# linjieli222/HERO

Hardware: AMD Instinct MI355X
Metric: videos/sec training step, HERO-base TVR-shaped batch (higher is better)
Workload: dtype bf16; 1 GPU; configs[1]: HERO-base TVR finetune micro-step (train-tvr-8gpu.json shapes: 32 videos x 60 frames, 15 subs x (4 frames + 20 tokens), 15-token query; vfeat 4352; fwd + VSM loss + bwd, all-reduce/clip/AdamW every 2nd micro-step); global_batch=32, parallelism=dp1, grad_accum=2, launch=hipGraph replay, input=one batch resident in HBM

## Files before the change

### hero_amd/_lib.py

```python
import ctypes as C
import os

import torch

_HERE = os.path.dirname(os.path.abspath(__file__))
LIB_PATH = os.environ.get("HERO_HIP_LIB") or os.path.join(_HERE, "libhero_hip.so")

ABI_VERSION = 3
F32, BF16 = 0, 1
LAYOUT_K, LAYOUT_O = 0, 1
ACT_NONE, ACT_GELU, ACT_RELU, ACT_GELU_BWD, ACT_RELU_BWD, ACT_GELU_DG, ACT_MUL_AUX = 0, 1, 2, 3, 4, 5, 6

EXPORTS = [
    "hero_last_error", "hero_abi_version", "hero_abi_struct_count", "hero_abi_struct_bytes", "hero_gemm", "hero_gemm_splits", "hero_fold_slabs", "hero_wgrad_group", "hero_wgrad_batch_plan", "hero_wgrad_batch", "hero_prof_enable", "hero_prof_read", "hero_probe_mfma", "hero_probe_hbm", "hero_gemm_force_config", "hero_layernorm_fwd",
    "hero_layernorm_bwd_workspace_bytes", "hero_layernorm_bwd", "hero_colsum_workspace_bytes",
    "hero_colsum", "hero_colsum_multi", "hero_colsum_multi_workspace_bytes", "hero_layernorm_bwd_blocks", "hero_attention_fwd", "hero_attention_bwd", "hero_attention_max_len", "hero_attention_max_packed_len", "hero_attention_stats_ok", "hero_attention_force_ppw",
    "hero_gather_rows", "hero_inverse_first", "hero_csr_gather_sum", "hero_scatter_add_rows", "hero_segment_sort_workspace_bytes", "hero_scatter_add_sorted_workspace_bytes", "hero_segment_sort", "hero_scatter_add_sorted", "hero_cast", "hero_transpose_cast", "hero_copy_multi",
    "hero_relu_bwd", "hero_gelu_bwd", "hero_add", "hero_sumsq", "hero_adamw", "hero_adamw_multi", "hero_adamw_multi_chunk",
    "hero_query_pool_fwd", "hero_query_pool_bwd", "hero_rownorm_fwd", "hero_rownorm_bwd", "hero_score_max_fwd",
    "hero_score_max_bwd", "hero_rank_loss", "hero_sums_scaled", "hero_st_ed_fwd", "hero_st_ed_bwd", "hero_st_ed_bwd_workspace_bytes",
    "hero_cross_entropy_fwd", "hero_cross_entropy_bwd", "hero_qa_pool_fwd", "hero_qa_pool_bwd",
    "hero_topk_rows", "hero_st_ed_probs", "hero_moment_topk", "hero_moment_nms", "hero_first_hit",
    "hero_collate_subs", "hero_collate_clip_mask", "hero_collate_frame_map", "hero_collate_gather_feats", "hero_derive_multi",
    "hero_comm_available", "hero_comm_unique_id", "hero_comm_init", "hero_comm_destroy", "hero_comm_rank", "hero_comm_world",
    "hero_comm_allreduce_buckets", "hero_comm_broadcast", "hero_comm_allgather", "hero_comm_allgather_var",
]


class Dropout(C.Structure):
    _fields_ = [("seed_ptr", C.c_void_p), ("site", C.c_uint64),
                ("threshold16", C.c_uint32), ("scale", C.c_float)]


class GemmEpilogue(C.Structure):
    _fields_ = [("bias", C.c_void_p), ("residual", C.c_void_p), ("aux", C.c_void_p),
                ("act", C.c_int), ("out_f32", C.c_int), ("beta", C.c_float),
                ("split_k", C.c_int), ("dropout", Dropout), ("colsum", C.c_void_p), ("colsum_partial", C.c_int), ("pad_", C.c_int), ("split_stride", C.c_longlong)]


class CrossEntropy(C.Structure):
    _fields_ = [("logits", C.c_void_p), ("labels", C.c_void_p), ("loss", C.c_void_p), ("lse", C.c_void_p),
                ("dloss", C.c_void_p), ("dlogits", C.c_void_p), ("rows", C.c_int), ("cols", C.c_int),
                ("ld", C.c_int), ("dtype", C.c_int), ("inv_temp", C.c_float), ("ignore_index", C.c_int64)]


class Derive(C.Structure):
    _fields_ = [("src", C.c_void_p), ("dst", C.c_void_p), ("n", C.c_int64), ("mode", C.c_int), ("p0", C.c_int),
                ("p1", C.c_int), ("p2", C.c_int)]


DERIVE_MASK_ADD, DERIVE_F32, DERIVE_I32, DERIVE_FLAT_GATHER = 0, 1, 2, 3


class WgradProblem(C.Structure):
    _fields_ = [("dy", C.c_void_p), ("x", C.c_void_p), ("dw", C.c_void_p), ("M", C.c_int), ("N", C.c_int),
                ("ld_dy", C.c_int), ("ld_x", C.c_int), ("ld_dw", C.c_int), ("split_hint", C.c_int), ("dbias", C.c_void_p)]


class LnFwd(C.Structure):
    _fields_ = [("x", C.c_void_p), ("tab", C.c_void_p * 3), ("idx", C.c_void_p * 3),
                ("gamma", C.c_void_p), ("beta", C.c_void_p), ("y", C.c_void_p),
                ("pre", C.c_void_p), ("mean", C.c_void_p), ("rstd", C.c_void_p),
                ("rows", C.c_int), ("cols", C.c_int), ("eps", C.c_float),
                ("x_dtype", C.c_int), ("y_dtype", C.c_int), ("dropout", Dropout)]


class LnBwd(C.Structure):
    _fields_ = [("x", C.c_void_p), ("dy", C.c_void_p), ("gamma", C.c_void_p),
                ("mean", C.c_void_p), ("rstd", C.c_void_p), ("dx", C.c_void_p),
                ("dx_dropped", C.c_void_p), ("dgamma", C.c_void_p), ("dbeta", C.c_void_p),
                ("grad_beta", C.c_float), ("workspace", C.c_void_p),
                ("rows", C.c_int), ("cols", C.c_int), ("x_dtype", C.c_int), ("dtype", C.c_int),
                ("dropout_out", Dropout), ("dropout_in", Dropout), ("dbias_in", C.c_void_p), ("defer_fold", C.c_int)]


class Colsum(C.Structure):
    _fields_ = [("src", C.c_void_p), ("dst", C.c_void_p), ("rows", C.c_int), ("cols", C.c_int), ("ld", C.c_int),
                ("dtype", C.c_int), ("beta", C.c_float), ("row_cols", C.c_int), ("dst_rows", C.c_void_p)]


class Attn(C.Structure):
    _fields_ = [("qkv", C.c_void_p), ("mask", C.c_void_p), ("ctx", C.c_void_p),
                ("probs", C.c_void_p), ("dctx", C.c_void_p), ("dqkv", C.c_void_p),
                ("S", C.c_int), ("L", C.c_int), ("H", C.c_int), ("scale", C.c_float),
                ("dtype", C.c_int), ("dropout", Dropout), ("seq_off", C.c_void_p), ("stats", C.c_void_p)]


class AdamW(C.Structure):
    _fields_ = [("p", C.c_void_p), ("g", C.c_void_p), ("m", C.c_void_p), ("v", C.c_void_p),
                ("n", C.c_size_t), ("lr", C.c_float), ("beta1", C.c_float), ("beta2", C.c_float),
                ("eps", C.c_float), ("weight_decay", C.c_float), ("step", C.c_int),
                ("grad_sumsq", C.c_void_p), ("max_grad_norm", C.c_float),
                ("grad_scale", C.c_float), ("shadow", C.c_void_p)]


class TensorDesc(C.Structure):
    _fields_ = [("p", C.c_void_p), ("g", C.c_void_p), ("m", C.c_void_p), ("v", C.c_void_p),
                ("n", C.c_uint64), ("group", C.c_int32), ("step_lag", C.c_int32)]


class AdamWGroup(C.Structure):
    _fields_ = [("lr", C.c_float), ("beta1", C.c_float), ("beta2", C.c_float), ("eps", C.c_float),
                ("weight_decay", C.c_float)]


class AdamWMulti(C.Structure):
    _fields_ = [("descs", C.c_void_p), ("chunk_tensor", C.c_void_p), ("chunk_index", C.c_void_p),
                ("n_chunks", C.c_int), ("groups", AdamWGroup * 8), ("step", C.c_int),
                ("grad_sumsq", C.c_void_p), ("max_grad_norm", C.c_float), ("grad_scale", C.c_float),
                ("step_ptr", C.c_void_p), ("lr_ptr", C.c_void_p), ("tensor_steps", C.c_void_p), ("n_tensors", C.c_int)]


class CopyDesc(C.Structure):
    _fields_ = [("src", C.c_void_p), ("dst", C.c_void_p), ("rows", C.c_int32), ("cols", C.c_int32),
                ("ldd", C.c_int32), ("transpose", C.c_int32), ("dst_dtype", C.c_int32), ("pad_", C.c_int32)]


class QueryPool(C.Structure):
    _fields_ = [("q", C.c_void_p), ("mask", C.c_void_p), ("w", C.c_void_p), ("pooled", C.c_void_p),
                ("att", C.c_void_p), ("dpooled", C.c_void_p), ("dq", C.c_void_p), ("dw", C.c_void_p),
                ("B", C.c_int), ("L", C.c_int), ("D", C.c_int), ("dtype", C.c_int)]


class RowNorm(C.Structure):
    _fields_ = [("x", C.c_void_p), ("y", C.c_void_p), ("rnorm", C.c_void_p), ("dy", C.c_void_p),
                ("dx", C.c_void_p), ("rows", C.c_int), ("cols", C.c_int), ("x_dtype", C.c_int),
                ("eps", C.c_float)]


class ScoreMax(C.Structure):
    _fields_ = [("s", C.c_void_p), ("mask", C.c_void_p), ("out", C.c_void_p), ("arg", C.c_void_p),
                ("ds_ctx", C.c_void_p), ("ds_q", C.c_void_p), ("gc", C.c_void_p), ("gq", C.c_void_p),
                ("qn", C.c_void_p), ("cn", C.c_void_p), ("dqn", C.c_void_p), ("dcn", C.c_void_p),
                ("M", C.c_int), ("N", C.c_int), ("L", C.c_int), ("D", C.c_int), ("n0", C.c_int),
                ("n_own", C.c_int), ("ld_s", C.c_int), ("gc_scale", C.c_float), ("gq_scale", C.c_float)]


class RankLoss(C.Structure):
    _fields_ = [("s", C.c_void_p), ("loss_ctx_rows", C.c_void_p), ("loss_q_rows", C.c_void_p),
                ("ds_ctx", C.c_void_p), ("ds_q", C.c_void_p), ("nq", C.c_int), ("nv", C.c_int),
                ("margin", C.c_float), ("lse", C.c_int), ("hard", C.c_int), ("pool", C.c_int),
                ("hard_w", C.c_float), ("easy_w", C.c_float)]


class StEd(C.Structure):
    _fields_ = [("q2", C.c_void_p), ("ctx", C.c_void_p), ("mask", C.c_void_p), ("w_st", C.c_void_p),
                ("w_ed", C.c_void_p), ("targets", C.c_void_p), ("loss_rows", C.c_void_p),
                ("p_st", C.c_void_p), ("p_ed", C.c_void_p), ("sim", C.c_void_p), ("g", C.c_void_p),
                ("dq2", C.c_void_p), ("dctx", C.c_void_p), ("dw_st", C.c_void_p), ("dw_ed", C.c_void_p),
                ("B", C.c_int), ("L", C.c_int), ("D", C.c_int), ("K", C.c_int), ("dtype", C.c_int), ("g_scale", C.c_float),
                ("ws", C.c_void_p)]


class CommBucket(C.Structure):
    _fields_ = [("buf", C.c_void_p), ("count", C.c_size_t), ("dtype", C.c_int), ("pad_", C.c_int)]


ABI_STRUCTS = [Dropout, GemmEpilogue, WgradProblem, LnFwd, LnBwd, Colsum, Attn, AdamW, TensorDesc, AdamWGroup, AdamWMulti,
               CopyDesc, QueryPool, RowNorm, ScoreMax, RankLoss, StEd, CrossEntropy, Derive, CommBucket]


def abi_struct_sizes():
    return {st.__name__: C.sizeof(st) for st in ABI_STRUCTS}


_lib = None


def lib():
    global _lib
    if _lib is None:
        if not os.path.exists(LIB_PATH):
            raise RuntimeError(
                "hero_amd: %s is missing. Build it with `python -m hero_amd.build` "
                "(needs hipcc; cross-compiles for gfx950 without a GPU). There is no fallback "
                "path." % LIB_PATH)
        L = C.CDLL(LIB_PATH)
        L.hero_last_error.restype = C.c_char_p
        have = L.hero_abi_version()
        if have != ABI_VERSION:
            raise RuntimeError("hero_amd: %s reports ABI version %d, this binding was written against %d (struct layouts "
                               "differ: rebuild with `python -m hero_amd.build --force`)" % (LIB_PATH, have, ABI_VERSION))
        L.hero_abi_struct_bytes.argtypes = [C.c_int]
        if L.hero_abi_struct_count() != len(ABI_STRUCTS):
            raise RuntimeError("hero_amd: %s declares %d ABI structs, this binding mirrors %d" % (LIB_PATH, L.hero_abi_struct_count(), len(ABI_STRUCTS)))
        bad = [(st.__name__, C.sizeof(st), L.hero_abi_struct_bytes(i)) for i, st in enumerate(ABI_STRUCTS)
               if C.sizeof(st) != L.hero_abi_struct_bytes(i)]
        if bad:
            raise RuntimeError("hero_amd: struct layouts differ from %s (name, binding bytes, library bytes): %s" % (LIB_PATH, bad))
        L.hero_layernorm_bwd_workspace_bytes.restype = C.c_size_t
        L.hero_colsum_workspace_bytes.restype = C.c_size_t
        L.hero_colsum_multi_workspace_bytes.restype = C.c_size_t
        L.hero_colsum_multi_workspace_bytes.argtypes = [C.POINTER(Colsum), C.c_int]
        L.hero_colsum_multi.argtypes = [C.POINTER(Colsum), C.c_int, C.c_void_p, C.c_void_p]
        L.hero_layernorm_bwd_blocks.argtypes = [C.c_int]
        L.hero_gemm.argtypes = [C.c_void_p, C.c_void_p, C.c_void_p] + [C.c_int] * 9 + [
            C.POINTER(GemmEpilogue), C.c_void_p]
        L.hero_gemm_splits.argtypes = [C.c_int, C.c_int, C.c_int]
        L.hero_fold_slabs.argtypes = [C.c_void_p, C.c_int, C.c_size_t, C.c_void_p, C.c_size_t, C.c_int, C.c_void_p]
        L.hero_wgrad_group.argtypes = [C.POINTER(WgradProblem), C.c_int, C.c_int, C.c_int, C.c_void_p]
        L.hero_wgrad_batch_plan.argtypes = [C.POINTER(WgradProblem), C.c_int, C.c_int, C.c_void_p, C.c_int]
        L.hero_wgrad_batch.argtypes = [C.POINTER(WgradProblem), C.c_int, C.c_int, C.c_int, C.c_void_p, C.c_int, C.c_void_p]
        L.hero_prof_enable.argtypes = [C.c_int]
        L.hero_prof_read.argtypes = [C.c_int, C.POINTER(C.c_double), C.POINTER(C.c_double),
                                     C.POINTER(C.c_longlong)]
        L.hero_probe_mfma.argtypes = [C.c_void_p, C.c_size_t, C.POINTER(C.c_double), C.POINTER(C.c_double), C.c_void_p]
        L.hero_probe_hbm.argtypes = [C.c_void_p, C.c_void_p, C.c_size_t, C.POINTER(C.c_double), C.POINTER(C.c_double), C.c_void_p]
        L.hero_layernorm_fwd.argtypes = [C.POINTER(LnFwd), C.c_void_p]
        L.hero_layernorm_bwd.argtypes = [C.POINTER(LnBwd), C.c_void_p]
        L.hero_layernorm_bwd_workspace_bytes.argtypes = [C.c_int, C.c_int]
        L.hero_colsum_workspace_bytes.argtypes = [C.c_int, C.c_int]
        L.hero_colsum.argtypes = [C.c_void_p, C.c_void_p, C.c_int, C.c_int, C.c_int, C.c_int,
                                  C.c_float, C.c_void_p, C.c_void_p]
        L.hero_attention_fwd.argtypes = [C.POINTER(Attn), C.c_void_p]
        L.hero_attention_bwd.argtypes = [C.POINTER(Attn), C.c_void_p]
        L.hero_attention_stats_ok.argtypes = [C.c_int, C.c_int]
        L.hero_attention_force_ppw.argtypes = [C.c_int]
        L.hero_attention_max_len.argtypes = [C.c_int, C.c_int]
        L.hero_attention_max_packed_len.argtypes = [C.c_int]
        L.hero_gather_rows.argtypes = [C.c_void_p, C.c_void_p, C.c_void_p, C.c_void_p,
                                       C.c_int, C.c_int, C.c_int, C.c_void_p]
        L.hero_inverse_first.argtypes = [C.c_void_p, C.c_int, C.c_void_p, C.c_int, C.c_int, C.c_void_p]
        L.hero_csr_gather_sum.argtypes = [C.c_void_p, C.c_void_p, C.c_void_p, C.c_void_p,
                                          C.c_int, C.c_int, C.c_int, C.c_void_p]
        L.hero_scatter_add_rows.argtypes = [C.c_void_p, C.c_void_p, C.c_void_p, C.c_void_p,
                                            C.c_int, C.c_int, C.c_int, C.c_int, C.c_int, C.c_void_p]
        L.hero_segment_sort_workspace_bytes.argtypes = [C.c_int]
        L.hero_segment_sort_workspace_bytes.restype = C.c_size_t
        L.hero_segment_sort.argtypes = [C.c_void_p, C.c_int, C.c_int, C.c_int, C.c_void_p, C.c_void_p, C.c_void_p]
        L.hero_scatter_add_sorted_workspace_bytes.argtypes = [C.c_int, C.c_int]
        L.hero_scatter_add_sorted_workspace_bytes.restype = C.c_size_t
        L.hero_scatter_add_sorted.argtypes = [C.c_void_p, C.c_void_p, C.c_void_p, C.c_void_p, C.c_int, C.c_int, C.c_int, C.c_int,
                                              C.c_void_p, C.c_void_p]
        L.hero_st_ed_bwd_workspace_bytes.argtypes = [C.c_int]
        L.hero_st_ed_bwd_workspace_bytes.restype = C.c_size_t
        L.hero_cast.argtypes = [C.c_void_p, C.c_void_p, C.c_size_t, C.c_int, C.c_int, C.c_void_p]
        L.hero_transpose_cast.argtypes = [C.c_void_p, C.c_void_p, C.c_int, C.c_int, C.c_int, C.c_int,
                                          C.c_void_p]
        L.hero_relu_bwd.argtypes = [C.c_void_p, C.c_void_p, C.c_void_p, C.c_size_t, C.c_int,
                                    C.c_void_p]
        L.hero_gelu_bwd.argtypes = L.hero_relu_bwd.argtypes
        L.hero_add.argtypes = [C.c_void_p, C.c_void_p, C.c_void_p, C.c_size_t, C.c_int, C.c_void_p]
        L.hero_sumsq.argtypes = [C.c_void_p, C.c_size_t, C.c_void_p, C.c_void_p, C.c_void_p]
        L.hero_adamw.argtypes = [C.POINTER(AdamW), C.c_void_p]
        L.hero_adamw_multi.argtypes = [C.POINTER(AdamWMulti), C.c_void_p]
        L.hero_copy_multi.argtypes = [C.c_void_p, C.c_void_p, C.c_void_p, C.c_int, C.c_void_p]
        for fn, st in (("hero_query_pool_fwd", QueryPool), ("hero_query_pool_bwd", QueryPool),
                       ("hero_rownorm_fwd", RowNorm), ("hero_rownorm_bwd", RowNorm),
                       ("hero_score_max_fwd", ScoreMax), ("hero_score_max_bwd", ScoreMax),
                       ("hero_rank_loss", RankLoss), ("hero_st_ed_fwd", StEd), ("hero_st_ed_bwd", StEd)):
            getattr(L, fn).argtypes = [C.POINTER(st), C.c_void_p]
        L.hero_sums_scaled.argtypes = [C.c_void_p, C.c_int, C.c_int, C.POINTER(C.c_float), C.c_void_p, C.c_void_p]
        L.hero_topk_rows.argtypes = [C.c_void_p, C.c_int, C.c_int, C.c_int, C.c_int, C.c_float, C.c_void_p, C.c_void_p, C.c_void_p]
        L.hero_st_ed_probs.argtypes = [C.c_void_p, C.c_longlong] + [C.c_void_p] * 4 + [C.c_int] * 5 + [C.c_void_p] * 3
        L.hero_moment_topk.argtypes = [C.c_void_p] * 3 + [C.c_int] * 6 + [C.c_void_p] * 3
        L.hero_moment_nms.argtypes = [C.c_void_p] * 3 + [C.c_int, C.c_int, C.c_double, C.c_int, C.c_int] + [C.c_void_p] * 3
        L.hero_first_hit.argtypes = [C.c_void_p] * 3 + [C.c_int] * 3 + [C.c_void_p, C.c_void_p, C.c_float, C.c_void_p, C.c_int, C.c_void_p, C.c_void_p]
        L.hero_collate_subs.argtypes = [C.c_void_p] * 4 + [C.c_int] * 3 + [C.c_void_p]
        L.hero_collate_gather_feats.argtypes = [C.c_void_p] * 7 + [C.c_int] * 5 + [C.c_void_p]
        L.hero_derive_multi.argtypes = [C.POINTER(Derive), C.c_int, C.c_void_p]
        L.hero_collate_clip_mask.argtypes = [C.c_void_p, C.c_void_p, C.c_int, C.c_int, C.c_void_p]
        L.hero_collate_frame_map.argtypes = [C.c_void_p] * 7 + [C.c_int] * 4 + [C.c_void_p]
        L.hero_cross_entropy_fwd.argtypes = [C.POINTER(CrossEntropy), C.c_void_p]
        L.hero_cross_entropy_bwd.argtypes = [C.POINTER(CrossEntropy), C.c_void_p]
        L.hero_qa_pool_fwd.argtypes = [C.c_void_p] * 8 + [C.c_int] * 6 + [C.c_void_p]
        L.hero_qa_pool_bwd.argtypes = [C.c_void_p] * 11 + [C.c_int] * 6 + [C.c_void_p]
        L.hero_comm_unique_id.argtypes = [C.c_void_p]
        L.hero_comm_init.argtypes = [C.c_void_p, C.c_int, C.c_int, C.POINTER(C.c_void_p)]
        L.hero_comm_destroy.argtypes = [C.c_void_p]
        L.hero_comm_rank.argtypes = [C.c_void_p]
        L.hero_comm_world.argtypes = [C.c_void_p]
        L.hero_comm_allreduce_buckets.argtypes = [C.c_void_p, C.POINTER(CommBucket), C.c_int, C.c_void_p]
        L.hero_comm_broadcast.argtypes = [C.c_void_p, C.c_void_p, C.c_size_t, C.c_int, C.c_void_p]
        L.hero_comm_allgather.argtypes = [C.c_void_p, C.c_void_p, C.c_void_p, C.c_size_t, C.c_void_p]
        L.hero_comm_allgather_var.argtypes = [C.c_void_p, C.c_void_p, C.c_void_p, C.POINTER(C.c_size_t), C.c_void_p]
        _lib = L
    return _lib


def check(rc):
    if rc != 0:
        raise RuntimeError("libhero_hip: %s (code %d)" % (lib().hero_last_error().decode(), rc))


def dt(t):
    if t.dtype == torch.float32:
        return F32
    if t.dtype == torch.bfloat16:
        return BF16
    raise TypeError("hero_amd: unsupported dtype %s (float32 / bfloat16 only)" % t.dtype)


def ptr(t):
    if t is None:
        return None
    if not t.is_cuda:
        raise RuntimeError("hero_amd: tensor is on %s; the HIP path needs CUDA/ROCm tensors and has "
                           "no CPU fallback" % t.device)
    if not t.is_contiguous():
        raise RuntimeError("hero_amd: non-contiguous tensor passed to a HIP kernel")
    return t.data_ptr()


_raw_stream = getattr(torch._C, "_cuda_getCurrentRawStream", None)
_cur_device = getattr(torch._C, "_cuda_getDevice", None)


def stream():
    if _raw_stream is not None and _cur_device is not None:
        return _raw_stream(_cur_device())
    return torch.cuda.current_stream().cuda_stream


def no_dropout():
    return Dropout(None, 0, 0, 1.0)
```

### hero_amd/csrc/rows.hip

```cpp
#include "common.h"

namespace hero {

template <typename T>
__global__ void gather_rows_kernel(const T* __restrict__ a, const T* __restrict__ b, const int32_t* __restrict__ idx,
                                   T* __restrict__ out, int rows, int cols) {
  const int c4n = cols >> 2;
  for (size_t q = blockIdx.x * (size_t)blockDim.x + threadIdx.x; q < (size_t)rows * c4n; q += (size_t)gridDim.x * blockDim.x) {
    const int r = (int)(q / c4n), c = (int)(q - (size_t)r * c4n) * 4;
    const int i = idx[r];
    float4 v = make_float4(0.f, 0.f, 0.f, 0.f);
    if (i >= 0) v = V4<T>::ld(a + (size_t)i * cols + c);
    else if (i <= -2) v = V4<T>::ld(b + (size_t)(-i - 2) * cols + c);
    V4<T>::st(out + (size_t)r * cols + c, v);
  }
}

__global__ __launch_bounds__(1024) void inverse_first_kernel(const int32_t* __restrict__ idx, int n, int32_t* __restrict__ inv, int na, int nb) {
  extern __shared__ int lds_inv[];
  const int tot = na + nb;
  for (int i = threadIdx.x; i < tot; i += 1024) lds_inv[i] = 0x7fffffff;
  __syncthreads();
  for (int j = threadIdx.x; j < n; j += 1024) {
    const int v = idx[j];
    if (v >= 0 && v < na) atomicMin(&lds_inv[v], j);
    else if (v <= -2 && -v - 2 < nb) atomicMin(&lds_inv[na - v - 2], j);
  }
  __syncthreads();
  for (int i = threadIdx.x; i < tot; i += 1024) { const int v = lds_inv[i]; inv[i] = v == 0x7fffffff ? -1 : v; }
}

template <typename T>
__global__ void csr_gather_sum_kernel(const T* __restrict__ src, const int32_t* __restrict__ offs,
                                      const int32_t* __restrict__ ent, T* __restrict__ out, int rows, int cols) {
  const int c4n = cols >> 2;
  for (size_t q = blockIdx.x * (size_t)blockDim.x + threadIdx.x; q < (size_t)rows * c4n; q += (size_t)gridDim.x * blockDim.x) {
    const int r = (int)(q / c4n), c = (int)(q - (size_t)r * c4n) * 4;
    float4 v = make_float4(0.f, 0.f, 0.f, 0.f);
    for (int e = offs[r]; e < offs[r + 1]; ++e) {
      const float4 w = V4<T>::ld(src + (size_t)ent[e] * cols + c);
      v.x += w.x; v.y += w.y; v.z += w.z; v.w += w.w;
    }
    V4<T>::st(out + (size_t)r * cols + c, v);
  }
}

__device__ __forceinline__ void atomic_add2(float* p, float x, float y) {
  atomicAdd(p, x);
  atomicAdd(p + 1, y);
}
__device__ __forceinline__ void atomic_add2(bf16_t* p, float x, float y) {
  uint32_t* w = reinterpret_cast<uint32_t*>(p);
  uint32_t old = *w, assumed;
  do {
    assumed = old;
    const float lo = __uint_as_float(assumed << 16) + x;
    const float hi = __uint_as_float(assumed & 0xffff0000u) + y;
    const uint32_t nw = (uint32_t)f2bf(lo) | ((uint32_t)f2bf(hi) << 16);
    old = atomicCAS(w, assumed, nw);
  } while (old != assumed);
}

template <typename TS, typename TD>
__global__ void scatter_add_rows_kernel(const TS* __restrict__ src, const int32_t* __restrict__ idx, TD* dst_a, TD* dst_b,
                                        int rows, int cols, int skip) {
  const int c2n = cols >> 1;
  for (size_t q = blockIdx.x * (size_t)blockDim.x + threadIdx.x; q < (size_t)rows * c2n; q += (size_t)gridDim.x * blockDim.x) {
    const int r = (int)(q / c2n), c = (int)(q - (size_t)r * c2n) * 2;
    const int i = idx[r];
    if (i == -1 || i == skip) continue;
    const float x = ld1<TS>(src + (size_t)r * cols + c), y = ld1<TS>(src + (size_t)r * cols + c + 1);
    if (x == 0.f && y == 0.f) continue;
    TD* d = i >= 0 ? dst_a + (size_t)i * cols + c : (dst_b ? dst_b + (size_t)(-i - 2) * cols + c : nullptr);
    if (d) atomic_add2(d, x, y);
  }
}

constexpr int SORT_NT = 1024;
__global__ __launch_bounds__(SORT_NT) void segment_sort_kernel(const int32_t* __restrict__ idx, int rows, int skip, int nbits,
                                                               uint2* __restrict__ buf0, uint2* __restrict__ buf1,
                                                               int32_t* __restrict__ order) {
  extern __shared__ uint32_t hist[];
  uint32_t* wsum = hist + 16 * SORT_NT;
  const int t = threadIdx.x, lane = t & 63, wv = t >> 6;
  const int cpt = (rows + SORT_NT - 1) / SORT_NT;
  const int beg = min(t * cpt, rows), end = min(beg + cpt, rows);
  const uint32_t last_key = (1u << nbits) - 1u;
  for (int i = beg; i < end; ++i) {
    const int v = idx[i];
    buf0[i] = make_uint2((v < 0 || v == skip) ? last_key : (uint32_t)v, (uint32_t)i);
  }
  __syncthreads();
  uint2* src = buf0;
  uint2* dst = buf1;
  for (int shift = 0; shift < nbits; shift += 4) {
    uint32_t cnt[16];
#pragma unroll
    for (int b = 0; b < 16; ++b) cnt[b] = 0;
    for (int i = beg; i < end; ++i) {
      const uint32_t d = (src[i].x >> shift) & 15u;
#pragma unroll
      for (int b = 0; b < 16; ++b) cnt[b] += (d == (uint32_t)b);
    }
#pragma unroll
    for (int b = 0; b < 16; ++b) hist[b * SORT_NT + t] = cnt[b];
    __syncthreads();
    uint32_t loc[16], run = 0;
#pragma unroll
    for (int k = 0; k < 16; ++k) { loc[k] = run; run += hist[16 * t + k]; }
    uint32_t inc = run;
#pragma unroll
    for (int o = 1; o < 64; o <<= 1) {
      const uint32_t u = __shfl_up(inc, o, 64);
      if (lane >= o) inc += u;
    }
    if (lane == 63) wsum[wv] = inc;
    __syncthreads();
    uint32_t base = inc - run;
    for (int w = 0; w < wv; ++w) base += wsum[w];
#pragma unroll
    for (int k = 0; k < 16; ++k) hist[16 * t + k] = base + loc[k];
    __syncthreads();
    uint32_t pos[16];
#pragma unroll
    for (int b = 0; b < 16; ++b) pos[b] = hist[b * SORT_NT + t];
    for (int i = beg; i < end; ++i) {
      const uint2 e = src[i];
      const uint32_t d = (e.x >> shift) & 15u;
      uint32_t at = 0;
#pragma unroll
      for (int b = 0; b < 16; ++b)
        if (d == (uint32_t)b) { at = pos[b]; pos[b] += 1; }
      dst[at] = e;
    }
    __syncthreads();
    uint2* tmp = src; src = dst; dst = tmp;
  }
  for (int i = t; i < rows; i += SORT_NT) order[i] = (int32_t)src[i].y;
}

#ifndef HERO_SEG_B
#define HERO_SEG_B 16
#endif
constexpr int SEG_B = HERO_SEG_B;
constexpr int UNR = 8;
__device__ __forceinline__ int seg_key(const int32_t* idx, const int32_t* order, int i, int rows, int skip) {
  if (i < 0 || i >= rows) return -2;
  const int v = idx[order[i]];
  return (v < 0 || v == skip) ? -1 : v;
}

template <typename TS, int NCH>
__global__ __launch_bounds__(256) void scatter_sorted_kernel(const TS* __restrict__ src, const int32_t* __restrict__ idx,
                                                             const int32_t* __restrict__ order, float* __restrict__ dst,
                                                             float* __restrict__ partial, int rows, int cols, int skip) {
  const int blk = blockIdx.x * 4 + (threadIdx.x >> 6), lane = threadIdx.x & 63;
  const int base = blk * SEG_B;
  if (base >= rows) return;
  const int n = min(SEG_B, rows - base);
  const int my_row = lane < n ? order[base + lane] : 0;
  int my_key = -2;
  if (lane < n) { const int v = idx[my_row]; my_key = (v < 0 || v == skip) ? -1 : v; }
  const int prev_key = seg_key(idx, order, base - 1, rows, skip), next_key = seg_key(idx, order, base + n, rows, skip);
  for (int c0 = 0; c0 < cols; c0 += NCH * 256) {
    float4 acc[NCH];
#pragma unroll
    for (int k = 0; k < NCH; ++k) acc[k] = make_float4(0.f, 0.f, 0.f, 0.f);
    int seg_start = 0;
    for (int p0 = 0; p0 < n; p0 += UNR) {
      float4 v[UNR][NCH], old[UNR][NCH];
      int keys[UNR];
#pragma unroll
      for (int u = 0; u < UNR; ++u) {
        const int p = min(p0 + u, n - 1);
        keys[u] = __shfl(my_key, p, 64);
        const int r = __shfl(my_row, p, 64);
        const int kd = max(keys[u], 0);
#pragma unroll
        for (int k = 0; k < NCH; ++k) {
          const int c = min(c0 + k * 256 + lane * 4, cols - 4);
          v[u][k] = V4<TS>::ld(src + (size_t)r * cols + c);
          old[u][k] = *reinterpret_cast<const float4*>(dst + (size_t)kd * cols + c);
        }
      }
#pragma unroll
      for (int u = 0; u < UNR; ++u) {
        const int p = p0 + u;
        if (p < n) {
          const int key = keys[u];
          const int key_next = p + 1 < n ? __shfl(my_key, p + 1, 64) : -3;
          if (key >= 0) {
#pragma unroll
            for (int k = 0; k < NCH; ++k) { acc[k].x += v[u][k].x; acc[k].y += v[u][k].y; acc[k].z += v[u][k].z; acc[k].w += v[u][k].w; }
          }
          if (key_next != key) {
            if (key >= 0) {
              const bool left_open = seg_start == 0 && prev_key == key;
              const bool right_open = p == n - 1 && next_key == key;
              const bool closed = !left_open && !right_open;
              float* out = closed ? dst + (size_t)key * cols : partial + ((size_t)blk * 2 + (left_open ? 0 : 1)) * cols;
#pragma unroll
              for (int k = 0; k < NCH; ++k) {
                const int c = c0 + k * 256 + lane * 4;
                if (c < cols) {
                  float4 o = acc[k];
                  if (closed) { o.x += old[u][k].x; o.y += old[u][k].y; o.z += old[u][k].z; o.w += old[u][k].w; }
                  *reinterpret_cast<float4*>(out + c) = o;
                }
              }
            }
#pragma unroll
            for (int k = 0; k < NCH; ++k) acc[k] = make_float4(0.f, 0.f, 0.f, 0.f);
            seg_start = p + 1;
          }
        }
      }
    }
  }
}

__global__ __launch_bounds__(256) void scatter_sorted_fold_kernel(const int32_t* __restrict__ idx, const int32_t* __restrict__ order,
                                                                  float* __restrict__ dst, const float* __restrict__ partial,
                                                                  int rows, int cols, int skip) {
  const int blk = blockIdx.x * 4 + (threadIdx.x >> 6), lane = threadIdx.x & 63;
  const int base = blk * SEG_B;
  if (base >= rows) return;
  const int n = min(SEG_B, rows - base);
  const int last = seg_key(idx, order, base + n - 1, rows, skip);
  if (last < 0 || seg_key(idx, order, base + n, rows, skip) != last) return;
  const bool whole = seg_key(idx, order, base, rows, skip) == last;
  if (whole && seg_key(idx, order, base - 1, rows, skip) == last) return;
  const int nblk = (rows + SEG_B - 1) / SEG_B;
  int nb = 0;
  for (int b0 = blk + 1; b0 < nblk; b0 += 64) {
    const int b = b0 + lane;
    const bool cont = b < nblk && seg_key(idx, order, b * SEG_B, rows, skip) == last;
    const unsigned long long m = __ballot(cont);
    const int run = m == ~0ull ? 64 : __builtin_ctzll(~m);
    nb += run;
    if (run < 64) break;
  }
  constexpr int NCH = 3, FB = 8;
  for (int c0 = 0; c0 < cols; c0 += NCH * 256) {
    float4 acc[NCH];
    int cc[NCH];
#pragma unroll
    for (int k = 0; k < NCH; ++k) {
      cc[k] = min(c0 + k * 256 + lane * 4, cols - 4);
      acc[k] = *reinterpret_cast<const float4*>(partial + ((size_t)blk * 2 + 1) * cols + cc[k]);
    }
    for (int b0 = 1; b0 <= nb; b0 += FB) {
      float4 t[FB][NCH];
#pragma unroll
      for (int u = 0; u < FB; ++u) {
        const int b = blk + min(b0 + u, nb);
#pragma unroll
        for (int k = 0; k < NCH; ++k) t[u][k] = *reinterpret_cast<const float4*>(partial + ((size_t)b * 2 + 0) * cols + cc[k]);
      }
#pragma unroll
      for (int u = 0; u < FB; ++u) {
        if (b0 + u <= nb) {
#pragma unroll
          for (int k = 0; k < NCH; ++k) { acc[k].x += t[u][k].x; acc[k].y += t[u][k].y; acc[k].z += t[u][k].z; acc[k].w += t[u][k].w; }
        }
      }
    }
#pragma unroll
    for (int k = 0; k < NCH; ++k) {
      const int c = c0 + k * 256 + lane * 4;
      if (c < cols) {
        float4* d = reinterpret_cast<float4*>(dst + (size_t)last * cols + c);
        float4 o = *d;
        o.x += acc[k].x; o.y += acc[k].y; o.z += acc[k].z; o.w += acc[k].w;
        *d = o;
      }
    }
  }
}

template <typename TS, typename TD>
__global__ void cast_kernel(const TS* __restrict__ s, TD* __restrict__ d, size_t n) {
  const size_t n4 = n >> 2;
  for (size_t q = blockIdx.x * (size_t)blockDim.x + threadIdx.x; q < n4; q += (size_t)gridDim.x * blockDim.x)
    V4<TD>::st(d + q * 4, V4<TS>::ld(s + q * 4));
  if (blockIdx.x == 0 && threadIdx.x < (n & 3)) st1<TD>(d + n4 * 4 + threadIdx.x, ld1<TS>(s + n4 * 4 + threadIdx.x));
}
template <typename TD>
__global__ __launch_bounds__(256) void transpose_cast_kernel(const float* __restrict__ src, TD* __restrict__ dst, int R, int C, int ldd) {
  __shared__ float tile[32][33];
  const int tx = threadIdx.x & 31, ty = threadIdx.x >> 5;
  const int r0 = blockIdx.y * 32, c0 = blockIdx.x * 32;
#pragma unroll
  for (int k = 0; k < 4; ++k) {
    const int r = r0 + ty + 8 * k, c = c0 + tx;
    tile[ty + 8 * k][tx] = (r < R && c < C) ? src[(size_t)r * C + c] : 0.f;
  }
  __syncthreads();
#pragma unroll
  for (int k = 0; k < 4; ++k) {
    const int c = c0 + ty + 8 * k, r = r0 + tx;
    if (c < C && r < R) st1<TD>(dst + (size_t)c * ldd + r, tile[tx][ty + 8 * k]);
  }
}

__global__ __launch_bounds__(256) void copy_multi_kernel(const HeroCopyDesc* __restrict__ descs, const int32_t* __restrict__ tile_desc,
                                                         const int32_t* __restrict__ tile_index) {
  __shared__ float tile[64][65];
  const HeroCopyDesc d = descs[tile_desc[blockIdx.x]];
  const int tcols = (d.cols + 63) >> 6;
  const int ti = tile_index[blockIdx.x];
  const int r0 = (ti / tcols) * 64, c0 = (ti % tcols) * 64;
  const int q = threadIdx.x & 15, ty = threadIdx.x >> 4;
  const bool vec = (d.cols & 3) == 0 && (d.ldd & 3) == 0 && ((uintptr_t)d.src & 15) == 0 && ((uintptr_t)d.dst & 15) == 0;
  if (!d.transpose) {
#pragma unroll
    for (int k = 0; k < 4; ++k) {
      const int r = r0 + ty + 16 * k, c = c0 + 4 * q;
      if (r >= d.rows || c >= d.cols) continue;
      if (vec) {
        const float4 v = *reinterpret_cast<const float4*>(d.src + (size_t)r * d.cols + c);
        if (d.dst_dtype == HERO_BF16) V4<bf16_t>::st(static_cast<bf16_t*>(d.dst) + (size_t)r * d.ldd + c, v);
        else *reinterpret_cast<float4*>(static_cast<float*>(d.dst) + (size_t)r * d.ldd + c) = v;
      } else {
        for (int e = 0; e < 4 && c + e < d.cols; ++e) {
          const float v = d.src[(size_t)r * d.cols + c + e];
          if (d.dst_dtype == HERO_BF16) static_cast<bf16_t*>(d.dst)[(size_t)r * d.ldd + c + e] = f2bf(v);
          else static_cast<float*>(d.dst)[(size_t)r * d.ldd + c + e] = v;
        }
      }
    }
    return;
  }
  const bool vin = (d.cols & 3) == 0 && ((uintptr_t)d.src & 15) == 0;
#pragma unroll
  for (int k = 0; k < 4; ++k) {
    const int rl = ty + 16 * k, r = r0 + rl, c = c0 + 4 * q;
    float4 v = make_float4(0.f, 0.f, 0.f, 0.f);
    if (r < d.rows && c < d.cols) {
      if (vin) v = *reinterpret_cast<const float4*>(d.src + (size_t)r * d.cols + c);
      else {
        v.x = d.src[(size_t)r * d.cols + c];
        if (c + 1 < d.cols) v.y = d.src[(size_t)r * d.cols + c + 1];
        if (c + 2 < d.cols) v.z = d.src[(size_t)r * d.cols + c + 2];
        if (c + 3 < d.cols) v.w = d.src[(size_t)r * d.cols + c + 3];
      }
    }
    tile[rl][4 * q] = v.x; tile[rl][4 * q + 1] = v.y; tile[rl][4 * q + 2] = v.z; tile[rl][4 * q + 3] = v.w;
  }
  __syncthreads();
  const bool vout = (d.ldd & 3) == 0 && (((uintptr_t)d.dst) & 15) == 0 && (d.rows & 3) == 0;
#pragma unroll
  for (int k = 0; k < 4; ++k) {
    const int cl = ty + 16 * k, c = c0 + cl, r = r0 + 4 * q;
    if (c >= d.cols || r >= d.rows) continue;
    const float4 v = make_float4(tile[4 * q][cl], tile[4 * q + 1][cl], tile[4 * q + 2][cl], tile[4 * q + 3][cl]);
    if (vout) {
      if (d.dst_dtype == HERO_BF16) V4<bf16_t>::st(static_cast<bf16_t*>(d.dst) + (size_t)c * d.ldd + r, v);
      else *reinterpret_cast<float4*>(static_cast<float*>(d.dst) + (size_t)c * d.ldd + r) = v;
    } else {
      const float e4[4] = {v.x, v.y, v.z, v.w};
      for (int e = 0; e < 4 && r + e < d.rows; ++e) {
        if (d.dst_dtype == HERO_BF16) static_cast<bf16_t*>(d.dst)[(size_t)c * d.ldd + r + e] = f2bf(e4[e]);
        else static_cast<float*>(d.dst)[(size_t)c * d.ldd + r + e] = e4[e];
      }
    }
  }
}

template <typename T>
__global__ void relu_bwd_kernel(const T* __restrict__ dy, const T* __restrict__ y, T* __restrict__ dx, size_t n) {
  const size_t n4 = n >> 2;
  for (size_t q = blockIdx.x * (size_t)blockDim.x + threadIdx.x; q < n4; q += (size_t)gridDim.x * blockDim.x) {
    float4 g = V4<T>::ld(dy + q * 4);
    const float4 v = V4<T>::ld(y + q * 4);
    g.x = v.x > 0.f ? g.x : 0.f; g.y = v.y > 0.f ? g.y : 0.f; g.z = v.z > 0.f ? g.z : 0.f; g.w = v.w > 0.f ? g.w : 0.f;
    V4<T>::st(dx + q * 4, g);
  }
}
template <typename T>
__global__ void gelu_bwd_kernel(const T* __restrict__ dy, const T* __restrict__ u, T* __restrict__ dx, size_t n) {
  const size_t n4 = n >> 2;
  for (size_t q = blockIdx.x * (size_t)blockDim.x + threadIdx.x; q < n4; q += (size_t)gridDim.x * blockDim.x) {
    float4 g = V4<T>::ld(dy + q * 4);
    const float4 v = V4<T>::ld(u + q * 4);
    g.x *= gelu_erf_grad(v.x); g.y *= gelu_erf_grad(v.y); g.z *= gelu_erf_grad(v.z); g.w *= gelu_erf_grad(v.w);
    V4<T>::st(dx + q * 4, g);
  }
}
template <typename T>
__global__ void add_kernel(const T* __restrict__ a, const T* __restrict__ b, T* __restrict__ y, size_t n) {
  const size_t n4 = n >> 2;
  for (size_t q = blockIdx.x * (size_t)blockDim.x + threadIdx.x; q < n4; q += (size_t)gridDim.x * blockDim.x) {
    float4 u = V4<T>::ld(a + q * 4);
    const float4 v = V4<T>::ld(b + q * 4);
    u.x += v.x; u.y += v.y; u.z += v.z; u.w += v.w;
    V4<T>::st(y + q * 4, u);
  }
}

__global__ void sumsq_kernel(const float* __restrict__ g, size_t n, float* out) {
  __shared__ float red[4];
  float s = 0.f;
  const size_t n4 = n >> 2;
  for (size_t q = blockIdx.x * (size_t)blockDim.x + threadIdx.x; q < n4; q += (size_t)gridDim.x * blockDim.x) {
    const float4 v = *reinterpret_cast<const float4*>(g + q * 4);
    s += (v.x * v.x + v.y * v.y) + (v.z * v.z + v.w * v.w);
  }
  if (blockIdx.x == 0 && threadIdx.x < (n & 3)) { const float v = g[n4 * 4 + threadIdx.x]; s += v * v; }
  s = wave_sum(s);
  if ((threadIdx.x & 63) == 0) red[threadIdx.x >> 6] = s;
  __syncthreads();
  if (threadIdx.x == 0) out[blockIdx.x] = (red[0] + red[1]) + (red[2] + red[3]);
}
__global__ void sumsq_final_kernel(const float* __restrict__ partial, int nblocks, float* out) {
  __shared__ float red[4];
  float s = 0.f;
  for (int i = threadIdx.x; i < nblocks; i += 256) s += partial[i];
  s = wave_sum(s);
  if ((threadIdx.x & 63) == 0) red[threadIdx.x >> 6] = s;
  __syncthreads();
  if (threadIdx.x == 0) out[0] += (red[0] + red[1]) + (red[2] + red[3]);
}

__global__ void adamw_kernel(HeroAdamW a, float bc1, float bc2) {
  float gs = a.grad_scale;
  if (a.grad_sumsq) {
    const float norm = sqrtf(*a.grad_sumsq) * fabsf(a.grad_scale);
    const float clip = a.max_grad_norm / (norm + 1e-6f);
    if (clip < 1.f) gs *= clip;
  }
  const float step_size = a.lr * sqrtf(bc2) / bc1;
  const float decay = a.lr * a.weight_decay;
  bf16_t* sh = static_cast<bf16_t*>(a.shadow);
  const size_t n4 = a.n >> 2;
  for (size_t q = blockIdx.x * (size_t)blockDim.x + threadIdx.x; q < n4; q += (size_t)gridDim.x * blockDim.x) {
    float4 p = *reinterpret_cast<float4*>(a.p + q * 4);
    const float4 g4 = *reinterpret_cast<const float4*>(a.g + q * 4);
    float4 m = *reinterpret_cast<float4*>(a.m + q * 4);
    float4 v = *reinterpret_cast<float4*>(a.v + q * 4);
    float* pp = &p.x; const float* gp = &g4.x; float* mp = &m.x; float* vp = &v.x;
#pragma unroll
    for (int k = 0; k < 4; ++k) {
      const float g = gp[k] * gs;
      mp[k] = a.beta1 * mp[k] + (1.f - a.beta1) * g;
      vp[k] = a.beta2 * vp[k] + (1.f - a.beta2) * g * g;
      pp[k] -= step_size * mp[k] / (sqrtf(vp[k]) + a.eps);
      pp[k] -= decay * pp[k];
    }
    *reinterpret_cast<float4*>(a.p + q * 4) = p;
    *reinterpret_cast<float4*>(a.m + q * 4) = m;
    *reinterpret_cast<float4*>(a.v + q * 4) = v;
    if (sh) V4<bf16_t>::st(sh + q * 4, p);
  }
  if (blockIdx.x == 0 && threadIdx.x < (a.n & 3)) {
    const size_t i = n4 * 4 + threadIdx.x;
    const float g = a.g[i] * gs;
    const float m = a.beta1 * a.m[i] + (1.f - a.beta1) * g;
    const float v = a.beta2 * a.v[i] + (1.f - a.beta2) * g * g;
    float p = a.p[i] - step_size * m / (sqrtf(v) + a.eps);
    p -= decay * p;
    a.p[i] = p; a.m[i] = m; a.v[i] = v;
    if (sh) sh[i] = f2bf(p);
  }
}

constexpr int MT_CHUNK = 16384;
__global__ void adamw_steps_inc_kernel(const HeroTensorDesc* descs, int n, int32_t* steps) {
  const int i = blockIdx.x * blockDim.x + threadIdx.x;
  if (i < n) steps[descs[i].step_lag] += 1;
}
__global__ __launch_bounds__(256) void adamw_multi_kernel(HeroAdamWMulti a) {
  const int ti = a.chunk_tensor[blockIdx.x];
  const HeroTensorDesc d = a.descs[ti];
  const HeroAdamWGroup gr = a.groups[d.group];
  const size_t beg = (size_t)a.chunk_index[blockIdx.x] * MT_CHUNK;
  const size_t end = beg + MT_CHUNK < d.n ? beg + MT_CHUNK : d.n;
  float gs = a.grad_scale;
  if (a.grad_sumsq) {
    const float norm = sqrtf(*a.grad_sumsq) * fabsf(a.grad_scale);
    const float clip = a.max_grad_norm / (norm + 1e-6f);
    if (clip < 1.f) gs *= clip;
  }
  const float st = a.tensor_steps ? (float)a.tensor_steps[d.step_lag] : (float)((a.step_ptr ? *a.step_ptr : a.step) - d.step_lag);
  const float lr = a.lr_ptr ? a.lr_ptr[d.group] : gr.lr;
  const float bc1 = 1.f - powf(gr.beta1, st), bc2 = 1.f - powf(gr.beta2, st);
  const float step_size = lr * sqrtf(bc2) / bc1;
  const float decay = lr * gr.weight_decay;
  const bool vec = (((uintptr_t)d.p | (uintptr_t)d.g | (uintptr_t)d.m | (uintptr_t)d.v) & 15) == 0;
  if (vec) {
    const size_t e4 = beg + ((end - beg) & ~(size_t)3);
    for (size_t i = beg + threadIdx.x * 4; i < e4; i += 256 * 4) {
      float4 p = *reinterpret_cast<float4*>(d.p + i);
      const float4 g4 = *reinterpret_cast<const float4*>(d.g + i);
      float4 m = *reinterpret_cast<float4*>(d.m + i);
      float4 v = *reinterpret_cast<float4*>(d.v + i);
      float* pp = &p.x; const float* gp = &g4.x; float* mp = &m.x; float* vp = &v.x;
#pragma unroll
      for (int k = 0; k < 4; ++k) {
        const float g = gp[k] * gs;
        mp[k] = gr.beta1 * mp[k] + (1.f - gr.beta1) * g;
        vp[k] = gr.beta2 * vp[k] + (1.f - gr.beta2) * g * g;
        pp[k] -= step_size * mp[k] / (sqrtf(vp[k]) + gr.eps);
        pp[k] -= decay * pp[k];
      }
      *reinterpret_cast<float4*>(d.p + i) = p;
      *reinterpret_cast<float4*>(d.m + i) = m;
      *reinterpret_cast<float4*>(d.v + i) = v;
    }
    for (size_t i = e4 + threadIdx.x; i < end; i += 256) {
      const float g = d.g[i] * gs;
      const float m = gr.beta1 * d.m[i] + (1.f - gr.beta1) * g;
      const float v = gr.beta2 * d.v[i] + (1.f - gr.beta2) * g * g;
      float p = d.p[i] - step_size * m / (sqrtf(v) + gr.eps);
      p -= decay * p;
      d.p[i] = p; d.m[i] = m; d.v[i] = v;
    }
  } else {
    for (size_t i = beg + threadIdx.x; i < end; i += 256) {
      const float g = d.g[i] * gs;
      const float m = gr.beta1 * d.m[i] + (1.f - gr.beta1) * g;
      const float v = gr.beta2 * d.v[i] + (1.f - gr.beta2) * g * g;
      float p = d.p[i] - step_size * m / (sqrtf(v) + gr.eps);
      p -= decay * p;
      d.p[i] = p; d.m[i] = m; d.v[i] = v;
    }
  }
}

static inline int grid_for(size_t work_items) {
  size_t b = (work_items + 255) / 256;
  if (b < 1) b = 1;
  if (b > 2048) b = 2048;
  return (int)b;
}

}

using namespace hero;

extern "C" int hero_gather_rows(const void* a, const void* b, const int32_t* idx, void* out, int rows, int cols, int dtype,
                                hero_stream_t stream) {
  HERO_REQUIRE(idx && out, "hero_gather_rows: null pointer");
  HERO_REQUIRE(cols > 0 && cols % 4 == 0, "hero_gather_rows: cols (%d) must be a multiple of 4", cols);
  if (rows <= 0) return HERO_OK;
  hipStream_t s = static_cast<hipStream_t>(stream);
  const int grid = grid_for((size_t)rows * (cols >> 2));
  if (dtype == HERO_F32)
    hipLaunchKernelGGL(gather_rows_kernel<float>, dim3(grid), dim3(256), 0, s, (const float*)a, (const float*)b, idx, (float*)out, rows, cols);
  else if (dtype == HERO_BF16)
    hipLaunchKernelGGL(gather_rows_kernel<bf16_t>, dim3(grid), dim3(256), 0, s, (const bf16_t*)a, (const bf16_t*)b, idx, (bf16_t*)out, rows, cols);
  else { set_error("hero_gather_rows: bad dtype %d", dtype); return HERO_ERR_ARG; }
  return check_launch("hero_gather_rows");
}

extern "C" int hero_inverse_first(const int32_t* idx, int n, int32_t* inv, int na, int nb, hero_stream_t stream) {
  HERO_REQUIRE(idx && inv && n >= 0 && na >= 0 && nb >= 0, "hero_inverse_first: bad arguments");
  if (na + nb == 0) return HERO_OK;
  const size_t lds = (size_t)(na + nb) * sizeof(int);
  if (lds > 150 * 1024) { set_error("hero_inverse_first: %d source rows exceed the LDS-resident table (38400)", na + nb); return HERO_ERR_UNSUPPORTED; }
  if (lds > 65536) HERO_ENSURE_LDS(&inverse_first_kernel, 150 * 1024, "inverse_first_kernel");
  hipLaunchKernelGGL(inverse_first_kernel, dim3(1), dim3(1024), lds, static_cast<hipStream_t>(stream), idx, n, inv, na, nb);
  return check_launch("hero_inverse_first");
}

extern "C" int hero_csr_gather_sum(const void* src, const int32_t* offsets, const int32_t* entries, void* out, int rows,
                                   int cols, int dtype, hero_stream_t stream) {
  HERO_REQUIRE(src && offsets && out, "hero_csr_gather_sum: null pointer");
  HERO_REQUIRE(cols > 0 && cols % 4 == 0, "hero_csr_gather_sum: cols (%d) must be a multiple of 4", cols);
  if (rows <= 0) return HERO_OK;
  hipStream_t s = static_cast<hipStream_t>(stream);
  const int grid = grid_for((size_t)rows * (cols >> 2));
  if (dtype == HERO_F32)
    hipLaunchKernelGGL(csr_gather_sum_kernel<float>, dim3(grid), dim3(256), 0, s, (const float*)src, offsets, entries, (float*)out, rows, cols);
  else if (dtype == HERO_BF16)
    hipLaunchKernelGGL(csr_gather_sum_kernel<bf16_t>, dim3(grid), dim3(256), 0, s, (const bf16_t*)src, offsets, entries, (bf16_t*)out, rows, cols);
  else { set_error("hero_csr_gather_sum: bad dtype %d", dtype); return HERO_ERR_ARG; }
  return check_launch("hero_csr_gather_sum");
}

extern "C" int hero_scatter_add_rows(const void* src, const int32_t* idx, void* dst_a, void* dst_b, int rows, int cols,
                                     int src_dtype, int dst_dtype, int skip_idx, hero_stream_t stream) {
  HERO_REQUIRE(src && idx && dst_a, "hero_scatter_add_rows: null pointer");
  HERO_REQUIRE(cols > 0 && cols % 2 == 0, "hero_scatter_add_rows: cols (%d) must be even", cols);
  if (rows <= 0) return HERO_OK;
  hipStream_t s = static_cast<hipStream_t>(stream);
  const int grid = grid_for((size_t)rows * (cols >> 1));
  const int skip = skip_idx >= 0 ? skip_idx : -1;
  if (src_dtype == HERO_F32 && dst_dtype == HERO_F32)
    hipLaunchKernelGGL((scatter_add_rows_kernel<float, float>), dim3(grid), dim3(256), 0, s, (const float*)src, idx, (float*)dst_a, (float*)dst_b, rows, cols, skip);
  else if (src_dtype == HERO_BF16 && dst_dtype == HERO_F32)
    hipLaunchKernelGGL((scatter_add_rows_kernel<bf16_t, float>), dim3(grid), dim3(256), 0, s, (const bf16_t*)src, idx, (float*)dst_a, (float*)dst_b, rows, cols, skip);
  else if (src_dtype == HERO_BF16 && dst_dtype == HERO_BF16)
    hipLaunchKernelGGL((scatter_add_rows_kernel<bf16_t, bf16_t>), dim3(grid), dim3(256), 0, s, (const bf16_t*)src, idx, (bf16_t*)dst_a, (bf16_t*)dst_b, rows, cols, skip);
  else { set_error("hero_scatter_add_rows: unsupported dtypes %d -> %d", src_dtype, dst_dtype); return HERO_ERR_UNSUPPORTED; }
  return check_launch("hero_scatter_add_rows");
}

extern "C" size_t hero_segment_sort_workspace_bytes(int rows) { return (size_t)(rows > 0 ? rows : 0) * 2 * sizeof(uint2); }

extern "C" int hero_segment_sort(const int32_t* idx, int rows, int n_dst, int skip_idx, int32_t* order, void* workspace,
                                 hero_stream_t stream) {
  HERO_REQUIRE(idx && order && workspace, "hero_segment_sort: null pointer");
  HERO_REQUIRE(n_dst > 0 && n_dst < (1 << 30), "hero_segment_sort: n_dst = %d", n_dst);
  if (rows <= 0) return HERO_OK;
  int nbits = 1;
  while ((1 << nbits) <= n_dst) ++nbits;
  nbits = (nbits + 3) & ~3;
  const int lds = (16 * SORT_NT + 32) * (int)sizeof(uint32_t);
  HERO_ENSURE_LDS(&segment_sort_kernel, lds, "segment_sort_kernel");
  uint2* b0 = static_cast<uint2*>(workspace);
  hipLaunchKernelGGL(segment_sort_kernel, dim3(1), dim3(SORT_NT), lds, static_cast<hipStream_t>(stream), idx, rows,
                     skip_idx >= 0 ? skip_idx : -1, nbits, b0, b0 + rows, order);
  return check_launch("hero_segment_sort");
}

extern "C" size_t hero_scatter_add_sorted_workspace_bytes(int rows, int cols) {
  if (rows <= 0 || cols <= 0) return 0;
  return (size_t)((rows + SEG_B - 1) / SEG_B) * 2 * (size_t)cols * sizeof(float);
}

extern "C" int hero_scatter_add_sorted(const void* src, const int32_t* idx, const int32_t* order, float* dst, int rows, int cols,
                                       int src_dtype, int skip_idx, void* workspace, hero_stream_t stream) {
  HERO_REQUIRE(src && idx && order && dst && workspace, "hero_scatter_add_sorted: null pointer");
  HERO_REQUIRE(cols > 0 && cols % 4 == 0, "hero_scatter_add_sorted: cols (%d) must be a multiple of 4", cols);
  if (rows <= 0) return HERO_OK;
  hipStream_t s = static_cast<hipStream_t>(stream);
  const int nblk = (rows + SEG_B - 1) / SEG_B, grid = (nblk + 3) / 4, skip = skip_idx >= 0 ? skip_idx : -1;
  float* part = static_cast<float*>(workspace);
  if (src_dtype == HERO_BF16) hipLaunchKernelGGL((scatter_sorted_kernel<bf16_t, 3>), dim3(grid), dim3(256), 0, s, (const bf16_t*)src, idx, order, dst, part, rows, cols, skip);
  else if (src_dtype == HERO_F32) hipLaunchKernelGGL((scatter_sorted_kernel<float, 3>), dim3(grid), dim3(256), 0, s, (const float*)src, idx, order, dst, part, rows, cols, skip);
  else { set_error("hero_scatter_add_sorted: bad dtype %d", src_dtype); return HERO_ERR_ARG; }
  int rc = check_launch("hero_scatter_add_sorted");
  if (rc) return rc;
  hipLaunchKernelGGL(scatter_sorted_fold_kernel, dim3(grid), dim3(256), 0, s, idx, order, dst, part, rows, cols, skip);
  return check_launch("hero_scatter_add_sorted(fold)");
}

extern "C" int hero_cast(const void* src, void* dst, size_t n, int sd, int dd, hero_stream_t stream) {
  HERO_REQUIRE(src && dst, "hero_cast: null pointer");
  if (n == 0) return HERO_OK;
  hipStream_t s = static_cast<hipStream_t>(stream);
  const int grid = grid_for(n >> 2);
  if (sd == HERO_F32 && dd == HERO_BF16) hipLaunchKernelGGL((cast_kernel<float, bf16_t>), dim3(grid), dim3(256), 0, s, (const float*)src, (bf16_t*)dst, n);
  else if (sd == HERO_BF16 && dd == HERO_F32) hipLaunchKernelGGL((cast_kernel<bf16_t, float>), dim3(grid), dim3(256), 0, s, (const bf16_t*)src, (float*)dst, n);
  else if (sd == HERO_F32 && dd == HERO_F32) hipLaunchKernelGGL((cast_kernel<float, float>), dim3(grid), dim3(256), 0, s, (const float*)src, (float*)dst, n);
  else if (sd == HERO_BF16 && dd == HERO_BF16) hipLaunchKernelGGL((cast_kernel<bf16_t, bf16_t>), dim3(grid), dim3(256), 0, s, (const bf16_t*)src, (bf16_t*)dst, n);
  else { set_error("hero_cast: bad dtypes %d -> %d", sd, dd); return HERO_ERR_ARG; }
  return check_launch("hero_cast");
}

extern "C" int hero_transpose_cast(const float* src, void* dst, int rows, int cols, int ldd, int dst_dtype, hero_stream_t stream) {
  HERO_REQUIRE(src && dst, "hero_transpose_cast: null pointer");
  if (rows <= 0 || cols <= 0) return HERO_OK;
  hipStream_t s = static_cast<hipStream_t>(stream);
  const dim3 grid((cols + 31) / 32, (rows + 31) / 32);
  if (dst_dtype == HERO_BF16) hipLaunchKernelGGL(transpose_cast_kernel<bf16_t>, grid, dim3(256), 0, s, src, (bf16_t*)dst, rows, cols, ldd);
  else if (dst_dtype == HERO_F32) hipLaunchKernelGGL(transpose_cast_kernel<float>, grid, dim3(256), 0, s, src, (float*)dst, rows, cols, ldd);
  else { set_error("hero_transpose_cast: bad dtype %d", dst_dtype); return HERO_ERR_ARG; }
  return check_launch("hero_transpose_cast");
}

extern "C" int hero_copy_multi(const HeroCopyDesc* descs, const int32_t* tile_desc, const int32_t* tile_index, int n_tiles,
                               hero_stream_t stream) {
  HERO_REQUIRE(descs && tile_desc && tile_index, "hero_copy_multi: null pointer");
  if (n_tiles <= 0) return HERO_OK;
  hipLaunchKernelGGL(copy_multi_kernel, dim3(n_tiles), dim3(256), 0, static_cast<hipStream_t>(stream), descs, tile_desc, tile_index);
  return check_launch("hero_copy_multi");
}

extern "C" int hero_relu_bwd(const void* dy, const void* y, void* dx, size_t n, int dtype, hero_stream_t stream) {
  HERO_REQUIRE(dy && y && dx, "hero_relu_bwd: null pointer");
  HERO_REQUIRE(n % 4 == 0, "hero_relu_bwd: n must be a multiple of 4");
  if (n == 0) return HERO_OK;
  hipStream_t s = static_cast<hipStream_t>(stream);
  const int grid = grid_for(n >> 2);
  if (dtype == HERO_F32) hipLaunchKernelGGL(relu_bwd_kernel<float>, dim3(grid), dim3(256), 0, s, (const float*)dy, (const float*)y, (float*)dx, n);
  else if (dtype == HERO_BF16) hipLaunchKernelGGL(relu_bwd_kernel<bf16_t>, dim3(grid), dim3(256), 0, s, (const bf16_t*)dy, (const bf16_t*)y, (bf16_t*)dx, n);
  else { set_error("hero_relu_bwd: bad dtype %d", dtype); return HERO_ERR_ARG; }
  return check_launch("hero_relu_bwd");
}

extern "C" int hero_gelu_bwd(const void* dy, const void* u, void* dx, size_t n, int dtype, hero_stream_t stream) {
  HERO_REQUIRE(dy && u && dx, "hero_gelu_bwd: null pointer");
  HERO_REQUIRE(n % 4 == 0, "hero_gelu_bwd: n must be a multiple of 4");
  if (n == 0) return HERO_OK;
  hipStream_t s = static_cast<hipStream_t>(stream);
  const int grid = grid_for(n >> 2);
  if (dtype == HERO_F32) hipLaunchKernelGGL(gelu_bwd_kernel<float>, dim3(grid), dim3(256), 0, s, (const float*)dy, (const float*)u, (float*)dx, n);
  else if (dtype == HERO_BF16) hipLaunchKernelGGL(gelu_bwd_kernel<bf16_t>, dim3(grid), dim3(256), 0, s, (const bf16_t*)dy, (const bf16_t*)u, (bf16_t*)dx, n);
  else { set_error("hero_gelu_bwd: bad dtype %d", dtype); return HERO_ERR_ARG; }
  return check_launch("hero_gelu_bwd");
}

extern "C" int hero_add(const void* a, const void* b, void* y, size_t n, int dtype, hero_stream_t stream) {
  HERO_REQUIRE(a && b && y, "hero_add: null pointer");
  HERO_REQUIRE(n % 4 == 0, "hero_add: n must be a multiple of 4");
  if (n == 0) return HERO_OK;
  hipStream_t s = static_cast<hipStream_t>(stream);
  const int grid = grid_for(n >> 2);
  if (dtype == HERO_F32) hipLaunchKernelGGL(add_kernel<float>, dim3(grid), dim3(256), 0, s, (const float*)a, (const float*)b, (float*)y, n);
  else if (dtype == HERO_BF16) hipLaunchKernelGGL(add_kernel<bf16_t>, dim3(grid), dim3(256), 0, s, (const bf16_t*)a, (const bf16_t*)b, (bf16_t*)y, n);
  else { set_error("hero_add: bad dtype %d", dtype); return HERO_ERR_ARG; }
  return check_launch("hero_add");
}

template <typename TO>
__global__ void __launch_bounds__(256) fold_slabs_kernel(const float* __restrict__ slabs, int n_slabs, size_t stride, TO* __restrict__ out, size_t n4) {
  for (size_t i = (size_t)blockIdx.x * 256 + threadIdx.x; i < n4; i += (size_t)gridDim.x * 256) {
    float4 a = *reinterpret_cast<const float4*>(slabs + 4 * i);
    for (int s = 1; s < n_slabs; ++s) {
      const float4 b = *reinterpret_cast<const float4*>(slabs + (size_t)s * stride + 4 * i);
      a.x += b.x; a.y += b.y; a.z += b.z; a.w += b.w;
    }
    V4<TO>::st(out + 4 * i, a);
  }
}

extern "C" int hero_fold_slabs(const float* slabs, int n_slabs, size_t stride, void* out, size_t n, int out_dtype, hero_stream_t stream) {
  HERO_REQUIRE(slabs && out && n_slabs >= 1, "hero_fold_slabs: null pointer / no slab");
  HERO_REQUIRE(n % 4 == 0 && stride % 4 == 0 && (((uintptr_t)slabs | (uintptr_t)out) & 7) == 0, "hero_fold_slabs: n and stride must be multiples of 4, pointers aligned");
  if (n == 0) return HERO_OK;
  hipStream_t s = static_cast<hipStream_t>(stream);
  const int grid = grid_for(n >> 2);
  if (out_dtype == HERO_F32) hipLaunchKernelGGL(fold_slabs_kernel<float>, dim3(grid), dim3(256), 0, s, slabs, n_slabs, stride, (float*)out, n >> 2);
  else if (out_dtype == HERO_BF16) hipLaunchKernelGGL(fold_slabs_kernel<bf16_t>, dim3(grid), dim3(256), 0, s, slabs, n_slabs, stride, (bf16_t*)out, n >> 2);
  else { set_error("hero_fold_slabs: bad dtype %d", out_dtype); return HERO_ERR_ARG; }
  return check_launch("hero_fold_slabs");
}

extern "C" int hero_sumsq(const float* g, size_t n, float* sumsq, float* workspace, hero_stream_t stream) {
  HERO_REQUIRE(g && sumsq && workspace, "hero_sumsq: null pointer");
  if (n == 0) return HERO_OK;
  hipStream_t s = static_cast<hipStream_t>(stream);
  const int nb = grid_for(n >> 2);
  hipLaunchKernelGGL(sumsq_kernel, dim3(nb), dim3(256), 0, s, g, n, workspace);
  hipLaunchKernelGGL(sumsq_final_kernel, dim3(1), dim3(256), 0, s, workspace, nb, sumsq);
  return check_launch("hero_sumsq");
}

extern "C" int hero_adamw(const HeroAdamW* a, hero_stream_t stream) {
  HERO_REQUIRE(a && a->p && a->g && a->m && a->v, "hero_adamw: null pointer");
  HERO_REQUIRE(a->step >= 1, "hero_adamw: step must be >= 1");
  if (a->n == 0) return HERO_OK;
  hipStream_t s = static_cast<hipStream_t>(stream);
  const float bc1 = 1.f - powf(a->beta1, (float)a->step);
  const float bc2 = 1.f - powf(a->beta2, (float)a->step);
  hipLaunchKernelGGL(adamw_kernel, dim3(grid_for(a->n >> 2)), dim3(256), 0, s, *a, bc1, bc2);
  return check_launch("hero_adamw");
}

extern "C" int hero_adamw_multi(const HeroAdamWMulti* a, hero_stream_t stream) {
  HERO_REQUIRE(a && a->descs && a->chunk_tensor && a->chunk_index, "hero_adamw_multi: null pointer");
  HERO_REQUIRE(a->step >= 1 || a->step_ptr || a->tensor_steps, "hero_adamw_multi: step must be >= 1");
  if (a->n_chunks <= 0) return HERO_OK;
  if (a->tensor_steps) {
    HERO_REQUIRE(a->n_tensors > 0, "hero_adamw_multi: tensor_steps needs n_tensors");
    hipLaunchKernelGGL(adamw_steps_inc_kernel, dim3((a->n_tensors + 255) / 256), dim3(256), 0, static_cast<hipStream_t>(stream), a->descs,
                       a->n_tensors, a->tensor_steps);
    const int rc = check_launch("hero_adamw_multi(steps)");
    if (rc) return rc;
  }
  hipLaunchKernelGGL(adamw_multi_kernel, dim3(a->n_chunks), dim3(256), 0, static_cast<hipStream_t>(stream), *a);
  return check_launch("hero_adamw_multi");
}
extern "C" int hero_adamw_multi_chunk(void) { return MT_CHUNK; }
```

### hero_amd/functional.py

```python
import ctypes as C
import math
import os
import weakref

import numpy as np
import torch

from . import _lib as L

_COMPUTE_DTYPE = torch.bfloat16


def set_compute_dtype(dtype):
    global _COMPUTE_DTYPE
    if dtype not in (torch.float32, torch.bfloat16):
        raise ValueError("compute dtype must be torch.float32 or torch.bfloat16")
    _COMPUTE_DTYPE = dtype


def compute_dtype():
    return _COMPUTE_DTYPE


class _Rng:

    def __init__(self):
        self.seeds = {}
        self.site = 0

    def seed_tensor(self, device):
        idx = device.index if device.index is not None else (torch.cuda.current_device() if device.type == "cuda" else None)
        key = (device.type, idx)
        t = self.seeds.get(key)
        if t is None:
            t = torch.tensor([torch.initial_seed() & 0x7FFFFFFFFFFFFFFF], dtype=torch.int64,
                             device=device)
            self.seeds[key] = t
        return t

    def make(self, p, training, device):
        if not training or p <= 0.0:
            return None
        if p >= 1.0:
            raise ValueError("dropout p must be < 1")
        self.site += 1
        return L.Dropout(self.seed_tensor(device).data_ptr(), self.site,
                         max(1, int(round(p * 65536.0))), 1.0 / (1.0 - p))


RNG = _Rng()


def manual_seed(seed, device=None):
    RNG.site = 0
    for t in RNG.seeds.values():
        t.fill_(seed & 0x7FFFFFFFFFFFFFFF)
    if device is not None:
        RNG.seed_tensor(torch.device(device)).fill_(seed & 0x7FFFFFFFFFFFFFFF)


def advance_seed():
    for t in RNG.seeds.values():
        t.add_(1)


def _d(drop):
    return drop if drop is not None else L.no_dropout()


_WCACHE = {}
_WEPOCH = [0]
_WGEN = [0]


def weight_cache_generation():
    return _WGEN[0]


def notify_weights_updated():
    _WEPOCH[0] += 1


def clear_weight_cache():
    _WGEN[0] += 1
    _WCACHE.clear()
    for k in [k for k in _REFRESH if k not in _REFRESH_PINNED]:
        del _REFRESH[k]


_TRUST = [False]


class weights_frozen:

    def __enter__(self):
        self.prev = _TRUST[0]
        _TRUST[0] = True

    def __exit__(self, *exc):
        _TRUST[0] = self.prev


_REFRESH = {}
_REFRESH_PINNED = set()


def refresh_weight_cache():
    if not _WCACHE:
        return
    entries = list(_WCACHE.items())
    tsig = tuple((key, val[1].data_ptr(), tuple(p.data_ptr() for p in val[2])) for key, val in entries)
    if tsig not in _REFRESH:
        if len(_REFRESH) > 16:
            for k in [k for k in _REFRESH if k not in _REFRESH_PINNED][:8]:
                del _REFRESH[k]
        descs, tdesc, tidx = [], [], []
        for key, (_, out, params) in entries:
            transposed = len(key) == 3
            esz, code = out.element_size(), L.dt(out)
            off = 0
            for p in params:
                if not p.is_contiguous() or p.dtype != torch.float32:
                    raise RuntimeError("hero_amd: master weights must be contiguous fp32")
                rows = p.shape[0] if p.dim() > 1 else 1
                cols = p.numel() // rows
                if transposed:
                    d = L.CopyDesc(p.data_ptr(), out.data_ptr() + off * esz, rows, cols, out.shape[1], 1, code, 0)
                    off += rows
                else:
                    d = L.CopyDesc(p.data_ptr(), out.data_ptr() + off * esz, rows, cols, cols, 0, code, 0)
                    off += rows * cols
                nt = (-(-rows // 64)) * (-(-cols // 64))
                tdesc += [len(descs)] * nt
                tidx += list(range(nt))
                descs.append(d)
        dev = entries[0][1][1].device
        arr = (L.CopyDesc * len(descs))(*descs)
        raw = torch.frombuffer(bytearray(bytes(arr)), dtype=torch.uint8).to(dev)
        _REFRESH[tsig] = (raw, torch.tensor(tdesc, dtype=torch.int32, device=dev),
                          torch.tensor(tidx, dtype=torch.int32, device=dev), len(tdesc))
    if torch.cuda.is_current_stream_capturing():
        _REFRESH_PINNED.add(tsig)
    raw, tdesc, tidx, n = _REFRESH[tsig]
    L.check(L.lib().hero_copy_multi(raw.data_ptr(), tdesc.data_ptr(), tidx.data_ptr(), n, L.stream()))
    ep = _WEPOCH[0]
    for key, (_, out, params) in entries:
        _WCACHE[key] = ((tuple(p._version for p in params), tuple(p.data_ptr() for p in params), ep), out, params)


def packed(params, dtype):
    params = tuple(params)
    if len(params) == 1 and dtype == torch.float32 and params[0].is_contiguous():
        return params[0].detach()
    key = (tuple(id(p) for p in params), dtype)
    hit = _WCACHE.get(key)
    if _TRUST[0] and hit is not None and hit[0] is not None and hit[0][2] == _WEPOCH[0]:
        return hit[1]
    sig = (tuple(p._version for p in params), tuple(p.data_ptr() for p in params), _WEPOCH[0])
    if hit is not None and hit[0] == sig:
        return hit[1]
    rows = sum(p.shape[0] for p in params)
    shape = (rows,) + tuple(params[0].shape[1:])
    reuse = hit is not None and tuple(hit[1].shape) == shape and hit[1].device == params[0].device
    out = hit[1] if reuse else torch.empty(shape, dtype=dtype, device=params[0].device)
    off = 0
    for p in params:
        n = p.numel()
        dst = out[off:off + p.shape[0]]
        L.check(L.lib().hero_cast(L.ptr(p.detach().contiguous()), dst.data_ptr(), n, L.F32,
                                  L.dt(out), L.stream()))
        off += p.shape[0]
    if hit is None or not reuse:
        _WGEN[0] += 1
    _WCACHE[key] = (sig, out, params)
    return out


def packed_t(params, dtype):
    params = tuple(params)
    key = (tuple(id(p) for p in params), dtype, "T")
    hit = _WCACHE.get(key)
    if _TRUST[0] and hit is not None and hit[0] is not None and hit[0][2] == _WEPOCH[0]:
        return hit[1]
    sig = (tuple(p._version for p in params), tuple(p.data_ptr() for p in params), _WEPOCH[0])
    if hit is not None and hit[0] == sig:
        return hit[1]
    kin = params[0].shape[1]
    cols = sum(p.shape[0] for p in params)
    reuse = hit is not None and tuple(hit[1].shape) == (kin, cols) and hit[1].device == params[0].device
    out = hit[1] if reuse else torch.empty((kin, cols), dtype=dtype, device=params[0].device)
    off = 0
    for p in params:
        L.check(L.lib().hero_transpose_cast(L.ptr(p.detach().contiguous()),
                                            out.data_ptr() + off * out.element_size(), p.shape[0], kin,
                                            cols, L.dt(out), L.stream()))
        off += p.shape[0]
    if hit is None or not reuse:
        _WGEN[0] += 1
    _WCACHE[key] = (sig, out, params)
    return out


class GradSink:

    def dst(self, p):
        if p.grad is None:
            p.grad = torch.zeros_like(p, memory_format=torch.contiguous_format)
        return p.grad

    def dst_group(self, params):
        return None

    def use(self, p):
        pass

    def done(self, p):
        pass

    def wants_overlap(self):
        return False


SINK = GradSink()


def set_grad_sink(sink):
    global SINK
    SINK = sink if sink is not None else GradSink()


def _use(*params):
    for p in params:
        if p is not None and p.requires_grad:
            SINK.use(p)


def _is_param(t):
    return t is not None and t.is_leaf and t.requires_grad


def _p(t):
    return t if isinstance(t, int) else L.ptr(t)


def k_gemm(A, B, Cm, M, N, K, lda, ldb, ldc, al, bl, dtype_code, bias=None, residual=None,
           aux=None, act=L.ACT_NONE, out_f32=False, beta=0.0, split_k=1, drop=None, colsum=None, split_stride=0,
           colsum_partial=False):
    epi = L.GemmEpilogue(_p(bias), _p(residual), _p(aux), act, 1 if out_f32 else 0,
                         beta, split_k, _d(drop), _p(colsum), 1 if colsum_partial else 0, 0, split_stride)
    L.check(L.lib().hero_gemm(_p(A), _p(B), _p(Cm), M, N, K, lda, ldb, ldc, al, bl,
                              dtype_code, C.byref(epi), L.stream()))


def k_linear(x2, Wc, bias=None, act=L.ACT_NONE, aux=None, residual=None, drop=None):
    M, K = x2.shape
    N = Wc.shape[0]
    y = torch.empty((M, N), dtype=x2.dtype, device=x2.device)
    k_gemm(x2, Wc, y, M, N, K, K, K, N, L.LAYOUT_K, L.LAYOUT_K, L.dt(x2), bias=bias,
           residual=residual, aux=aux, act=act, drop=drop)
    return y


def k_dgrad(dy2, Wc, act=L.ACT_NONE, aux=None, residual=None):
    M, N = dy2.shape
    K = Wc.shape[1]
    dx = torch.empty((M, K), dtype=dy2.dtype, device=dy2.device)
    k_gemm(dy2, Wc, dx, M, K, N, N, K, K, L.LAYOUT_K, L.LAYOUT_O, L.dt(dy2), act=act, aux=aux,
           residual=residual)
    return dx


def k_dgrad_t(dy2, Wt, act=L.ACT_NONE, aux=None, residual=None, colsum=None, colsum_partial=False):
    M, N = dy2.shape
    K = Wt.shape[0]
    if (dy2.dtype == torch.bfloat16 and act == L.ACT_NONE and aux is None and residual is None and colsum is None
            and N >= 8192 and M * K <= (1 << 21) and (M * K) % 4 == 0 and (N - N // 64 * 64) % 8 == 0
            and dy2.is_contiguous() and Wt.is_contiguous() and Wt.shape[1] == N):
        return _dgrad_long_reduction(dy2, Wt)
    dx = torch.empty((M, K), dtype=dy2.dtype, device=dy2.device)
    k_gemm(dy2, Wt, dx, M, K, N, N, N, K, L.LAYOUT_K, L.LAYOUT_K, L.dt(dy2), act=act, aux=aux,
           residual=residual, colsum=colsum, colsum_partial=colsum_partial)
    return dx


def _dgrad_long_reduction(dy2, Wt):
    M, N = dy2.shape
    K = Wt.shape[0]
    n1 = N // 64 * 64
    tiles = -(-M // 128) * -(-K // 128)
    split = max(1, min(n1 // 64 // 8, 16, -(-512 // tiles)))
    n_main = L.lib().hero_gemm_splits(n1, split, L.BF16)
    stride = M * K
    slabs = torch.empty((n_main + (1 if n1 < N else 0), M, K), dtype=torch.float32, device=dy2.device)
    if n_main > 1:
        k_gemm(dy2, Wt, slabs, M, K, n1, N, N, K, L.LAYOUT_K, L.LAYOUT_K, L.BF16, out_f32=True, split_k=split, split_stride=stride)
    else:
        k_gemm(dy2, Wt, slabs, M, K, n1, N, N, K, L.LAYOUT_K, L.LAYOUT_K, L.BF16, out_f32=True)
    if n1 < N:
        k_gemm(L.ptr(dy2) + 2 * n1, L.ptr(Wt) + 2 * n1, L.ptr(slabs) + 4 * n_main * stride, M, K, N - n1, N, N, K,
               L.LAYOUT_K, L.LAYOUT_K, L.BF16, out_f32=True)
    out = torch.empty((M, K), dtype=torch.bfloat16, device=dy2.device)
    L.check(L.lib().hero_fold_slabs(L.ptr(slabs), slabs.shape[0], stride, L.ptr(out), stride, L.BF16, L.stream()))
    return out


def _split_for(n_out, n_in, rows, bk):
    tiles = ((n_out + 127) // 128) * ((n_in + 127) // 128)
    ktiles = max(1, -(-rows // bk))
    flops = 2.0 * n_out * n_in * rows
    out_bytes = 4.0 * n_out * n_in
    best, best_t = 1, None
    for s in range(1, 17):
        if s > 1 and ktiles // s < 4:
            break
        blocks = tiles * s
        rounds = -(-blocks // 512)
        last = blocks - (rounds - 1) * 512
        t = flops / blocks * ((rounds - 1) / 1.83e12 + (1 / 2.7e12 if last <= 256 else 1 / 1.83e12))
        if s > 1:
            t += out_bytes * s / 2.0e12
        if best_t is None or t < best_t:
            best, best_t = s, t
    return best


_WQ = []
_WQ_TASK = [-1]
GROUP_WGRADS = [True]
WGRAD_BATCH = [32]
WGRAD_DBIAS_RIDE = [True]
WGRAD_RIDE_MAX_ROWS = [1 << 30]
B1_EPILOGUE = [False]
B1_PARTIALS = [True]
WGRAD_QUEUE_BYTES = [int(os.environ.get("HERO_WGRAD_QUEUE_MB", "4096")) << 20]
_WQ_BYTES = [0]
_WPLANS = {}
_WPLANS_PINNED = set()


def _wgrad_queue_full(device):
    if _WQ_BYTES[0] <= WGRAD_QUEUE_BYTES[0]:
        return False
    hard = _WQ_HARD.get(device.index)
    if hard is None:
        env = os.environ.get("HERO_WGRAD_QUEUE_HARD_MB")
        hard = (int(env) << 20) if env else max(2 * WGRAD_QUEUE_BYTES[0], int(0.15 * torch.cuda.get_device_properties(device).total_memory))
        _WQ_HARD[device.index] = hard
    if _WQ_BYTES[0] > hard:
        return True
    tiles = sum(-(-e[4] // 192) * -(-e[1].shape[1] // 192) for e in _WQ)
    full, rem = divmod(tiles, 256)
    if rem == 0:
        return True
    p = -(-rem // 8)
    slices = max(1, min(32 // p, 8))
    return tiles / 256.0 >= 0.9 * (full + (1.4 if slices > 1 else 1.0) / slices)


_WQ_HARD = {}


def _wgrad_limit():
    return 4 if (WGRAD_BATCH[0] <= 4 or SINK.wants_overlap()) else min(WGRAD_BATCH[0], 32)


def _wgrad_plan(probs, n, rows, device):
    key = (rows, device.index, tuple((probs[i].M, probs[i].N) for i in range(n)))
    hit = _WPLANS.get(key, False)
    if hit is False:
        buf = np.zeros(8 + 8 * 512 * 16, dtype=np.int32)
        words = L.lib().hero_wgrad_batch_plan(probs, n, rows, buf.ctypes.data, buf.size)
        if words < 0:
            L.check(words)
        hit = (torch.from_numpy(buf[:words].copy()).to(device), words) if words > 0 else None
        if len(_WPLANS) > 256:
            for k in [k for k in _WPLANS if k not in _WPLANS_PINNED][:128]:
                del _WPLANS[k]
        _WPLANS[key] = hit
    if hit is not None and torch.cuda.is_current_stream_capturing():
        _WPLANS_PINNED.add(key)
    return hit


_CB_TASK = [-1]


def _ensure_flush_callback(task):
    if _CB_TASK[0] != task:
        _CB_TASK[0] = task
        torch.autograd.Variable._execution_engine.queue_callback(deferred_flush)


def deferred_flush():
    _CB_TASK[0] = -1
    wgrad_flush()
    colsum_flush()


_CQ = []
_CQ_TASK = [-1]


def _colsum_defer_ok():
    return GROUP_WGRADS[0] and not SINK.wants_overlap() and torch._C._current_graph_task_id() != -1


def _colsum_queue(keep, src_ptr, dst, rows, cols, ld, dtype, on_done=None, dst_rows=None, row_cols=0):
    task = torch._C._current_graph_task_id()
    if _CQ and _CQ_TASK[0] != task:
        del _CQ[:]
    _CQ_TASK[0] = task
    _ensure_flush_callback(task)
    _CQ.append(((keep, dst_rows), L.Colsum(src_ptr, L.ptr(dst), rows, cols, ld, dtype, 1.0, row_cols, L.ptr(dst_rows)), dst, on_done))
    if len(_CQ) >= 64:
        colsum_flush()


def colsum_flush():
    while _CQ:
        part, seen = [], []
        while _CQ and len(part) < 64:
            lo = _CQ[0][1].dst
            hi = lo + 4 * _CQ[0][2].numel()
            if any(lo < b and a < hi for a, b in seen):
                break
            seen.append((lo, hi))
            part.append(_CQ.pop(0))
        n = len(part)
        probs = (L.Colsum * n)(*[e[1] for e in part])
        need = L.lib().hero_colsum_multi_workspace_bytes(probs, n) // 4
        ws = _workspace(max(need, 1), part[0][2].device, slot="colsum_multi")
        L.check(L.lib().hero_colsum_multi(probs, n, L.ptr(ws), L.stream()))
        for e in part:
            if e[3] is not None:
                e[3]()


def wgrad_flush():
    _WQ_BYTES[0] = 0
    while _WQ:
        rows, dtype = _WQ[0][0].shape[0], _WQ[0][0].dtype
        dst_key = lambda e: (e[2].data_ptr(), e[6].data_ptr() if e[6] is not None else None)
        seen_w, seen_b = {_WQ[0][2].data_ptr()}, {dst_key(_WQ[0])[1]} - {None}
        n = 1
        while n < len(_WQ) and n < 32 and _WQ[n][0].shape[0] == rows and _WQ[n][0].dtype == dtype:
            kw, kb = dst_key(_WQ[n])
            if kw in seen_w or (kb is not None and kb in seen_b):
                break
            seen_w.add(kw)
            if kb is not None:
                seen_b.add(kb)
            n += 1
        group, rest = _WQ[:n], _WQ[n:]
        del _WQ[:]
        _WQ.extend(rest)
        probs = (L.WgradProblem * n)()
        for i, (dy2, x2, out, col0, N, _, _, _) in enumerate(group):
            K = x2.shape[1]
            probs[i] = L.WgradProblem(L.ptr(dy2) + col0 * dy2.element_size(), L.ptr(x2), L.ptr(out), N, K,
                                      dy2.shape[1], K, K, _split_for(N, K, rows, 64 if dtype == torch.bfloat16 else 32), None)
        plan = _wgrad_plan(probs, n, rows, group[0][0].device) if dtype == torch.bfloat16 else None
        if plan is not None:
            ride = WGRAD_DBIAS_RIDE[0] and rows <= WGRAD_RIDE_MAX_ROWS[0]
            for i, e in enumerate(group):
                probs[i].dbias = L.ptr(e[6]) if ride else None
                if not ride and e[6] is not None:
                    k_colsum(e[0], out=e[6], beta=1.0, col0=e[3], ncols=e[4], on_done=lambda: None)
            L.check(L.lib().hero_wgrad_batch(probs, n, rows, L.BF16, L.ptr(plan[0]), plan[1], L.stream()))
            for e in group:
                if e[6] is not None and e[7] is not None:
                    e[7]()
        else:
            for g0 in range(0, n, 4):
                sub = (L.WgradProblem * min(4, n - g0))(*[probs[i] for i in range(g0, min(g0 + 4, n))])
                L.check(L.lib().hero_wgrad_group(sub, len(sub), rows, L.dt(group[0][0]), L.stream()))
            for dy2, _, _, col0, N, _, dbias, dbias_done in group:
                if dbias is not None:
                    k_colsum(dy2, out=dbias, beta=1.0, col0=col0, ncols=N, on_done=dbias_done or (lambda: None))
        for e in group:
            if e[5] is not None:
                e[5]()


def k_wgrad(dy2, x2, out=None, beta=0.0, col0=0, ncols=None, on_done=None, dbias=None, dbias_done=None):
    M, ld = dy2.shape
    N = ld - col0 if ncols is None else ncols
    K = x2.shape[1]
    if (out is not None and beta == 1.0 and GROUP_WGRADS[0] and out.is_contiguous() and dy2.is_contiguous()
            and x2.is_contiguous() and torch._C._current_graph_task_id() != -1):
        task = torch._C._current_graph_task_id()
        if _WQ and _WQ_TASK[0] != task:
            del _WQ[:]
            _WQ_BYTES[0] = 0
        if _WQ and (_WQ[0][0].shape[0] != M or _WQ[0][0].dtype != dy2.dtype):
            wgrad_flush()
        if not _WQ:
            _WQ_TASK[0] = task
        _ensure_flush_callback(task)
        _WQ.append((dy2, x2, out, col0, N, on_done, dbias, dbias_done))
        _WQ_BYTES[0] += dy2.numel() * dy2.element_size()
        if len(_WQ) >= _wgrad_limit() or _wgrad_queue_full(dy2.device):
            wgrad_flush()
        return out
    if dbias is not None:
        k_colsum(dy2, out=dbias, beta=1.0, col0=col0, ncols=N, on_done=dbias_done or (lambda: None))
    if out is None:
        out = torch.empty((N, K), dtype=torch.float32, device=dy2.device)
    split = _split_for(N, K, M, 64 if dy2.dtype == torch.bfloat16 else 32)
    a = L.ptr(dy2) + col0 * dy2.element_size()
    k_gemm(a, x2, out, N, K, M, ld, K, K, L.LAYOUT_O, L.LAYOUT_O, L.dt(dy2), out_f32=True,
           beta=beta, split_k=split)
    if on_done is not None:
        on_done()
    return out


_WS = {}


def _workspace(n_floats, device, slot=""):
    key = (device.type, device.index, slot)
    t = _WS.get(key)
    if t is None or t.numel() < n_floats:
        t = torch.empty((max(n_floats, 1 << 20),), dtype=torch.float32, device=device)
        _WS[key] = t
    return t


def k_colsum(dy2, out=None, beta=0.0, col0=0, ncols=None, on_done=None):
    M, ld = dy2.shape
    N = ld - col0 if ncols is None else ncols
    if (on_done is not None and out is not None and beta == 1.0 and dy2.is_contiguous() and N % 4 == 0 and ld % 4 == 0
            and (col0 * dy2.element_size()) % 8 == 0 and _colsum_defer_ok()):
        _colsum_queue(dy2, L.ptr(dy2) + col0 * dy2.element_size(), out, M, N, ld, L.dt(dy2), on_done)
        return out
    if out is None:
        out = torch.empty((N,), dtype=torch.float32, device=dy2.device)
    ws = _workspace(256 * N, dy2.device)
    L.check(L.lib().hero_colsum(L.ptr(dy2) + col0 * dy2.element_size(), L.ptr(out), M, N, ld,
                                L.dt(dy2), beta, L.ptr(ws), L.stream()))
    if on_done is not None:
        on_done()
    return out


def acc_linear_grads(dy2, x2, weight, bias, col0=0, ncols=None):
    N = ncols if ncols is not None else weight.shape[0]
    want_b = bias is not None and bias.requires_grad
    if weight is not None and weight.requires_grad:
        k_wgrad(dy2, x2, out=SINK.dst(weight), beta=1.0, col0=col0, ncols=N, on_done=lambda: SINK.done(weight),
                dbias=SINK.dst(bias) if want_b else None, dbias_done=(lambda: SINK.done(bias)) if want_b else None)
    elif want_b:
        k_colsum(dy2, out=SINK.dst(bias), beta=1.0, col0=col0, ncols=N, on_done=lambda: SINK.done(bias))


def k_ln_fwd(x2, gamma, beta, eps, out_dtype, rows, cols, tabs=(), idxs=(), want_pre=False,
             drop=None, device=None):
    device = device or (x2.device if x2 is not None else gamma.device)
    y = torch.empty((rows, cols), dtype=out_dtype, device=device)
    mean = torch.empty((rows,), dtype=torch.float32, device=device)
    rstd = torch.empty((rows,), dtype=torch.float32, device=device)
    pre = torch.empty((rows, cols), dtype=out_dtype, device=device) if want_pre else None
    a = L.LnFwd()
    a.x = L.ptr(x2)
    for k in range(3):
        a.tab[k] = L.ptr(tabs[k]) if k < len(tabs) else None
        a.idx[k] = L.ptr(idxs[k]) if k < len(idxs) and idxs[k] is not None else None
    a.gamma, a.beta, a.y, a.pre = L.ptr(gamma), L.ptr(beta), L.ptr(y), L.ptr(pre)
    a.mean, a.rstd = L.ptr(mean), L.ptr(rstd)
    a.rows, a.cols, a.eps = rows, cols, eps
    a.x_dtype = L.dt(x2) if x2 is not None else L.dt(y)
    a.y_dtype = L.dt(y)
    a.dropout = _d(drop)
    L.check(L.lib().hero_layernorm_fwd(C.byref(a), L.stream()))
    return y, mean, rstd, pre


def ln_param_dsts(gamma_p, beta_p):
    dg = SINK.dst(gamma_p) if gamma_p.requires_grad else None
    db = SINK.dst(beta_p) if beta_p.requires_grad else None
    return dg, db


def ln_params_done(gamma_p, beta_p):
    if gamma_p.requires_grad:
        SINK.done(gamma_p)
    if beta_p.requires_grad:
        SINK.done(beta_p)


def k_ln_bwd(x2, dy2, gamma, mean, rstd, want_dx=True, want_params=True, drop_out=None,
             drop_in=None, dgamma=None, dbeta=None, grad_beta=0.0, dbias_in=None):
    rows, cols = dy2.shape
    dev = dy2.device
    dx = torch.empty_like(dy2) if want_dx else None
    dxd = torch.empty_like(dy2) if (want_dx and drop_in is not None) else None
    dg, db = dgamma, dbeta
    if want_params and dg is None and db is None:
        dg = torch.empty((cols,), dtype=torch.float32, device=dev)
        db = torch.empty((cols,), dtype=torch.float32, device=dev)
    ws = _workspace(3072 * cols, dev) if (dg is not None or db is not None or dbias_in is not None) else None
    defer = (grad_beta == 1.0 and ws is not None and cols <= 1024 and (want_dx or dbias_in is not None) and _colsum_defer_ok())
    if defer:
        nblk = L.lib().hero_layernorm_bwd_blocks(rows)
        ws = torch.empty((nblk, 3 * cols), dtype=torch.float32, device=dev)
    a = L.LnBwd()
    a.x, a.dy, a.gamma, a.mean, a.rstd = L.ptr(x2), L.ptr(dy2), L.ptr(gamma), L.ptr(mean), L.ptr(rstd)
    a.dx, a.dx_dropped, a.dgamma, a.dbeta = L.ptr(dx), L.ptr(dxd), L.ptr(dg), L.ptr(db)
    a.grad_beta, a.workspace = grad_beta, L.ptr(ws)
    a.rows, a.cols, a.x_dtype, a.dtype = rows, cols, L.dt(x2), L.dt(dy2)
    a.dropout_out, a.dropout_in = _d(drop_out), _d(drop_in)
    a.dbias_in = L.ptr(dbias_in)
    a.defer_fold = 1 if defer else 0
    L.check(L.lib().hero_layernorm_bwd(C.byref(a), L.stream()))
    if defer:
        for k, dst in enumerate((dg, db, dbias_in)):
            if dst is not None:
                _colsum_queue(ws, L.ptr(ws) + 4 * k * cols, dst, ws.shape[0], cols, 3 * cols, L.F32)
    return dx, (dxd if dxd is not None else dx), dg, db


ATTN_SAVE_PROBS = False


def k_attn_fwd(qkv, mask_add, S, Lq, H, drop=None, want_probs=True, out=None, seq_off=None):
    D = H * 64
    ctx = out if out is not None else torch.empty((qkv.shape[0], D), dtype=qkv.dtype, device=qkv.device)
    probs = stats = None
    if want_probs:
        if not ATTN_SAVE_PROBS and L.lib().hero_attention_stats_ok(L.dt(qkv), Lq):
            stats = torch.empty((S * H * Lq * 2,), dtype=torch.float32, device=qkv.device)
        else:
            probs = torch.empty((S, H, Lq, Lq), dtype=torch.float32, device=qkv.device)
    a = L.Attn(L.ptr(qkv), L.ptr(mask_add), L.ptr(ctx), L.ptr(probs), None, None, S, Lq, H,
               1.0 / math.sqrt(64.0), L.dt(qkv), _d(drop), L.ptr(seq_off), L.ptr(stats))
    L.check(L.lib().hero_attention_fwd(C.byref(a), L.stream()))
    return ctx, (stats if stats is not None else probs)


def k_attn_bwd(qkv, saved, dctx, S, Lq, H, drop=None, out=None, seq_off=None, ctx=None, mask_add=None):
    dqkv = out if out is not None else torch.empty_like(qkv)
    is_stats = saved.dim() == 1
    a = L.Attn(L.ptr(qkv), L.ptr(mask_add) if is_stats else None, L.ptr(ctx), None if is_stats else L.ptr(saved), L.ptr(dctx),
               L.ptr(dqkv), S, Lq, H, 1.0 / math.sqrt(64.0), L.dt(qkv), _d(drop), L.ptr(seq_off), L.ptr(saved) if is_stats else None)
    L.check(L.lib().hero_attention_bwd(C.byref(a), L.stream()))
    return dqkv


_SLACK = {}


def k_gather_rows(a, b, idx, rows, cols, tail_rows=0):
    ref = a if a is not None else b
    if tail_rows > 0:
        base = torch.empty((rows + tail_rows, cols), dtype=ref.dtype, device=ref.device)
        _SLACK[base.untyped_storage().data_ptr()] = weakref.ref(base)
        if len(_SLACK) > 64:
            for k in [k for k, r in _SLACK.items() if r() is None]:
                del _SLACK[k]
        out = base[:rows]
    else:
        out = torch.empty((rows, cols), dtype=ref.dtype, device=ref.device)
    L.check(L.lib().hero_gather_rows(L.ptr(a), L.ptr(b), L.ptr(idx), L.ptr(out), rows, cols,
                                     L.dt(ref), L.stream()))
    return out


def k_scatter_add(src2, idx, dst_a, dst_b=None, skip=-1):
    rows, cols = src2.shape
    L.check(L.lib().hero_scatter_add_rows(L.ptr(src2), L.ptr(idx), L.ptr(dst_a), L.ptr(dst_b), rows,
                                          cols, L.dt(src2), L.dt(dst_a), skip, L.stream()))


def segment_order(idx, n_dst, skip=-1):
    def build():
        order = torch.empty(idx.numel(), dtype=torch.int32, device=idx.device)
        ws = torch.empty(max(L.lib().hero_segment_sort_workspace_bytes(idx.numel()) // 4, 1), dtype=torch.int32, device=idx.device)
        L.check(L.lib().hero_segment_sort(L.ptr(idx), idx.numel(), n_dst, skip, L.ptr(order), L.ptr(ws), L.stream()))
        return order
    return memo("seg_order", (idx,), build, (n_dst, skip))


def k_scatter_add_sorted(src2, idx, dst, skip=-1):
    rows, cols = src2.shape
    order = segment_order(idx, dst.shape[0], skip)
    ws = _workspace(L.lib().hero_scatter_add_sorted_workspace_bytes(rows, cols) // 4, src2.device, slot="scatter_sorted")
    L.check(L.lib().hero_scatter_add_sorted(L.ptr(src2), L.ptr(idx), L.ptr(order), L.ptr(dst), rows, cols, L.dt(src2), skip,
                                            L.ptr(ws), L.stream()))


def k_cast(x, dtype):
    if x.dtype == dtype:
        return x
    x = x.contiguous()
    y = torch.empty(x.shape, dtype=dtype, device=x.device)
    L.check(L.lib().hero_cast(L.ptr(x), L.ptr(y), x.numel(), L.dt(x), L.dt(y), L.stream()))
    return y


def k_act_bwd(dy, aux, act):
    dx = torch.empty_like(dy)
    fn = L.lib().hero_relu_bwd if act == L.ACT_RELU else L.lib().hero_gelu_bwd
    L.check(fn(L.ptr(dy), L.ptr(aux), L.ptr(dx), dy.numel(), L.dt(dy), L.stream()))
    return dx


def _as2d(x):
    if not x.is_contiguous():
        x = x.contiguous()
    return x.view(-1, x.shape[-1])


class _MemoEntry:
    __slots__ = ("tag", "extra", "sources", "out", "fn", "spec", "key", "seq")

    def __init__(self, tag, extra, sources, out, fn, spec, key, seq):
        self.tag, self.extra, self.sources, self.out, self.fn, self.spec, self.key, self.seq = \
            tag, extra, sources, out, fn, spec, key, seq


_MEMO = {}
_MEMO_SEQ = 0


def _memo_key(tag, extra, tensors):
    return (tag, extra) + tuple((t.data_ptr(), t._version, tuple(t.shape), t.dtype) for t in tensors)


def memo(tag, tensors, fn, extra=(), spec=None):
    global _MEMO_SEQ
    key = _memo_key(tag, extra, tensors)
    hit = _MEMO.get(key)
    if hit is not None:
        return hit.out
    if torch.cuda.is_available() and torch.cuda.is_current_stream_capturing():
        return fn()
    if len(_MEMO) > 512:
        _MEMO.clear()
    out = fn()
    if spec is not None and not (len(tensors) == 1 and tensors[0].dtype == torch.int64 and tensors[0].is_contiguous()
                                 and tensors[0].is_cuda and out.is_contiguous() and out.numel() == tensors[0].numel()):
        spec = None
    _MEMO[key] = _MemoEntry(tag, extra, tensors, out, fn, spec, key, _MEMO_SEQ)
    _MEMO_SEQ += 1
    return out


def reset_caches():
    global _MEMO_SEQ
    clear_weight_cache()
    _REFRESH.clear()
    _REFRESH_PINNED.clear()
    _MEMO.clear()
    _MEMO_SEQ = 0
    _WS.clear()
    _WPLANS.clear()
    _WPLANS_PINNED.clear()
    _SEQ_OFF.clear()
    _SLACK.clear()
    del _WQ[:]
    del _CQ[:]
    set_grad_sink(None)
    from .model.layers import BertEncoder
    BertEncoder._PLANS.clear()
    BertEncoder._STATIC_PLANS.clear()


def host_sortable_orders(batch):
    ids_of = {e.out.data_ptr(): e.sources[0].data_ptr() for e in _MEMO.values()
              if e.tag == "row_index" and e.spec is not None and e.spec[0] == L.DERIVE_I32}
    keys = {t.data_ptr(): k for k, t in batch.items() if torch.is_tensor(t) and t.dtype == torch.int64}
    found = []
    for e in sorted(_MEMO.values(), key=lambda e: e.seq):
        if e.tag != "seg_order" or len(e.sources) != 1:
            continue
        k = keys.get(ids_of.get(e.sources[0].data_ptr()))
        if k is not None and batch[k].numel() == e.out.numel():
            found.append((k, e.out, int(e.extra[1])))
    return found


def host_segment_order(ids, skip):
    v = np.asarray(ids, dtype=np.int64).reshape(-1)
    key = np.where((v < 0) | (v == skip), np.int64(1) << 40, v)
    return np.argsort(key, kind="stable").astype(np.int32)


def refresh_memo(sources=None, skip_outputs=()):
    skip_ids = {id(t) for t in skip_outputs}
    src = {t.data_ptr() for t in sources or ()}
    level_of = {}
    levels = []
    for e in sorted(_MEMO.values(), key=lambda e: e.seq):
        ptrs = [t.data_ptr() for t in e.sources]
        if id(e.out) in skip_ids or (sources is not None and not any(p in src or p in level_of for p in ptrs)):
            continue
        n = 1 + max([level_of.get(p, 0) for p in ptrs] + [0])
        if isinstance(e.out, torch.Tensor):
            level_of[e.out.data_ptr()] = n
        if n > len(levels):
            levels.append([])
        levels[n - 1].append(e)
    done = []
    for todo in levels:
        spec = [e for e in todo if e.spec is not None]
        built = [e for e in todo if e.spec is None]
        for i in range(0, len(spec), 16):
            part = [L.Derive(L.ptr(e.sources[0]), L.ptr(e.out), e.out.numel(), *e.spec) for e in spec[i:i + 16]]
            L.check(L.lib().hero_derive_multi((L.Derive * len(part))(*part), len(part), L.stream()))
        for e in built:
            new = e.fn()
            if isinstance(e.out, torch.Tensor):
                if new.shape != e.out.shape:
                    raise RuntimeError("refresh_memo: a derived tensor changed shape %s -> %s; the batch structure is "
                                       "different, not just its contents" % (tuple(e.out.shape), tuple(new.shape)))
                e.out.copy_(new)
        done += spec + built
    return done


def restamp_memo(entries):
    for e in entries:
        if _MEMO.get(e.key) is e:
            del _MEMO[e.key]
            e.key = _memo_key(e.tag, e.extra, e.sources)
            _MEMO[e.key] = e


def as_mask_add(mask, S, Lq):
    if mask is None:
        return None
    if mask.dim() == 4:
        if mask.shape[1] != 1 or mask.shape[2] != 1:
            raise NotImplementedError("hero_amd attention supports key masks of shape (S,1,1,L) only")
        return mask.reshape(S, Lq).to(torch.float32).contiguous()
    if mask.requires_grad:
        return ((1.0 - mask.reshape(S, Lq).to(torch.float32)) * -10000.0).contiguous()
    return memo("mask_add", (mask,), lambda: ((1.0 - mask.reshape(S, Lq).to(torch.float32)) * -10000.0).contiguous(),
                (S, Lq), spec=(L.DERIVE_MASK_ADD, 0, 0, 0))


class CastFn(torch.autograd.Function):
    @staticmethod
    def forward(ctx, x, dtype):
        ctx.src = x.dtype
        return k_cast(x, dtype)

    @staticmethod
    def backward(ctx, dy):
        return k_cast(dy.contiguous(), ctx.src), None


def cast(x, dtype):
    return x if x.dtype == dtype else CastFn.apply(x, dtype)


class LinearFn(torch.autograd.Function):

    @staticmethod
    def forward(ctx, x, weight, bias, act, residual):
        x2 = _as2d(x)
        Wc = packed((weight,), x2.dtype)
        aux = torch.empty((x2.shape[0], Wc.shape[0]), dtype=x2.dtype, device=x2.device) \
            if act != L.ACT_NONE else None
        r2 = _as2d(residual) if residual is not None else None
        y = k_linear(x2, Wc, bias.detach() if bias is not None else None, act=act, aux=aux,
                     residual=r2)
        ctx.act = act
        ctx.has_res = residual is not None
        ctx.xshape = x.shape
        ctx.params = (weight, bias)
        ctx.sink = _is_param(weight) and (bias is None or _is_param(bias))
        if ctx.sink:
            _use(weight, bias)
        Wt = packed_t((weight,), x2.dtype) if ctx.needs_input_grad[0] else None
        ctx.save_for_backward(x2, Wt, aux)
        return y.view(*x.shape[:-1], Wc.shape[0])

    @staticmethod
    def backward(ctx, dy):
        x2, Wt, aux = ctx.saved_tensors
        weight, bias = ctx.params
        dy2 = _as2d(dy)
        dz = dy2 if ctx.act == L.ACT_NONE else k_act_bwd(dy2, aux, ctx.act)
        dx = k_dgrad_t(dz, Wt).view(ctx.xshape) if ctx.needs_input_grad[0] else None
        dW = db = None
        if ctx.sink:
            acc_linear_grads(dz, x2, weight, bias)
        else:
            dW = k_wgrad(dz, x2) if ctx.needs_input_grad[1] else None
            db = k_colsum(dz) if (bias is not None and ctx.needs_input_grad[2]) else None
        return dx, dW, db, None, (dy if ctx.has_res else None)


def linear(x, weight, bias=None, act=L.ACT_NONE, residual=None):
    if x.dtype == torch.bfloat16 and weight.shape[0] % 8 != 0:
        x = cast(x, torch.float32)
        residual = cast(residual, torch.float32) if residual is not None else None
    return LinearFn.apply(x, weight, bias, act, residual)


class MatmulNTFn(torch.autograd.Function):

    @staticmethod
    def forward(ctx, a, b):
        a2, b2 = a.contiguous(), b.contiguous()
        ctx.save_for_backward(a2, b2)
        return k_linear(a2, b2)

    @staticmethod
    def backward(ctx, dy):
        a2, b2 = ctx.saved_tensors
        dy2 = dy.contiguous()
        da = k_dgrad(dy2, b2) if ctx.needs_input_grad[0] else None
        db = k_wgrad(dy2, a2).to(b2.dtype) if ctx.needs_input_grad[1] else None
        return da, db


def matmul_nt(a, b):
    return MatmulNTFn.apply(a, b)


class CrossEntropyFn(torch.autograd.Function):

    @staticmethod
    def forward(ctx, logits, labels, ncols, ignore_index, inv_temp):
        x2 = logits.contiguous()
        rows, ld = x2.shape
        lab = labels.contiguous().to(torch.int64)
        loss = torch.empty((rows,), dtype=torch.float32, device=x2.device)
        lse = torch.empty((rows,), dtype=torch.float32, device=x2.device)
        a = L.CrossEntropy(L.ptr(x2), L.ptr(lab), L.ptr(loss), L.ptr(lse), None, None, rows, ncols, ld, L.dt(x2),
                           inv_temp, ignore_index)
        L.check(L.lib().hero_cross_entropy_fwd(C.byref(a), L.stream()))
        ctx.save_for_backward(x2, lab, lse)
        ctx.meta = (ncols, ignore_index, inv_temp)
        return loss

    @staticmethod
    def backward(ctx, dloss):
        x2, lab, lse = ctx.saved_tensors
        ncols, ignore_index, inv_temp = ctx.meta
        rows, ld = x2.shape
        g = dloss.contiguous().float()
        dx = torch.empty_like(x2)
        a = L.CrossEntropy(L.ptr(x2), L.ptr(lab), None, L.ptr(lse), L.ptr(g), L.ptr(dx), rows, ncols, ld, L.dt(x2),
                           inv_temp, ignore_index)
        L.check(L.lib().hero_cross_entropy_bwd(C.byref(a), L.stream()))
        return dx, None, None, None, None


def cross_entropy(logits, labels, ncols=None, ignore_index=-100, inv_temp=1.0):
    return CrossEntropyFn.apply(logits, labels, logits.shape[1] if ncols is None else ncols, ignore_index,
                                float(inv_temp))


class EmbedLnFn(torch.autograd.Function):

    @staticmethod
    def forward(ctx, x, gamma, beta, eps, drop, out_dtype, skip_idx, idxs, *tables):
        x2 = _as2d(x) if x is not None else None
        cols = gamma.shape[0]
        rows = x2.shape[0] if x2 is not None else idxs[0].numel()
        tabs = [t.detach()[i:i + 1] if isinstance(i, int) else t.detach()
                for t, i in zip(tables, tuple(idxs) + (None,) * len(tables))]
        y, mean, rstd, pre = k_ln_fwd(x2, gamma.detach(), beta.detach(), eps, out_dtype, rows, cols,
                                      tabs=tabs, idxs=[None if isinstance(i, int) else i for i in idxs],
                                      want_pre=len(tables) > 0, drop=drop, device=gamma.device)
        ctx.drop, ctx.idxs, ctx.skip = drop, idxs, skip_idx
        ctx.tables = tables
        ctx.ln = (gamma, beta)
        ctx.ln_sink = _is_param(gamma) and _is_param(beta)
        _use(*[t for t in tables if _is_param(t)])
        if ctx.ln_sink:
            _use(gamma, beta)
        ctx.has_x = x is not None
        ctx.xshape = x.shape if x is not None else None
        ctx.save_for_backward(pre if pre is not None else x2, gamma.detach(), mean, rstd)
        return y

    @staticmethod
    def backward(ctx, dy):
        pre, gamma, mean, rstd = ctx.saved_tensors
        dy2 = _as2d(dy)
        gp, bp = ctx.ln
        want_dx = (ctx.has_x and ctx.needs_input_grad[0]) or len(ctx.tables) > 0
        if ctx.ln_sink:
            dgd, dbd = ln_param_dsts(gp, bp)
            dx, _, _, _ = k_ln_bwd(pre, dy2, gamma, mean, rstd, want_dx=want_dx, drop_out=ctx.drop,
                                   dgamma=dgd, dbeta=dbd, grad_beta=1.0, want_params=False)
            ln_params_done(gp, bp)
            dg = db = None
        else:
            dx, _, dg, db = k_ln_bwd(pre, dy2, gamma, mean, rstd, want_dx=want_dx, drop_out=ctx.drop)
        grads_t = []
        for k, tab in enumerate(ctx.tables):
            idx = ctx.idxs[k] if k < len(ctx.idxs) else None
            skip = ctx.skip[k] if ctx.skip else -1
            row, idx = (idx, None) if isinstance(idx, int) else (0, idx)
            if _is_param(tab):
                per = getattr(idx, "_hero_period", 0) if idx is not None else 0
                if idx is None:
                    k_colsum(dx, out=SINK.dst(tab).view(-1, tab.shape[-1])[row], beta=1.0, on_done=lambda tab=tab: SINK.done(tab))
                    grads_t.append(None)
                    continue
                elif per and dx.shape[0] % per == 0 and dx.shape[0] // per >= 8:
                    D_ = dx.shape[1]
                    if (skip is None or skip < 0) and dx.is_contiguous() and (per * D_) % 4 == 0 and _colsum_defer_ok():
                        _colsum_queue(dx, L.ptr(dx), SINK.dst(tab), dx.shape[0] // per, per * D_, per * D_, L.dt(dx),
                                      on_done=lambda tab=tab: SINK.done(tab), dst_rows=idx[:per].contiguous(), row_cols=D_)
                        grads_t.append(None)
                        continue
                    folded = k_colsum(dx.view(dx.shape[0] // per, per * dx.shape[1]))
                    k_scatter_add(folded.view(per, dx.shape[1]), idx[:per], SINK.dst(tab), None, skip)
                elif (idx.dtype == torch.int32 and idx.is_contiguous() and dx.shape[1] % 4 == 0
                        and dx.shape[0] <= (1 << 17)):
                    k_scatter_add_sorted(dx, idx.view(-1), SINK.dst(tab).view(-1, tab.shape[-1]), skip)
                else:
                    k_scatter_add(dx, idx, SINK.dst(tab), None, skip)
                SINK.done(tab)
                grads_t.append(None)
            elif not ctx.needs_input_grad[8 + k]:
                grads_t.append(None)
            else:
                g = torch.zeros(tab.shape, dtype=torch.float32, device=dy.device)
                if idx is None:
                    k_colsum(dx, out=g.view(-1, tab.shape[-1])[row])
                else:
                    k_scatter_add(dx, idx, g, None, skip)
                grads_t.append(g)
        gx = dx.view(ctx.xshape) if (ctx.has_x and ctx.needs_input_grad[0]) else None
        return (gx, dg, db, None, None, None, None, None) + tuple(grads_t)


def embed_ln(x, gamma, beta, eps, drop, out_dtype, tables=(), idxs=(), skip_idx=None):
    return EmbedLnFn.apply(x, gamma, beta, eps, drop, out_dtype, skip_idx, tuple(idxs), *tables)


def _stack_in_place(blocks, rows, cols):
    first = blocks[0]
    total = sum(rows)
    ref = _SLACK.get(first.untyped_storage().data_ptr()) if first.is_cuda else None
    base = ref() if ref is not None else None
    if not (base is not None and first.is_contiguous() and first.dim() == 2 and first.storage_offset() == 0
            and base.dtype == first.dtype and base.shape[1] == cols and first.shape[0] == rows[0] and base.shape[0] >= total):
        return None
    full = base[:total]
    r0 = rows[0]
    for blk, n in zip(blocks[1:], rows[1:]):
        full[r0:r0 + n].copy_(blk.reshape(n, cols))
        r0 += n
    return full


class StackRowsFn(torch.autograd.Function):

    @staticmethod
    def forward(ctx, *xs):
        ctx.rows = [x.shape[0] for x in xs]
        full = _stack_in_place(xs, ctx.rows, xs[0].shape[1]) if all(x.dtype == xs[0].dtype for x in xs) else None
        return full if full is not None else torch.cat(xs, 0)

    @staticmethod
    def backward(ctx, dy):
        out, r0 = [], 0
        for i, n in enumerate(ctx.rows):
            out.append(dy[r0:r0 + n] if ctx.needs_input_grad[i] else None)
            r0 += n
        return tuple(out)


class SplitRowsFn(torch.autograd.Function):

    @staticmethod
    def forward(ctx, x, *sizes):
        ctx.sizes, ctx.meta = sizes, (x.shape[1], x.dtype, x.device)
        outs, r0 = [], 0
        for n in sizes:
            outs.append(x[r0:r0 + n])
            r0 += n
        return tuple(outs)

    @staticmethod
    def backward(ctx, *grads):
        cols, dtype, dev = ctx.meta
        parts = [g.reshape(n, cols) if g is not None else torch.zeros((n, cols), dtype=dtype, device=dev)
                 for g, n in zip(grads, ctx.sizes)]
        full = _stack_in_place(parts, list(ctx.sizes), cols) if all(p_.dtype == dtype for p_ in parts) else None
        return (full if full is not None else torch.cat(parts, 0),) + (None,) * len(ctx.sizes)


class _FirstRefCheck:
    __slots__ = ("flag", "event", "value")

    def __init__(self, flag, event):
        self.flag, self.event, self.value = flag, event, None

    def ok(self):
        if self.value is None:
            self.event.synchronize()
            self.value = int(self.flag[0]) == 0
        return self.value


def first_reference_map(idx, valid, na, nb):
    n = idx.numel()
    if (valid is None or valid.numel() != n or na + nb > 38400 or idx.dtype != torch.int32 or not idx.is_contiguous()
            or not idx.is_cuda):
        return None

    def build():
        inv = torch.empty(na + nb, dtype=torch.int32, device=idx.device)
        L.check(L.lib().hero_inverse_first(L.ptr(idx), n, L.ptr(inv), na, nb, L.stream()))
        return inv
    inv = memo("gather_inverse", (idx, valid), build, (na, nb))
    chk = getattr(inv, "_hero_first_check", None)
    if chk is None:
        if torch.cuda.is_current_stream_capturing():
            return None
        i64 = idx.to(torch.int64)
        src = torch.where(i64 >= 0, i64, na - i64 - 2).clamp_(0, na + nb - 1)
        pos = torch.arange(n, device=idx.device, dtype=torch.int32)
        later = (inv[src] != pos) & (idx != -1) & (valid.reshape(-1) != 0)
        flag = torch.empty(1, dtype=torch.int32).pin_memory()
        flag.copy_(later.any().to(torch.int32).reshape(1), non_blocking=True)
        ev = torch.cuda.Event()
        ev.record()
        chk = inv._hero_first_check = _FirstRefCheck(flag, ev)
    return inv, chk


class GatherRowsFn(torch.autograd.Function):

    @staticmethod
    def forward(ctx, a, b, idx, tail_rows=0, valid=None):
        a2, b2 = _as2d(a), (_as2d(b) if b is not None else None)
        ctx.save_for_backward(idx)
        ctx.ashape, ctx.bshape = a.shape, (b.shape if b is not None else None)
        na, nb = a2.shape[0], (b2.shape[0] if b2 is not None else 0)
        ctx.first = first_reference_map(idx, valid, na, nb) if valid is not None else None
        return k_gather_rows(a2, b2, idx, idx.numel(), a2.shape[1], tail_rows=tail_rows)

    @staticmethod
    def backward(ctx, dy):
        (idx,) = ctx.saved_tensors
        dy2 = _as2d(dy)
        if ctx.first is not None and ctx.first[1].ok():
            inv = ctx.first[0]
            na = inv.numel() if ctx.bshape is None else ctx.ashape.numel() // ctx.ashape[-1]
            both = k_gather_rows(dy2.contiguous(), None, inv, inv.numel(), dy2.shape[1])
            return both[:na].view(ctx.ashape), (both[na:].view(ctx.bshape) if ctx.bshape is not None else None), None, None, None
        da = torch.zeros(ctx.ashape, dtype=dy.dtype, device=dy.device)
        db = torch.zeros(ctx.bshape, dtype=dy.dtype, device=dy.device) if ctx.bshape is not None else None
        k_scatter_add(dy2, idx, da, db)
        return da, db, None, None, None


class PermuteRowsFn(torch.autograd.Function):

    @staticmethod
    def forward(ctx, a, idx, inv):
        a2 = _as2d(a)
        ctx.save_for_backward(inv)
        ctx.ashape = a.shape
        return k_gather_rows(a2, None, idx, idx.numel(), a2.shape[1])

    @staticmethod
    def backward(ctx, dy):
        (inv,) = ctx.saved_tensors
        dy2 = _as2d(dy)
        return k_gather_rows(dy2, None, inv, inv.numel(), dy2.shape[1]).view(ctx.ashape), None, None


class CsrGatherSumFn(torch.autograd.Function):

    @staticmethod
    def forward(ctx, src, offsets, entries, inverse, n_out):
        s2 = _as2d(src)
        out = torch.empty((n_out, s2.shape[1]), dtype=s2.dtype, device=s2.device)
        L.check(L.lib().hero_csr_gather_sum(L.ptr(s2), L.ptr(offsets), L.ptr(entries), L.ptr(out),
                                            n_out, s2.shape[1], L.dt(s2), L.stream()))
        ctx.save_for_backward(inverse)
        ctx.sshape = src.shape
        ctx.tail = int(getattr(src, "_hero_tail_rows", 0))
        return out

    @staticmethod
    def backward(ctx, dy):
        (inverse,) = ctx.saved_tensors
        dy2 = _as2d(dy)
        ds = k_gather_rows(dy2, None, inverse, inverse.numel(), dy2.shape[1], tail_rows=ctx.tail)
        return ds.view(ctx.sshape), None, None, None, None


class ExpandRowsFn(torch.autograd.Function):

    @staticmethod
    def forward(ctx, x, idx):
        x2 = x.reshape(x.shape[0], -1).contiguous()
        n = x2.shape[0]

        def i32():
            return idx.reshape(-1).to(torch.int32).contiguous()

        def csr():
            srt, order = torch.sort(idx.reshape(-1), stable=True)
            off = torch.searchsorted(srt, torch.arange(n + 1, device=idx.device, dtype=srt.dtype))
            return torch.cat([off.to(torch.int32), order.to(torch.int32)])
        i = memo("expand_idx", (idx,), i32, spec=(L.DERIVE_I32, 0, 0, 0))
        ctx.csr = memo("expand_csr", (idx,), csr, (n,))
        ctx.meta = (x.shape, n)
        out = k_gather_rows(x2, None, i, i.numel(), x2.shape[1])
        return out.view((i.numel(),) + tuple(x.shape[1:]))

    @staticmethod
    def backward(ctx, dy):
        shape, n = ctx.meta
        d2 = dy.reshape(dy.shape[0], -1).contiguous()
        out = torch.empty((n, d2.shape[1]), dtype=d2.dtype, device=d2.device)
        L.check(L.lib().hero_csr_gather_sum(L.ptr(d2), L.ptr(ctx.csr[:n + 1]), L.ptr(ctx.csr[n + 1:]), L.ptr(out), n, d2.shape[1],
                                            L.dt(d2), L.stream()))
        return out.view(shape), None


def _qkv_bwd(dqkv, x2, qkv_params, D):
    wq, bq, wk, bk, wv, bv = qkv_params
    ws, bs = (wq, wk, wv), (bq, bk, bv)
    gw = SINK.dst_group(ws) if all(p.requires_grad for p in ws) else None
    gb = SINK.dst_group(bs) if all(p.requires_grad for p in bs) else None
    if gw is not None:
        k_wgrad(dqkv, x2, out=gw, beta=1.0, on_done=lambda: [SINK.done(p) for p in ws],
                dbias=gb.view(-1) if gb is not None else None, dbias_done=lambda: [SINK.done(p) for p in bs])
    elif gb is not None:
        k_colsum(dqkv, out=gb.view(-1), beta=1.0, on_done=lambda: [SINK.done(p) for p in bs])
    for i, (w, b) in enumerate(zip(ws, bs)):
        acc_linear_grads(dqkv, x2, None if gw is not None else w, None if gb is not None else b, col0=i * D,
                         ncols=D)


class SelfAttentionFn(torch.autograd.Function):

    @staticmethod
    def forward(ctx, x, mask_add, H, drop_p, wq, bq, wk, bk, wv, bv):
        S, Lq, D = x.shape
        x2 = _as2d(x)
        Wqkv = packed((wq, wk, wv), x2.dtype)
        bqkv = packed((bq, bk, bv), torch.float32)
        qkv = k_linear(x2, Wqkv, bqkv)
        ctxt, probs = k_attn_fwd(qkv, mask_add, S, Lq, H, drop=drop_p)
        ctx.dims, ctx.drop, ctx.mask_add = (S, Lq, H, D), drop_p, mask_add
        ctx.params = (wq, bq, wk, bk, wv, bv)
        _use(*ctx.params)
        ctx.save_for_backward(x2, packed_t((wq, wk, wv), x2.dtype), qkv, probs, ctxt)
        return ctxt.view(S, Lq, D)

    @staticmethod
    def backward(ctx, dctx):
        x2, Wqkv_t, qkv, probs, ctxt = ctx.saved_tensors
        S, Lq, H, D = ctx.dims
        dqkv = k_attn_bwd(qkv, probs, _as2d(dctx), S, Lq, H, drop=ctx.drop, ctx=ctxt, mask_add=ctx.mask_add)
        dx = k_dgrad_t(dqkv, Wqkv_t).view(S, Lq, D) if ctx.needs_input_grad[0] else None
        _qkv_bwd(dqkv, x2, ctx.params, D)
        return (dx,) + (None,) * 9


class ProjResLnFn(torch.autograd.Function):

    @staticmethod
    def forward(ctx, h, res, eps, drop, w, b, gamma, beta):
        h2, r2 = _as2d(h), _as2d(res)
        Wc = packed((w,), h2.dtype)
        y = k_linear(h2, Wc, b.detach(), residual=r2, drop=drop)
        out, mean, rstd, _ = k_ln_fwd(y, gamma.detach(), beta.detach(), eps, y.dtype, y.shape[0], y.shape[1])
        ctx.drop = drop
        ctx.hshape, ctx.rshape = h.shape, res.shape
        ctx.params = (w, b, gamma, beta)
        _use(*ctx.params)
        ctx.save_for_backward(h2, packed_t((w,), h2.dtype), y, mean, rstd, gamma.detach())
        return out.view(res.shape)

    @staticmethod
    def backward(ctx, dout):
        h2, Wt, y, mean, rstd, gamma = ctx.saved_tensors
        w, b, gp, bp = ctx.params
        dgd, dbd = ln_param_dsts(gp, bp)
        fuse_b = b.requires_grad and y.shape[1] <= 1024
        dy, dyd, _, _ = k_ln_bwd(y, _as2d(dout), gamma, mean, rstd, drop_in=ctx.drop, dgamma=dgd,
                                 dbeta=dbd, grad_beta=1.0, want_params=False,
                                 dbias_in=SINK.dst(b) if fuse_b else None)
        ln_params_done(gp, bp)
        if fuse_b:
            SINK.done(b)
        acc_linear_grads(dyd, h2, w, None if fuse_b else b)
        dh = k_dgrad_t(dyd, Wt).view(ctx.hshape)
        return (dh, dy.view(ctx.rshape)) + (None,) * 6


ONE_ATTN_LAUNCH = [True]
_SEQ_OFF = {}


def _one_attention_launch(segs, masks, drops, x2):
    if not (ONE_ATTN_LAUNCH[0] and len(segs) > 1 and all(len(sg) == 2 for sg in segs) and x2.dtype == torch.bfloat16 and x2.is_cuda):
        return segs, masks, drops
    lmax = max(sg[1] for sg in segs)
    if ATTN_SAVE_PROBS or not L.lib().hero_attention_stats_ok(L.BF16, lmax) or any(m is not None and m.requires_grad for m in masks):
        return segs, masks, drops
    key = (tuple(segs), x2.device.index)
    off = _SEQ_OFF.get(key)
    if off is None:
        o, r = [0], 0
        for S_, L_ in segs:
            for _ in range(S_):
                r += L_
                o.append(r)
        off = _SEQ_OFF[key] = torch.tensor(o, dtype=torch.int32, device=x2.device)
    if all(m is None for m in masks):
        mcat = None
    else:
        def build():
            parts = []
            for (S_, L_), m in zip(segs, masks):
                mm = m.reshape(S_, L_).float() if m is not None else torch.zeros((S_, L_), dtype=torch.float32, device=x2.device)
                parts.append(torch.nn.functional.pad(mm, (0, lmax - L_)) if L_ < lmax else mm)
            return torch.cat(parts, 0).contiguous()
        mcat = memo("attn_mask_cat", tuple(m for m in masks if m is not None), build, (tuple(segs),))
    return (("packed", sum(sg[0] for sg in segs), lmax, off),), (mcat,), (drops[0],)


class AttnBlockFn(torch.autograd.Function):

    @staticmethod
    def forward(ctx, x, segs, masks, H, eps, drops_attn, drop_hid, wq, bq, wk, bk, wv, bv, wo, bo, g1, b1):
        x2 = _as2d(x)
        D = x2.shape[1]
        Wqkv = packed((wq, wk, wv), x2.dtype)
        bqkv = packed((bq, bk, bv), torch.float32)
        Wo = packed((wo,), x2.dtype)
        qkv = k_linear(x2, Wqkv, bqkv)
        ctxt = torch.empty((x2.shape[0], D), dtype=x2.dtype, device=x2.device)
        segs, masks, drops_attn = _one_attention_launch(segs, masks, drops_attn, x2)
        probs = []
        r0 = 0
        for seg, m, dr in zip(segs, masks, drops_attn):
            if len(seg) == 4:
                _, S, Lq, off = seg
                _, p = k_attn_fwd(qkv, m, S, Lq, H, drop=dr, out=ctxt, seq_off=off)
                probs.append(p)
                continue
            S, Lq = seg
            _, p = k_attn_fwd(qkv[r0:r0 + S * Lq], m, S, Lq, H, drop=dr, out=ctxt[r0:r0 + S * Lq])
            probs.append(p)
            r0 += S * Lq
        y1 = k_linear(ctxt, Wo, bo.detach(), residual=x2, drop=drop_hid)
        a, mean, rstd, _ = k_ln_fwd(y1, g1.detach(), b1.detach(), eps, y1.dtype, x2.shape[0], D)
        ctx.meta = (segs, H, D, drops_attn, drop_hid, x.shape)
        ctx.masks = masks
        ctx.params = (wq, bq, wk, bk, wv, bv, wo, bo, g1, b1)
        _use(*ctx.params)
        ctx.save_for_backward(x2, packed_t((wq, wk, wv), x2.dtype), packed_t((wo,), x2.dtype), qkv, ctxt, y1,
                              mean, rstd, g1.detach(), *probs)
        return a.view(x.shape)

    @staticmethod
    def backward(ctx, da):
        x2, Wqkv_t, Wo_t, qkv, ctxt, y1, mean, rstd, g1 = ctx.saved_tensors[:9]
        probs = ctx.saved_tensors[9:]
        segs, H, D, drops_attn, drop_hid, xshape = ctx.meta
        wq, bq, wk, bk, wv, bv, wo, bo, g1p, b1p = ctx.params
        dgd, dbd = ln_param_dsts(g1p, b1p)
        fuse_b = bo.requires_grad and D <= 1024
        dy1, dy1d, _, _ = k_ln_bwd(y1, _as2d(da), g1, mean, rstd, drop_in=drop_hid, dgamma=dgd,
                                   dbeta=dbd, grad_beta=1.0, want_params=False,
                                   dbias_in=SINK.dst(bo) if fuse_b else None)
        ln_params_done(g1p, b1p)
        if fuse_b:
            SINK.done(bo)
        acc_linear_grads(dy1d, ctxt, wo, None if fuse_b else bo)
        dctx = k_dgrad_t(dy1d, Wo_t)
        dqkv = torch.empty_like(qkv)
        r0 = 0
        for seg, p, dr, m in zip(segs, probs, drops_attn, ctx.masks):
            if len(seg) == 4:
                _, S, Lq, off = seg
                k_attn_bwd(qkv, p, dctx, S, Lq, H, drop=dr, out=dqkv, seq_off=off, ctx=ctxt, mask_add=m)
                continue
            S, Lq = seg
            k_attn_bwd(qkv[r0:r0 + S * Lq], p, dctx[r0:r0 + S * Lq], S, Lq, H, drop=dr,
                       out=dqkv[r0:r0 + S * Lq], ctx=ctxt[r0:r0 + S * Lq], mask_add=m)
            r0 += S * Lq
        _qkv_bwd(dqkv, x2, (wq, bq, wk, bk, wv, bv), D)
        dx = k_dgrad_t(dqkv, Wqkv_t, residual=dy1).view(xshape)
        return (dx,) + (None,) * 16


class FfnBlockFn(torch.autograd.Function):

    @staticmethod
    def forward(ctx, a, eps, drop_hid, w1, b1, w2, b2, g2, bt2):
        shp = a.shape
        a2 = _as2d(a)
        W1, W2 = packed((w1,), a2.dtype), packed((w2,), a2.dtype)
        u = torch.empty((a2.shape[0], W1.shape[0]), dtype=a2.dtype, device=a2.device)
        hg = k_linear(a2, W1, b1.detach(), act=L.ACT_GELU_DG, aux=u)
        y2 = k_linear(hg, W2, b2.detach(), residual=a2, drop=drop_hid)
        out, mean, rstd, _ = k_ln_fwd(y2, g2.detach(), bt2.detach(), eps, y2.dtype, y2.shape[0], y2.shape[1])
        ctx.drop, ctx.shp = drop_hid, shp
        ctx.params = (w1, b1, w2, b2, g2, bt2)
        _use(*ctx.params)
        ctx.save_for_backward(a2, packed_t((w1,), a2.dtype), packed_t((w2,), a2.dtype), u, hg, y2, mean,
                              rstd, g2.detach())
        return out.view(shp)

    @staticmethod
    def backward(ctx, dout):
        a2, W1_t, W2_t, u, hg, y2, mean, rstd, g2 = ctx.saved_tensors
        w1, b1, w2, b2, g2p, bt2p = ctx.params
        dgd, dbd = ln_param_dsts(g2p, bt2p)
        fuse_b = b2.requires_grad and y2.shape[1] <= 1024
        dy2, dy2d, _, _ = k_ln_bwd(y2, _as2d(dout), g2, mean, rstd, drop_in=ctx.drop, dgamma=dgd,
                                   dbeta=dbd, grad_beta=1.0, want_params=False,
                                   dbias_in=SINK.dst(b2) if fuse_b else None)
        ln_params_done(g2p, bt2p)
        if fuse_b:
            SINK.done(b2)
        acc_linear_grads(dy2d, hg, w2, None if fuse_b else b2)
        part = None
        if b1.requires_grad and B1_PARTIALS[0] and dy2d.dtype == torch.bfloat16:
            part = torch.empty((-(-dy2d.shape[0] // 64), W2_t.shape[0]), dtype=torch.float32, device=dy2d.device)
        fuse_b1 = part is None and b1.requires_grad and (SINK.wants_overlap() or not GROUP_WGRADS[0] or B1_EPILOGUE[0])
        du = k_dgrad_t(dy2d, W2_t, act=L.ACT_MUL_AUX, aux=u,
                       colsum=part if part is not None else (SINK.dst(b1) if fuse_b1 else None), colsum_partial=part is not None)
        if part is not None:
            k_colsum(part, out=SINK.dst(b1), beta=1.0, on_done=lambda: SINK.done(b1))
        acc_linear_grads(du, a2, w1, None if (fuse_b1 or part is not None) else b1)
        if fuse_b1:
            SINK.done(b1)
        da = k_dgrad_t(du, W1_t, residual=dy2).view(ctx.shp)
        return (da,) + (None,) * 8
```

### hero_amd/optim/adamw.py

```python
import ctypes as C

import numpy as np
import torch
from torch.optim import Optimizer

from .. import _lib as L
from .. import functional as HF


class AdamW(Optimizer):
    def __init__(self, params, lr=1e-3, betas=(0.9, 0.999), eps=1e-6, weight_decay=0.0,
                 correct_bias=True):
        if lr < 0.0 or eps < 0.0 or not (0.0 <= betas[0] < 1.0) or not (0.0 <= betas[1] < 1.0):
            raise ValueError("invalid AdamW hyper-parameters")
        if not correct_bias:
            raise NotImplementedError("correct_bias=False is not used by HERO")
        super().__init__(params, dict(lr=lr, betas=betas, eps=eps, weight_decay=weight_decay,
                                      correct_bias=correct_bias))
        if len(self.param_groups) > 8:
            raise ValueError("hero_amd AdamW supports up to 8 parameter groups")
        self._global_step = 0
        self._tables = {}
        self._pinned = []
        self._tsteps = None
        self._slots = None
        self.last_active = []

    def load_state_dict(self, state_dict):
        super().load_state_dict(state_dict)
        self._tables = {}
        self._tsteps = None

    def __setstate__(self, state):
        super().__setstate__(state)
        self._tables, self._pinned = {}, []
        self._tsteps = self._slots = None

    def grad_sumsq(self, flat=None):
        dev = next(p for g in self.param_groups for p in g["params"]).device
        out = torch.zeros(1, dtype=torch.float32, device=dev)
        if getattr(self, "_sumsq_ws", None) is None or self._sumsq_ws.device != dev:
            self._sumsq_ws = torch.empty(2048, dtype=torch.float32, device=dev)
        ws = self._sumsq_ws
        if flat is not None:
            L.check(L.lib().hero_sumsq(L.ptr(flat), flat.numel(), L.ptr(out), L.ptr(ws), L.stream()))
            return out
        for g in self.param_groups:
            for p in g["params"]:
                if p.grad is not None:
                    gr = p.grad if p.grad.is_contiguous() else p.grad.contiguous()
                    L.check(L.lib().hero_sumsq(L.ptr(gr), gr.numel(), L.ptr(out), L.ptr(ws), L.stream()))
        return out

    def _device_steps(self, dev):
        if self._tsteps is None:
            params = [p for g in self.param_groups for p in g["params"]]
            self._slots = {p: i for i, p in enumerate(params)}
            host = [int(self.state[p].get("step", 0)) if p in self.state else 0 for p in params]
            self._tsteps = torch.tensor(host, dtype=torch.int32, device=dev)
        return self._tsteps

    def sync_steps_from_device(self):
        if self._tsteps is None:
            return
        host = self._tsteps.cpu().tolist()
        for p, i in self._slots.items():
            if p in self.state and "step" in self.state[p]:
                self.state[p]["step"] = host[i]
        self._global_step = max([self._global_step] + host)

    def _build_table(self, active, slots=False):
        chunk = L.lib().hero_adamw_multi_chunk()
        descs = (L.TensorDesc * len(active))()
        ct, ci = [], []
        for i, (gi, p) in enumerate(active):
            st = self.state[p]
            g = p.grad
            if not (p.is_contiguous() and g.is_contiguous()):
                raise RuntimeError("hero_amd AdamW needs contiguous parameters and gradients")
            descs[i] = L.TensorDesc(L.ptr(p), L.ptr(g), L.ptr(st["exp_avg"]), L.ptr(st["exp_avg_sq"]),
                                    p.numel(), gi, self._slots[p] if slots else self._global_step - st["step"])
            n = -(-p.numel() // chunk)
            ct.extend([i] * n)
            ci.extend(range(n))
        dev = active[0][1].device
        raw = torch.frombuffer(bytearray(bytes(descs)), dtype=torch.uint8).to(dev)
        t_ct = torch.from_numpy(np.asarray(ct, dtype=np.int32)).to(dev)
        t_ci = torch.from_numpy(np.asarray(ci, dtype=np.int32)).to(dev)
        return raw, t_ct, t_ci, len(ct)

    @torch.no_grad()
    def step(self, closure=None, grad_sumsq=None, max_grad_norm=0.0, grad_scale=1.0, skip=None,
             step_tensor=None, lr_tensor=None):
        loss = closure() if closure is not None else None
        device_state = step_tensor is not None
        if not device_state:
            if self._tsteps is not None:
                self.sync_steps_from_device()
                self._tsteps = None
            self._global_step += 1
        active = []
        for gi, group in enumerate(self.param_groups):
            for p in group["params"]:
                if p.grad is None or (skip is not None and p in skip):
                    continue
                st = self.state[p]
                if not st:
                    st["step"] = 0
                    st["exp_avg"] = torch.zeros_like(p, memory_format=torch.contiguous_format)
                    st["exp_avg_sq"] = torch.zeros_like(p, memory_format=torch.contiguous_format)
                if not device_state:
                    st["step"] += 1
                active.append((gi, p))
        if not active:
            return loss
        tsteps = self._device_steps(active[0][1].device) if device_state else None
        self.last_active = active
        sig = self._table_for(active, device_state)
        raw, t_ct, t_ci, n_chunks = self._tables[sig]
        return self._launch(raw, t_ct, t_ci, n_chunks, len(active), tsteps, grad_sumsq, max_grad_norm, grad_scale, step_tensor, lr_tensor, loss)

    def prebuild(self, active, device_state=True):
        if active:
            self._device_steps(active[0][1].device)
            self._table_for(list(active), device_state)

    def _table_for(self, active, device_state):
        if device_state:
            sig = ("dev",) + tuple((id(p), p.data_ptr(), p.grad.data_ptr(), self.state[p]["exp_avg"].data_ptr(),
                                    self.state[p]["exp_avg_sq"].data_ptr(), self._slots[p]) for _, p in active)
        else:
            sig = tuple((id(p), p.data_ptr(), p.grad.data_ptr(), self.state[p]["exp_avg"].data_ptr(),
                         self.state[p]["exp_avg_sq"].data_ptr(), self._global_step - self.state[p]["step"]) for _, p in active)
        capturing = torch.cuda.is_current_stream_capturing()
        if sig not in self._tables:
            if len(self._tables) >= 16 and not capturing:
                self._tables = {}
            self._tables[sig] = self._build_table(active, slots=device_state)
        if capturing and not any(t is self._tables[sig] for t in self._pinned):
            self._pinned.append(self._tables[sig])
        return sig

    def _launch(self, raw, t_ct, t_ci, n_chunks, n_active, tsteps, grad_sumsq, max_grad_norm, grad_scale, step_tensor, lr_tensor, loss):
        a = L.AdamWMulti()
        a.descs, a.chunk_tensor, a.chunk_index, a.n_chunks = raw.data_ptr(), t_ct.data_ptr(), t_ci.data_ptr(), n_chunks
        for gi, group in enumerate(self.param_groups):
            b1, b2 = group["betas"]
            a.groups[gi] = L.AdamWGroup(group["lr"], b1, b2, group["eps"], group["weight_decay"])
        a.step = max(self._global_step, 1)
        a.step_ptr, a.lr_ptr = L.ptr(step_tensor), L.ptr(lr_tensor)
        a.tensor_steps, a.n_tensors = L.ptr(tsteps), n_active
        a.grad_sumsq = L.ptr(grad_sumsq)
        a.max_grad_norm, a.grad_scale = max_grad_norm, grad_scale
        L.check(L.lib().hero_adamw_multi(C.byref(a), L.stream()))
        HF.notify_weights_updated()
        return loss
```

### hero_amd/step.py

```python
import os
from types import SimpleNamespace

import torch

from . import functional as HF
from .optim import build_optimizer, get_lr_sched
from .utils import distributed as D

TVR_OPTS = dict(
    learning_rate=1e-4, lr_mul=1.0, weight_decay=0.01, optim="adamw", betas=[0.9, 0.98],
    grad_norm=1.0, warmup_steps=500, num_train_steps=5000, gradient_accumulation_steps=2,
    train_batch_size=32, dropout=0.1, lw_neg_q=8.0, lw_neg_ctx=8.0, lw_st_ed=0.01, margin=0.1)
TVQA_OPTS = dict(
    learning_rate=5e-5, lr_mul=10.0, weight_decay=0.01, optim="adamw", betas=[0.9, 0.98],
    grad_norm=1.0, warmup_steps=1000, num_train_steps=10000, gradient_accumulation_steps=2,
    train_batch_size=4, dropout=0.1, lw_st_ed=0.4)
QA_TASKS = ("tvqa", "how2qa")


def qkv_groups(model):
    from .model.layers import BertSelfAttention
    groups = []
    for m in model.modules():
        if isinstance(m, BertSelfAttention):
            groups.append((m.query.weight, m.key.weight, m.value.weight))
            groups.append((m.query.bias, m.key.bias, m.value.bias))
    return groups


class _packing:

    def __init__(self, mode):
        self.mode = mode

    def __enter__(self):
        from .model.layers import BertEncoder
        self.prev, BertEncoder.packing_mode = BertEncoder.packing_mode, self.mode

    def __exit__(self, *exc):
        from .model.layers import BertEncoder
        BertEncoder.packing_mode = self.prev


def _packing_mode_of(batch):
    if not hasattr(batch, "get") or not batch.get("_static_buffers"):
        return "all"
    return "static" if batch.get("_static_plan") else "none"


class TrainStep:
    def __init__(self, model, opts=None, task="tvr", bucket_bytes=64 << 20, use_graph=False, static_usage=False,
                 grad_compress="bf16", uniform_shapes=False, graph_collectives=None):
        self.model = model
        self.opts = SimpleNamespace(**{**TVR_OPTS, **(opts or {})})
        self.task = task
        self.optimizer = build_optimizer(model, self.opts)
        if task in QA_TASKS:
            head = {id(p) for n, p in model.named_parameters() if p.requires_grad and "v_encoder" not in n}
            if {id(p) for g in self.optimizer.param_groups[:2] for p in g["params"]} != head:
                raise RuntimeError("TrainStep: build_optimizer no longer puts the task head's parameters in groups 0 and 1")
        self.arena = D.GradArena(list(model.parameters()), bucket_bytes=bucket_bytes,
                                 groups=qkv_groups(model), static_usage=static_usage,
                                 compress=grad_compress if D.collectives_active() else None)
        self.micro = 0
        self.global_step = 0
        D.broadcast_tensors([p.data for p in model.parameters()], 0)
        self.uniform_shapes = bool(uniform_shapes)
        if graph_collectives is None:
            graph_collectives = os.environ.get("HERO_DP_GRAPH", "0") not in ("", "0")
        self.use_graph = use_graph and (not D.collectives_active() or (graph_collectives and uniform_shapes))
        self.counts = {"replayed": 0, "eager_in_graph_mode": 0, "captures": 0}
        self._graphs = {}
        self._window = []
        model.register_load_state_dict_post_hook(lambda *_: HF.notify_weights_updated())
        dev = next(model.parameters()).device
        self._step_t = torch.zeros(1, dtype=torch.int32, device=dev)
        self._lr_t = torch.zeros(8, dtype=torch.float32, device=dev)

    def enable_graph(self, collectives=False):
        if D.collectives_active() and not (collectives and self.uniform_shapes):
            raise RuntimeError("graph replay of a data-parallel step needs collectives=True and uniform_shapes=True")
        if self.micro % self.opts.gradient_accumulation_steps != 0:
            raise RuntimeError("switch to graph replay on an accumulation boundary")
        self.use_graph = True

    def _fwd_bwd(self, batch, task=None):
        HF.advance_seed()
        HF.RNG.site = 0
        with _packing(_packing_mode_of(batch)), HF.weights_frozen(), D.uniform_shapes(self.uniform_shapes):
            out = self.model(batch, task=task or self.task, compute_loss=True)
            if (task or self.task) in QA_TASKS:
                loss = out[0] + self.opts.lw_st_ed * out[1]
            else:
                loss = (out[0] + out[1] + out[2]) if isinstance(out, (tuple, list)) else out
            if loss.dim() > 0:
                loss = loss.mean()
            loss.backward()
        return loss.detach()

    def _optimise(self, device_state):
        self.arena.finish()
        untouched = [p for p in self.arena.params if p not in self.arena.touched]
        sumsq = self.optimizer.grad_sumsq(self.arena.flat) if self.opts.grad_norm != -1 else None
        if device_state:
            self._step_t.add_(1)
        self.optimizer.step(grad_sumsq=sumsq, max_grad_norm=float(self.opts.grad_norm),
                            grad_scale=1.0 / D.world_size(), skip=set(untouched),
                            step_tensor=self._step_t if device_state else None,
                            lr_tensor=self._lr_t if device_state else None)
        HF.refresh_weight_cache()
        self.arena.zero()

    def _set_lr(self):
        self.global_step += 1
        lr = get_lr_sched(self.global_step, self.opts)
        for g in self.optimizer.param_groups:
            g["lr"] = lr
        if self.task in QA_TASKS:
            for g in self.optimizer.param_groups[:2]:
                g["lr"] = lr * self.opts.lr_mul
        return lr

    def _fill_lr(self, lr):
        self._lr_t.fill_(lr)
        if self.task in QA_TASKS and self.opts.lr_mul != 1.0:
            self._lr_t[:2].fill_(lr * self.opts.lr_mul)

    def micro_step(self, batch, task=None, eager=False):
        task = task or self.task
        if self.use_graph:
            if eager:
                return self._eager_step_in_graph_mode(batch, task)
            return self._graph_step(batch, task)
        accum = self.opts.gradient_accumulation_steps
        boundary = (self.micro + 1) % accum == 0
        self.arena.set_sync(boundary)
        loss = self._fwd_bwd(batch, task)
        self.micro += 1
        if boundary:
            self._set_lr()
            self._optimise(device_state=False)
        return loss

    def _capture(self, batch, task):
        if getattr(self.model, "drop_svmr_prob", 0) > 0 and getattr(self.model, "lw_st_ed", 0) != 0:
            raise RuntimeError("graph mode cannot capture a step whose loss terms are drawn per step on the host "
                               "(drop_svmr_prob > 0, model/pretrain.py:74-75): the branch taken at capture would be replayed "
                               "forever; run eagerly")
        accum = self.opts.gradient_accumulation_steps
        side = torch.cuda.Stream()
        side.wait_stream(torch.cuda.current_stream())
        with torch.cuda.stream(side):
            for i in range(2 * accum):
                self.arena.set_sync((i + 1) % accum == 0)
                self._fwd_bwd(batch, task)
                if (i + 1) % accum == 0:
                    lr = self._set_lr()
                    self._fill_lr(lr)
                    self._optimise(device_state=True)
        torch.cuda.current_stream().wait_stream(side)
        torch.cuda.synchronize()
        self.micro += 2 * accum
        self._record(batch, task)

    @staticmethod
    def _key(batch, task):
        bucket = batch.get("_bucket") if hasattr(batch, "get") else None
        return task if bucket is None else (task, bucket)

    def _eager_step_in_graph_mode(self, batch, task):
        accum = self.opts.gradient_accumulation_steps
        boundary = (self.micro + 1) % accum == 0
        self.counts["eager_in_graph_mode"] += 1
        self._window.append(task)
        if len(set(self._window)) > 1:
            raise RuntimeError("graph mode: one accumulation window mixes tasks %s" % sorted(set(self._window)))
        if boundary:
            self._window = []
        self.arena.set_sync(boundary)
        loss = self._fwd_bwd(batch, task)
        self.micro += 1
        if boundary:
            self._fill_lr(self._set_lr())
            self._optimise(device_state=True)
        return loss

    def _record(self, batch, task):
        ga, gb = torch.cuda.CUDAGraph(), torch.cuda.CUDAGraph()
        mode = dict(capture_error_mode="thread_local") if D.collectives_active() else {}
        self.arena.set_sync(False)
        with torch.cuda.graph(ga, **mode):
            loss_a = self._fwd_bwd(batch, task)
        self.arena.set_sync(True)
        with torch.cuda.graph(gb, pool=ga.pool(), **mode):
            loss_b = self._fwd_bwd(batch, task)
            self._optimise(device_state=True)
        key = self._key(batch, task)
        self.counts["captures"] += 1
        self._graphs[key] = (ga, loss_a, gb, loss_b, batch)
        self._graph_gen = getattr(self, "_graph_gen", {})
        self._graph_gen[key] = HF.weight_cache_generation()
        self._active_of = getattr(self, "_active_of", {})
        self._active_of[key] = list(getattr(self.optimizer, "last_active", []))

    def prepare(self, batch, task=None):
        task = task or self.task
        if self.use_graph:
            if self._key(batch, task) not in self._graphs:
                self._capture(batch, task)
        elif task not in getattr(self, "_prepared", set()):
            for _ in range(self.opts.gradient_accumulation_steps):
                self.micro_step(batch, task)
            self._prepared = getattr(self, "_prepared", set()) | {task}

    def _graph_step(self, batch, task):
        key = self._key(batch, task)
        if key not in self._graphs:
            if not any((k if isinstance(k, str) else k[0]) == task for k in self._graphs):
                self._capture(batch, task)
            else:
                seen = self.__dict__.setdefault("_seen_eager", set())
                if key in seen and self.micro % self.opts.gradient_accumulation_steps == 0:
                    torch.cuda.synchronize()
                    self._record(batch, task)
                else:
                    seen.add(key)
                    loss = self._eager_step_in_graph_mode(batch, task)
                    if self.micro % self.opts.gradient_accumulation_steps == 0:
                        torch.cuda.synchronize()
                        self._record(batch, task)
                    return loss
        accum = self.opts.gradient_accumulation_steps
        if self.micro % accum == 0 and self._graph_gen[key] != HF.weight_cache_generation():
            torch.cuda.synchronize()
            if hasattr(self.optimizer, "prebuild"):
                self.optimizer.prebuild(self._active_of.get(key, []))
            self._record(self._graphs[key][4], task)
        ga, loss_a, gb, loss_b, static_batch = self._graphs[key]
        if batch is not static_batch:
            raise RuntimeError("graph mode replays the captured batch buffers (and the index / mask tensors derived "
                               "from them at capture): copy new data of the SAME structure into them, or run eagerly")
        accum = self.opts.gradient_accumulation_steps
        boundary = (self.micro + 1) % accum == 0
        self._window.append(task)
        if len(set(self._window)) > 1:
            raise RuntimeError("graph mode: one accumulation window mixes tasks %s; the captured optimiser step only "
                               "updates the parameters of its own task" % sorted(set(self._window)))
        if boundary:
            self._window = []
        self.micro += 1
        self.counts["replayed"] += 1
        if boundary:
            self._fill_lr(self._set_lr())
            gb.replay()
            return loss_b
        ga.replay()
        return loss_a

    def _sync_optimizer_steps(self):
        self.optimizer.sync_steps_from_device()

    def state_dict(self):
        self._sync_optimizer_steps()
        return {"global_step": self.global_step, "micro": self.micro, "optimizer": self.optimizer.state_dict(),
                "optimizer_global_step": self.optimizer._global_step}

    def load_state_dict(self, sd):
        if self._graphs:
            raise RuntimeError("restore the training state before the first graph-mode step (captured graphs hold "
                               "the optimiser's device state)")
        self.optimizer.load_state_dict(sd["optimizer"])
        self.optimizer._global_step = sd["optimizer_global_step"]
        self.global_step, self.micro = sd["global_step"], sd["micro"]
        self._step_t.fill_(self.global_step)
        HF.notify_weights_updated()
```

### hero_amd/utils/distributed.py

```python
import os

import torch
import torch.distributed as dist

from .. import functional as HF


def _on():
    return dist.is_available() and dist.is_initialized()


def world_size():
    return dist.get_world_size() if _on() else 1


def rank():
    return dist.get_rank() if _on() else 0


_EXCHANGE = ["torch"]


def set_exchange(kind):
    if kind not in ("torch", "abi"):
        raise ValueError("set_exchange: 'torch' or 'abi'")
    if kind == "abi":
        from . import comm
        comm.communicator()
    _EXCHANGE[0] = kind


def exchange():
    return _EXCHANGE[0]


def _abi_on(t):
    return _EXCHANGE[0] == "abi" and t.is_cuda


def collectives_active():
    return _on() and (dist.get_world_size() > 1 or bool(os.environ.get("HERO_DP_FORCE_COLLECTIVES")))


def all_reduce_and_rescale_tensors(tensors, rescale_denom):
    tensors = list(tensors)
    if not tensors:
        return
    n = world_size()
    flat = torch.cat([t.reshape(-1) for t in tensors])
    if n > 1:
        dist.all_reduce(flat, op=dist.ReduceOp.SUM)
    flat.mul_(1.0 / (n * float(rescale_denom)))
    off = 0
    for t in tensors:
        k = t.numel()
        t.copy_(flat[off:off + k].view_as(t))
        off += k


def _broadcast(t, root):
    if _abi_on(t):
        from . import comm
        c = comm.communicator()
        c.fork()
        c.broadcast(t, root, stream=c.stream)
        c.join()
    else:
        dist.broadcast(t, src=root)


def broadcast_tensors(tensors, root_rank, buffer_size=10485760):
    if world_size() == 1:
        return
    bucket, filled = [], 0

    def flush():
        if not bucket:
            return
        flat = torch.cat([t.reshape(-1) for t in bucket])
        _broadcast(flat, root_rank)
        off = 0
        for t in bucket:
            t.copy_(flat[off:off + t.numel()].view_as(t))
            off += t.numel()

    for t in tensors:
        sz = t.numel() * t.element_size()
        if sz > buffer_size and t.is_contiguous():
            _broadcast(t, root_rank)
            continue
        if filled + sz > buffer_size:
            flush()
            bucket, filled = [], 0
        bucket.append(t)
        filled += sz
    flush()


class GradArena(HF.GradSink):

    def __init__(self, params, bucket_bytes=64 << 20, overlap=True, install=True, groups=(),
                 static_usage=False, compress=None, backend=None):
        self.params = [p for p in params if p.requires_grad]
        total = sum(p.numel() for p in self.params)
        dev = self.params[0].device
        self.flat = torch.zeros(total, dtype=torch.float32, device=dev)
        self.slices = {}
        self.buckets = []
        self.bucket_of = {}
        group_of = {}
        for g in groups:
            g = tuple(g)
            if all(q.requires_grad and q.numel() % 4 == 0 for q in g):
                for q in g:
                    group_of[q] = g
        off, start, count = 0, 0, 0
        for p in reversed(self.params):
            if p in self.slices:
                continue
            for q in group_of.get(p, (p,)):
                n = q.numel()
                pad = (-off) % 4
                off += pad
                self.slices[q] = (off, off + n)
                self.bucket_of[q] = len(self.buckets)
                off += n
                count += 1
            if (off - start) * 4 >= bucket_bytes:
                self.buckets.append([start, off, count])
                start, count = off, 0
        if count:
            self.buckets.append([start, off, count])
        if off > total:
            self.flat = torch.zeros(off, dtype=torch.float32, device=dev)
        for p in self.params:
            s, e = self.slices[p]
            p.grad = self.flat[s:e].view_as(p)
        self.sync = True
        self.overlap = overlap
        self.compress = compress
        if compress not in (None, "bf16"):
            raise ValueError("GradArena: compress must be None or 'bf16'")
        self._wire = {}
        if backend is None:
            backend = "abi" if _EXCHANGE[0] == "abi" and dev.type == "cuda" else "torch"
        if backend not in ("torch", "abi"):
            raise ValueError("GradArena: backend must be 'torch' or 'abi'")
        if backend == "abi" and dev.type != "cuda":
            raise ValueError("GradArena: backend 'abi' (hero_comm_* = RCCL) needs a CUDA arena")
        self.backend = backend
        self._comm = None
        self._abi_open = False
        if backend == "abi":
            self._abi()
        self.static_usage = static_usage
        self.mute = False
        self._expect = None
        self._pending = [b[2] for b in self.buckets]
        self._launched = [False] * len(self.buckets)
        self._final = set()
        self._uses = {}
        self._handles = []
        self.touched = set()
        for p in self.params:
            p.register_post_accumulate_grad_hook(self._autograd_hook)
        if install:
            HF.set_grad_sink(self)

    def dst(self, p):
        sl = self.slices.get(p)
        if sl is None:
            return super().dst(p)
        if p.grad is None or p.grad.data_ptr() != self.flat.data_ptr() + sl[0] * 4:
            p.grad = self.flat[sl[0]:sl[1]].view_as(p)
        return p.grad

    def dst_group(self, params):
        sl = [self.slices.get(p) for p in params]
        if any(x is None for x in sl) or any(sl[i][1] != sl[i + 1][0] for i in range(len(sl) - 1)):
            return None
        for p in params:
            self.dst(p)
        tail = params[0].shape[1:]
        if any(p.shape[1:] != tail for p in params):
            return None
        return self.flat[sl[0][0]:sl[-1][1]].view((-1,) + tuple(tail))

    def use(self, p):
        self._uses[p] = self._uses.get(p, 0) + 1

    def done(self, p):
        n = self._uses.get(p, 1) - 1
        self._uses[p] = n
        if n <= 0:
            self._on_final(p)

    def _autograd_hook(self, p):
        sl = self.slices[p]
        if p.grad.data_ptr() != self.flat.data_ptr() + sl[0] * 4:
            self.flat[sl[0]:sl[1]].add_(p.grad.reshape(-1))
            p.grad = self.flat[sl[0]:sl[1]].view_as(p)
        if self._uses.get(p, 0) > 0:
            return
        self._on_final(p)

    def _on_final(self, p):
        self.touched.add(p)
        if p in self._final or p not in self.bucket_of:
            return
        self._final.add(p)
        if not (self.sync and self.overlap) or not collectives_active() or self.mute:
            return
        b = self.bucket_of[p]
        if self._expect is not None and p not in self._expect:
            if self._launched[b]:
                raise RuntimeError("GradArena(static_usage=True): a parameter of shape %s received its first "
                                   "gradient after its bucket's all-reduce was issued; construct the arena "
                                   "with static_usage=False for steps that change the set of used "
                                   "parameters" % (tuple(p.shape),))
            self._expect = self._expect | {p}
            self._pending[b] = 1 << 30
            return
        self._pending[b] -= 1
        if self._pending[b] == 0:
            self._launch(b)

    def _launch(self, b):
        if self._launched[b]:
            return
        self._launched[b] = True
        s, e, _ = self.buckets[b]
        if self.backend == "abi":
            c = self._abi()
            buf = self.flat[s:e]
            if self.compress == "bf16":
                buf = self._wire.get(b)
                if buf is None:
                    buf = self._wire[b] = torch.empty(e - s, dtype=torch.bfloat16, device=self.flat.device)
                buf.copy_(self.flat[s:e])
            c.fork()
            c.allreduce_buckets([buf], stream=c.stream)
            self._abi_open = True
            self._handles.append((None, b if self.compress == "bf16" else None))
        elif self.compress == "bf16":
            w = self._wire.get(b)
            if w is None:
                w = self._wire[b] = torch.empty(e - s, dtype=torch.bfloat16, device=self.flat.device)
            w.copy_(self.flat[s:e])
            self._handles.append((dist.all_reduce(w, op=dist.ReduceOp.SUM, async_op=True), b))
        else:
            self._handles.append((dist.all_reduce(self.flat[s:e], op=dist.ReduceOp.SUM, async_op=True), None))

    def _abi(self):
        if self._comm is None:
            from . import comm
            self._comm = comm.communicator()
        return self._comm

    def set_sync(self, flag):
        self.sync = flag
        self._final.clear()
        self._uses.clear()

    def wants_overlap(self):
        return bool(self.sync) and collectives_active()

    def finish(self):
        if collectives_active() and self.sync and not self.mute:
            for b in range(len(self.buckets)):
                self._launch(b)
            if self._abi_open:
                self._comm.join()
                self._abi_open = False
            for h, b in self._handles:
                if h is not None:
                    h.wait()
                if b is not None:
                    s, e, _ = self.buckets[b]
                    self.flat[s:e].copy_(self._wire[b])
        self._handles = []
        if self.static_usage and self.touched:
            self._expect = frozenset(self.touched) | (self._expect or frozenset())
        if self._expect is not None:
            self._pending = [0] * len(self.buckets)
            for p in self._expect:
                self._pending[self.bucket_of[p]] += 1
        else:
            self._pending = [b[2] for b in self.buckets]
        self._launched = [False] * len(self.buckets)
        self._final.clear()
        self._uses.clear()

    def scale_(self, factor):
        self.flat.mul_(factor)

    def wire_bytes(self):
        per = 2 if self.compress == "bf16" else 4
        return sum((e - s) * per for s, e, _ in self.buckets)

    def probe_allreduce_ms(self, reps=3):
        if not collectives_active():
            return 0.0
        dt = torch.bfloat16 if self.compress == "bf16" else torch.float32
        bufs = [torch.zeros(e - s, dtype=dt, device=self.flat.device) for s, e, _ in self.buckets]
        times = []
        if self.backend == "abi":
            c = self._abi()
            for _ in range(reps + 1):
                torch.cuda.synchronize()
                e0, e1 = torch.cuda.Event(enable_timing=True), torch.cuda.Event(enable_timing=True)
                e0.record()
                c.fork()
                c.allreduce_buckets(bufs, stream=c.stream)
                c.join()
                e1.record()
                torch.cuda.synchronize()
                times.append(e0.elapsed_time(e1))
            return sorted(times[1:])[len(times[1:]) // 2]
        for _ in range(reps + 1):
            torch.cuda.synchronize()
            e0, e1 = torch.cuda.Event(enable_timing=True), torch.cuda.Event(enable_timing=True)
            e0.record()
            hs = [dist.all_reduce(b, op=dist.ReduceOp.SUM, async_op=True) for b in bufs]
            for h in hs:
                h.wait()
            e1.record()
            torch.cuda.synchronize()
            times.append(e0.elapsed_time(e1))
        return sorted(times[1:])[len(times[1:]) // 2]

    def zero(self):
        self.flat.zero_()
        self.touched.clear()
        for p in self.params:
            if p.grad is None:
                s, e = self.slices[p]
                p.grad = self.flat[s:e].view_as(p)


class _AllGatherRows(torch.autograd.Function):

    @staticmethod
    def forward(ctx, tensor, dims):
        r, n = rank(), world_size()
        ctx.offset, ctx.dim = sum(dims[:r]), tensor.shape[0]
        if _abi_on(tensor):
            from . import comm
            c = comm.communicator()
            send = tensor.contiguous()
            c.fork()
            out = c.allgather_var(send, dims, stream=c.stream)
            c.join()
            return out
        mx = max(dims)
        buf = tensor.new_zeros((mx,) + tuple(tensor.shape[1:]))
        buf[:tensor.shape[0]] = tensor
        out = [torch.empty_like(buf) for _ in range(n)]
        dist.all_gather(out, buf.contiguous())
        return torch.cat([o[:d] for o, d in zip(out, dims)], dim=0)

    @staticmethod
    def backward(ctx, grad):
        return grad.narrow(0, ctx.offset, ctx.dim), None


_HOST_GROUP = [None, None]


def _host_group():
    pg = dist.distributed_c10d._get_default_group()
    if _HOST_GROUP[0] is not pg:
        _HOST_GROUP[0] = pg
        if dist.get_backend() == "gloo":
            _HOST_GROUP[1] = None
        else:
            try:
                import os
                if os.environ.get("MASTER_ADDR", "") in ("127.0.0.1", "localhost"):
                    os.environ.setdefault("GLOO_SOCKET_IFNAME", "lo")
                _HOST_GROUP[1] = dist.new_group(backend="gloo")
            except Exception:
                _HOST_GROUP[1] = "device"
    return _HOST_GROUP[1]


UNIFORM_SHAPES = [False]


class uniform_shapes:

    def __init__(self, on):
        self.on = bool(on)

    def __enter__(self):
        self.prev, UNIFORM_SHAPES[0] = UNIFORM_SHAPES[0], self.on

    def __exit__(self, *exc):
        UNIFORM_SHAPES[0] = self.prev


def gather_negatives(query, context, context_mask, return_own=False):
    n = world_size()
    if UNIFORM_SHAPES[0]:
        metas = [[query.shape[0], context.shape[0], context.shape[1]]] * n
    else:
        hg = _host_group()
        meta = torch.tensor([query.shape[0], context.shape[0], context.shape[1]], dtype=torch.int64,
                            device=query.device if hg == "device" else "cpu")
        metas = [torch.empty_like(meta) for _ in range(n)]
        dist.all_gather(metas, meta, group=None if hg == "device" else hg)
        metas = torch.stack(metas).tolist()
    nq = [m[0] for m in metas]
    nv = [m[1] for m in metas]
    max_len = max(m[2] for m in metas)
    pad = max_len - context.shape[1]
    if pad:
        context = torch.cat([context, context.new_zeros(context.shape[0], pad, context.shape[2])], 1)
        context_mask = torch.cat([context_mask, context_mask.new_zeros(context_mask.shape[0], pad)], 1)
    q = _AllGatherRows.apply(query.contiguous(), nq)
    c = _AllGatherRows.apply(context.contiguous(), nv)
    m = _AllGatherRows.apply(context_mask.contiguous(), nv)
    if return_own:
        return q, c, m, (sum(nv[:rank()]), nv[rank()])
    return q, c, m


def all_gather_list(data):
    if world_size() == 1:
        return [data]
    out = [None] * world_size()
    dist.all_gather_object(out, data)
    return out


def any_broadcast(data, root_rank):
    if world_size() == 1:
        return data
    box = [data if rank() == root_rank else None]
    dist.broadcast_object_list(box, src=root_rank)
    return box[0]


__all__ = ["all_reduce_and_rescale_tensors", "broadcast_tensors", "GradArena", "gather_negatives",
           "all_gather_list", "any_broadcast", "world_size", "rank", "collectives_active"]
```

### include/hero_hip.h

```cpp
#ifndef HERO_HIP_H_
#define HERO_HIP_H_

#include <stddef.h>
#include <stdint.h>

#ifdef __cplusplus
extern "C" {
#endif

typedef void* hero_stream_t;

enum { HERO_F32 = 0, HERO_BF16 = 1 };
enum { HERO_OK = 0, HERO_ERR_ARG = -1, HERO_ERR_LAUNCH = -2, HERO_ERR_UNSUPPORTED = -3 };

const char* hero_last_error(void);
#define HERO_ABI_VERSION 3
int hero_abi_version(void);
enum { HERO_STRUCT_DROPOUT = 0, HERO_STRUCT_GEMM_EPILOGUE, HERO_STRUCT_WGRAD_PROBLEM, HERO_STRUCT_LN_FWD, HERO_STRUCT_LN_BWD,
       HERO_STRUCT_COLSUM, HERO_STRUCT_ATTN, HERO_STRUCT_ADAMW, HERO_STRUCT_TENSOR_DESC, HERO_STRUCT_ADAMW_GROUP,
       HERO_STRUCT_ADAMW_MULTI, HERO_STRUCT_COPY_DESC, HERO_STRUCT_QUERY_POOL, HERO_STRUCT_ROW_NORM, HERO_STRUCT_SCORE_MAX,
       HERO_STRUCT_RANK_LOSS, HERO_STRUCT_ST_ED, HERO_STRUCT_CROSS_ENTROPY, HERO_STRUCT_DERIVE, HERO_STRUCT_COMM_BUCKET,
       HERO_STRUCT_COUNT_ };
int hero_abi_struct_count(void);
int hero_abi_struct_bytes(int which);

typedef struct HeroDropout {
  const uint64_t* seed_ptr;
  uint64_t site;
  uint32_t threshold16;
  float scale;
} HeroDropout;

enum { HERO_LAYOUT_K = 0,
       HERO_LAYOUT_O = 1   };
enum { HERO_ACT_NONE = 0,
       HERO_ACT_GELU = 1,
       HERO_ACT_RELU = 2,
       HERO_ACT_GELU_BWD = 3,
       HERO_ACT_RELU_BWD = 4,
       HERO_ACT_GELU_DG = 5,
       HERO_ACT_MUL_AUX = 6    };

typedef struct HeroGemmEpilogue {
  const float* bias;
  const void* residual;
  void* aux;
  int act;
  int out_f32;
  float beta;
  int split_k;
  HeroDropout dropout;
  float* colsum;
  int colsum_partial;
  int pad_;
  long long split_stride;
} HeroGemmEpilogue;

int hero_gemm(const void* A, const void* B, void* C, int M, int N, int K, int lda, int ldb, int ldc,
              int a_layout, int b_layout, int dtype, const HeroGemmEpilogue* epi, hero_stream_t stream);
int hero_gemm_splits(int K, int split_k, int dtype);
int hero_fold_slabs(const float* slabs, int n_slabs, size_t stride, void* out, size_t n, int out_dtype, hero_stream_t stream);

typedef struct HeroWgradProblem {
  const void* dy;
  const void* x;
  float* dw;
  int M, N, ld_dy, ld_x, ld_dw;
  int split_hint;
  float* dbias;
} HeroWgradProblem;
int hero_wgrad_group(const HeroWgradProblem* probs, int n, int K, int dtype, hero_stream_t stream);
#define HERO_WGRAD_BATCH_MAX 32
int hero_wgrad_batch_plan(const HeroWgradProblem* probs, int n, int K, int32_t* plan, int capacity_words);
int hero_wgrad_batch(const HeroWgradProblem* probs, int n, int K, int dtype, const int32_t* plan_dev, int plan_words,
                     hero_stream_t stream);
int hero_gemm_force_config(int cfg);
int hero_prof_enable(int on);
int hero_prof_read(int slot, double* total_ms, double* total_flops, long long* launches);

int hero_probe_mfma(void* scratch, size_t scratch_bytes, double* tflops, double* ghz, hero_stream_t stream);
int hero_probe_hbm(const void* src, void* dst, size_t bytes, double* copy_gbps, double* read_gbps, hero_stream_t stream);

typedef struct HeroLnFwd {
  const void* x;
  const float* tab[3];
  const int32_t* idx[3];
  const float* gamma;
  const float* beta;
  void* y;
  void* pre;
  float* mean;
  float* rstd;
  int rows, cols;
  float eps;
  int x_dtype, y_dtype;
  HeroDropout dropout;
} HeroLnFwd;
int hero_layernorm_fwd(const HeroLnFwd* a, hero_stream_t stream);

typedef struct HeroLnBwd {
  const void* x;
  const void* dy;
  const float* gamma;
  const float* mean;
  const float* rstd;
  void* dx;
  void* dx_dropped;
  float* dgamma;
  float* dbeta;
  float grad_beta;
  void* workspace;
  int rows, cols;
  int x_dtype, dtype;
  HeroDropout dropout_out;
  HeroDropout dropout_in;
  float* dbias_in;
  int defer_fold;
} HeroLnBwd;
size_t hero_layernorm_bwd_workspace_bytes(int rows, int cols);
int hero_layernorm_bwd_blocks(int rows);
int hero_layernorm_bwd(const HeroLnBwd* a, hero_stream_t stream);

size_t hero_colsum_workspace_bytes(int rows, int cols);
int hero_colsum(const void* x, float* out, int rows, int cols, int ld, int dtype, float beta,
                void* workspace, hero_stream_t stream);
#define HERO_COLSUM_MULTI_MAX 64
typedef struct HeroColsum {
  const void* src;
  float* dst;
  int rows, cols, ld, dtype;
  float beta;
  int row_cols;
  const int32_t* dst_rows;
} HeroColsum;
size_t hero_colsum_multi_workspace_bytes(const HeroColsum* p, int n);
int hero_colsum_multi(const HeroColsum* p, int n, void* workspace, hero_stream_t stream);

typedef struct HeroAttn {
  const void* qkv;
  const float* mask;
  void* ctx;
  float* probs;
  const void* dctx;
  void* dqkv;
  int S, L, H;
  float scale;
  int dtype;
  HeroDropout dropout;
  const int32_t* seq_off;
  float* stats;
} HeroAttn;
int hero_attention_fwd(const HeroAttn* a, hero_stream_t stream);
int hero_attention_bwd(const HeroAttn* a, hero_stream_t stream);
int hero_attention_max_len(int dtype, int backward);
int hero_attention_max_packed_len(int dtype);
int hero_attention_force_ppw(int ppw);
int hero_attention_stats_ok(int dtype, int L);

int hero_gather_rows(const void* a, const void* b, const int32_t* idx, void* out, int rows, int cols,
                     int dtype, hero_stream_t stream);
int hero_inverse_first(const int32_t* idx, int n, int32_t* inv, int na, int nb, hero_stream_t stream);
int hero_csr_gather_sum(const void* src, const int32_t* offsets, const int32_t* entries, void* out,
                        int rows, int cols, int dtype, hero_stream_t stream);
int hero_scatter_add_rows(const void* src, const int32_t* idx, void* dst_a, void* dst_b, int rows,
                          int cols, int src_dtype, int dst_dtype, int skip_idx, hero_stream_t stream);
size_t hero_segment_sort_workspace_bytes(int rows);
size_t hero_scatter_add_sorted_workspace_bytes(int rows, int cols);
int hero_segment_sort(const int32_t* idx, int rows, int n_dst, int skip_idx, int32_t* order, void* workspace,
                      hero_stream_t stream);
int hero_scatter_add_sorted(const void* src, const int32_t* idx, const int32_t* order, float* dst, int rows, int cols,
                            int src_dtype, int skip_idx, void* workspace, hero_stream_t stream);

int hero_cast(const void* src, void* dst, size_t n, int src_dtype, int dst_dtype, hero_stream_t stream);
int hero_transpose_cast(const float* src, void* dst, int rows, int cols, int ldd, int dst_dtype, hero_stream_t stream);
int hero_relu_bwd(const void* dy, const void* y, void* dx, size_t n, int dtype, hero_stream_t stream);
int hero_gelu_bwd(const void* dy, const void* u, void* dx, size_t n, int dtype, hero_stream_t stream);
int hero_add(const void* a, const void* b, void* y, size_t n, int dtype, hero_stream_t stream);

int hero_sumsq(const float* g, size_t n, float* sumsq, float* workspace, hero_stream_t stream);
typedef struct HeroAdamW {
  float* p;
  const float* g;
  float* m;
  float* v;
  size_t n;
  float lr, beta1, beta2, eps, weight_decay;
  int step;
  const float* grad_sumsq;
  float max_grad_norm;
  float grad_scale;
  void* shadow;
} HeroAdamW;
int hero_adamw(const HeroAdamW* a, hero_stream_t stream);

typedef struct HeroTensorDesc {
  float* p;
  const float* g;
  float* m;
  float* v;
  uint64_t n;
  int32_t group;
  int32_t step_lag;
} HeroTensorDesc;
typedef struct HeroAdamWGroup {
  float lr, beta1, beta2, eps, weight_decay;
} HeroAdamWGroup;
typedef struct HeroAdamWMulti {
  const HeroTensorDesc* descs;
  const int32_t* chunk_tensor;
  const int32_t* chunk_index;
  int n_chunks;
  HeroAdamWGroup groups[8];
  int step;
  const float* grad_sumsq;
  float max_grad_norm;
  float grad_scale;
  const int32_t* step_ptr;
  const float* lr_ptr;
  int32_t* tensor_steps;
  int n_tensors;
} HeroAdamWMulti;
int hero_adamw_multi(const HeroAdamWMulti* a, hero_stream_t stream);
int hero_adamw_multi_chunk(void);

typedef struct HeroCopyDesc {
  const float* src;
  void* dst;
  int32_t rows, cols, ldd;
  int32_t transpose;
  int32_t dst_dtype;
  int32_t pad_;
} HeroCopyDesc;
int hero_copy_multi(const HeroCopyDesc* descs, const int32_t* tile_desc, const int32_t* tile_index,
                    int n_tiles, hero_stream_t stream);

typedef struct HeroQueryPool {
  const void* q;
  const float* mask;
  const float* w;
  float* pooled;
  float* att;
  const float* dpooled;
  void* dq;
  float* dw;
  int B, L, D, dtype;
} HeroQueryPool;
int hero_query_pool_fwd(const HeroQueryPool* a, hero_stream_t stream);
int hero_query_pool_bwd(const HeroQueryPool* a, hero_stream_t stream);

int hero_qa_pool_fwd(const void* x, const float* mask, const float* w_qa, const float* w_se, float* qa_pooled, float* se_pooled,
                     float* att_qa, float* att_se, int Nv, int A, int L, int Lt, int D, int dtype, hero_stream_t stream);
int hero_qa_pool_bwd(const void* x, const float* mask, const float* w_qa, const float* w_se, const float* att_qa, const float* att_se,
                     const float* dqa, const float* dse, void* dx, float* dw_qa, float* dw_se,
                     int Nv, int A, int L, int Lt, int D, int dtype, hero_stream_t stream);

typedef struct HeroRowNorm {
  const void* x;
  float* y;
  float* rnorm;
  const float* dy;
  void* dx;
  int rows, cols, x_dtype;
  float eps;
} HeroRowNorm;
int hero_rownorm_fwd(const HeroRowNorm* a, hero_stream_t stream);
int hero_rownorm_bwd(const HeroRowNorm* a, hero_stream_t stream);

typedef struct HeroScoreMax {
  const float* s;
  const float* mask;
  float* out;
  int32_t* arg;
  const float* ds_ctx;
  const float* ds_q;
  const float* gc;
  const float* gq;
  const float* qn;
  const float* cn;
  float* dqn;
  float* dcn;
  int M, N, L, D, n0, n_own, ld_s;
  float gc_scale, gq_scale;
} HeroScoreMax;
int hero_sums_scaled(const float* src, int n_segs, int seg_len, const float* scales, float* out, hero_stream_t stream);
int hero_score_max_fwd(const HeroScoreMax* a, hero_stream_t stream);
int hero_score_max_bwd(const HeroScoreMax* a, hero_stream_t stream);

typedef struct HeroRankLoss {
  const float* s;
  float* loss_ctx_rows;
  float* loss_q_rows;
  float* ds_ctx;
  float* ds_q;
  int nq, nv;
  float margin;
  int lse;
  int hard;
  int pool;
  float hard_w, easy_w;
} HeroRankLoss;
int hero_rank_loss(const HeroRankLoss* a, hero_stream_t stream);

typedef struct HeroStEd {
  const float* q2;
  const void* ctx;
  const float* mask;
  const float* w_st;
  const float* w_ed;
  const int64_t* targets;
  float* loss_rows;
  float* p_st;
  float* p_ed;
  float* sim;
  const float* g;
  float* dq2;
  void* dctx;
  float* dw_st;
  float* dw_ed;
  int B, L, D, K, dtype;
  float g_scale;
  float* ws;
} HeroStEd;
size_t hero_st_ed_bwd_workspace_bytes(int B);
int hero_st_ed_fwd(const HeroStEd* a, hero_stream_t stream);
int hero_st_ed_bwd(const HeroStEd* a, hero_stream_t stream);

int hero_topk_rows(const float* scores, int M, int N, int ld, int k, float alpha, float* val, int* idx, hero_stream_t stream);
int hero_st_ed_probs(const float* sim, long long ld_sim, const float* mask, const int* sel, const float* w_st, const float* w_ed, int Nq,
                     int Nv, int K, int L, int taps, float* st_prob, float* ed_prob, hero_stream_t stream);
int hero_moment_topk(const float* st_prob, const float* ed_prob, const float* w, int Nq, int K, int L, int min_l, int max_l, int top_n,
                     float* score, int* flat, hero_stream_t stream);
int hero_moment_nms(const int* video, const int* st, const int* ed, int Nq, int N, double thd, int per_video_cap, int max_after, int* keep,
                    int* count, hero_stream_t stream);
int hero_first_hit(const int* video, const int* st, const int* ed, int Nq, int P, int ld, const int* gt_video, const float* gt_ts, float interval,
                   const float* thds, int T, int* first, hero_stream_t stream);

typedef struct HeroCrossEntropy {
  const void* logits;
  const int64_t* labels;
  float* loss;
  float* lse;
  const float* dloss;
  void* dlogits;
  int rows, cols, ld, dtype;
  float inv_temp;
  int64_t ignore_index;
} HeroCrossEntropy;
int hero_cross_entropy_fwd(const HeroCrossEntropy* a, hero_stream_t stream);
int hero_cross_entropy_bwd(const HeroCrossEntropy* a, hero_stream_t stream);

int hero_collate_subs(const int32_t* sub_nfrm, const int32_t* sub_ntok, int64_t* gather_index, int64_t* attn_mask, int T,
                      int max_vl, int out_size, hero_stream_t stream);
int hero_collate_gather_feats(const float* c_v_feats, float* f_v_feats, const int32_t* vid_sub_off, const int32_t* vid_nfrm,
                              const int32_t* sub_frm_off, const int32_t* sub_frm, int32_t* row_vid, int T, int max_vl, int B, int NF,
                              int D, hero_stream_t stream);
int hero_collate_clip_mask(const int32_t* vid_nfrm, int64_t* attn_mask, int B, int NF, hero_stream_t stream);
int hero_collate_frame_map(const int32_t* vid_sub_off, const int32_t* sub_frm_off, const int32_t* sub_frm, const int32_t* offsets,
                           int32_t* counts, int32_t* entries, int32_t* inverse, int B, int NF, int Lf, int fill,
                           hero_stream_t stream);

enum { HERO_DERIVE_MASK_ADD = 0, HERO_DERIVE_F32 = 1, HERO_DERIVE_I32 = 2, HERO_DERIVE_FLAT_GATHER = 3 };
#define HERO_DERIVE_MAX 16
typedef struct HeroDerive {
  const int64_t* src;
  void* dst;
  int64_t n;
  int mode;
  int p0, p1, p2;
} HeroDerive;
int hero_derive_multi(const HeroDerive* d, int n, hero_stream_t stream);

typedef struct HeroCommBucket {
  void* buf;
  size_t count;
  int dtype;
  int pad_;
} HeroCommBucket;
int hero_comm_available(void);
int hero_comm_unique_id(void* id128);
int hero_comm_init(const void* id128, int rank, int world, void** comm_out);
int hero_comm_destroy(void* comm);
int hero_comm_rank(void* comm);
int hero_comm_world(void* comm);
int hero_comm_allreduce_buckets(void* comm, const HeroCommBucket* buckets, int n, hero_stream_t stream);
int hero_comm_broadcast(void* comm, void* buf, size_t bytes, int root, hero_stream_t stream);
int hero_comm_allgather(void* comm, const void* send, void* recv, size_t bytes_per_rank, hero_stream_t stream);
int hero_comm_allgather_var(void* comm, const void* send, void* recv, const size_t* bytes_per_rank, hero_stream_t stream);

#ifdef __cplusplus
}
#endif
#endif
```

Before: 5352 videos/s.

## Fuse gradient zeroing and bf16 weight-copy refresh into the multi-tensor AdamW kernel

Adds a fused variant of the multi-tensor AdamW kernel that, in the same pass over each parameter, zeroes its gradient slice and writes the cached bf16 (and transposed) weight copies. Gradient slices of skipped or never-optimised parameters are cleared by the same launch. The separate arena-wide zero fill and the weight-cache refresh copy at the optimizer boundary are meant to be dropped, saving extra HBM passes over grads and weights every other micro-step. In exchange it adds table and signature bookkeeping, a shared-memory transpose path, and coupling between the optimizer and the weight cache that could go stale.

```diff
diff --git a/hero_amd/_lib.py b/hero_amd/_lib.py
--- a/hero_amd/_lib.py
+++ b/hero_amd/_lib.py
@@ -16,7 +16,7 @@
     "hero_layernorm_bwd_workspace_bytes", "hero_layernorm_bwd", "hero_colsum_workspace_bytes",
     "hero_colsum", "hero_colsum_multi", "hero_colsum_multi_workspace_bytes", "hero_layernorm_bwd_blocks", "hero_attention_fwd", "hero_attention_bwd", "hero_attention_max_len", "hero_attention_max_packed_len", "hero_attention_stats_ok", "hero_attention_force_ppw",
     "hero_gather_rows", "hero_inverse_first", "hero_csr_gather_sum", "hero_scatter_add_rows", "hero_segment_sort_workspace_bytes", "hero_scatter_add_sorted_workspace_bytes", "hero_segment_sort", "hero_scatter_add_sorted", "hero_cast", "hero_transpose_cast", "hero_copy_multi",
-    "hero_relu_bwd", "hero_gelu_bwd", "hero_add", "hero_sumsq", "hero_adamw", "hero_adamw_multi", "hero_adamw_multi_chunk",
+    "hero_relu_bwd", "hero_gelu_bwd", "hero_add", "hero_sumsq", "hero_adamw", "hero_adamw_multi", "hero_adamw_multi_chunk", "hero_adamw_multi_fused", "hero_adamw_multi_tiles",
     "hero_query_pool_fwd", "hero_query_pool_bwd", "hero_rownorm_fwd", "hero_rownorm_bwd", "hero_score_max_fwd",
     "hero_score_max_bwd", "hero_rank_loss", "hero_sums_scaled", "hero_st_ed_fwd", "hero_st_ed_bwd", "hero_st_ed_bwd_workspace_bytes",
     "hero_cross_entropy_fwd", "hero_cross_entropy_bwd", "hero_qa_pool_fwd", "hero_qa_pool_bwd",
@@ -244,6 +244,7 @@
         L.hero_sumsq.argtypes = [C.c_void_p, C.c_size_t, C.c_void_p, C.c_void_p, C.c_void_p]
         L.hero_adamw.argtypes = [C.POINTER(AdamW), C.c_void_p]
         L.hero_adamw_multi.argtypes = [C.POINTER(AdamWMulti), C.c_void_p]
+        L.hero_adamw_multi_fused.argtypes = [C.POINTER(AdamWMulti), C.c_void_p, C.c_int, C.c_void_p]
         L.hero_copy_multi.argtypes = [C.c_void_p, C.c_void_p, C.c_void_p, C.c_int, C.c_void_p]
         for fn, st in (("hero_query_pool_fwd", QueryPool), ("hero_query_pool_bwd", QueryPool),
                        ("hero_rownorm_fwd", RowNorm), ("hero_rownorm_bwd", RowNorm),
diff --git a/hero_amd/csrc/rows.hip b/hero_amd/csrc/rows.hip
--- a/hero_amd/csrc/rows.hip
+++ b/hero_amd/csrc/rows.hip
@@ -422,71 +422,165 @@
   if (threadIdx.x == 0) out[0] += (red[0] + red[1]) + (red[2] + red[3]);
 }
 
+struct AdamCoef { float gs, beta1, beta2, eps, step_size, decay; };
+__device__ __forceinline__ void adam_update(float& p, float g0, float& m, float& v, const AdamCoef& c) {
+  const float g = g0 * c.gs;
+  m = c.beta1 * m + (1.f - c.beta1) * g;
+  v = c.beta2 * v + (1.f - c.beta2) * g * g;
+  p -= c.step_size * m / (sqrtf(v) + c.eps);
+  p -= c.decay * p;
+}
+__device__ __forceinline__ void adam_update4(float4& p, const float4& g, float4& m, float4& v, const AdamCoef& c) {
+  adam_update(p.x, g.x, m.x, v.x, c); adam_update(p.y, g.y, m.y, v.y, c);
+  adam_update(p.z, g.z, m.z, v.z, c); adam_update(p.w, g.w, m.w, v.w, c);
+}
+__device__ __forceinline__ float clipped_scale(const float* grad_sumsq, float max_grad_norm, float grad_scale) {
+  float gs = grad_scale;
+  if (grad_sumsq) {
+    const float norm = sqrtf(*grad_sumsq) * fabsf(grad_scale);
+    const float clip = max_grad_norm / (norm + 1e-6f);
+    if (clip < 1.f) gs *= clip;
+  }
+  return gs;
+}
+__device__ __forceinline__ void copy_st1(void* dst, int dtype, size_t i, float x) {
+  if (dtype == HERO_BF16) static_cast<bf16_t*>(dst)[i] = f2bf(x);
+  else static_cast<float*>(dst)[i] = x;
+}
+__device__ __forceinline__ void copy_st4(void* dst, int dtype, size_t i, const float4& x) {
+  if (dtype == HERO_BF16) V4<bf16_t>::st(static_cast<bf16_t*>(dst) + i, x);
+  else *reinterpret_cast<float4*>(static_cast<float*>(dst) + i) = x;
+}
+
 __global__ void adamw_kernel(HeroAdamW a, float bc1, float bc2) {
-  float gs = a.grad_scale;
-  if (a.grad_sumsq) {
-    const float norm = sqrtf(*a.grad_sumsq) * fabsf(a.grad_scale);
-    const float clip = a.max_grad_norm / (norm + 1e-6f);
-    if (clip < 1.f) gs *= clip;
-  }
-  const float step_size = a.lr * sqrtf(bc2) / bc1;
-  const float decay = a.lr * a.weight_decay;
-  bf16_t* sh = static_cast<bf16_t*>(a.shadow);
+  const AdamCoef c = {clipped_scale(a.grad_sumsq, a.max_grad_norm, a.grad_scale), a.beta1, a.beta2, a.eps,
+                      a.lr * sqrtf(bc2) / bc1, a.lr * a.weight_decay};
   const size_t n4 = a.n >> 2;
   for (size_t q = blockIdx.x * (size_t)blockDim.x + threadIdx.x; q < n4; q += (size_t)gridDim.x * blockDim.x) {
     float4 p = *reinterpret_cast<float4*>(a.p + q * 4);
     const float4 g4 = *reinterpret_cast<const float4*>(a.g + q * 4);
     float4 m = *reinterpret_cast<float4*>(a.m + q * 4);
     float4 v = *reinterpret_cast<float4*>(a.v + q * 4);
-    float* pp = &p.x; const float* gp = &g4.x; float* mp = &m.x; float* vp = &v.x;
-#pragma unroll
-    for (int k = 0; k < 4; ++k) {
-      const float g = gp[k] * gs;
-      mp[k] = a.beta1 * mp[k] + (1.f - a.beta1) * g;
-      vp[k] = a.beta2 * vp[k] + (1.f - a.beta2) * g * g;
-      pp[k] -= step_size * mp[k] / (sqrtf(vp[k]) + a.eps);
-      pp[k] -= decay * pp[k];
-    }
+    adam_update4(p, g4, m, v, c);
     *reinterpret_cast<float4*>(a.p + q * 4) = p;
     *reinterpret_cast<float4*>(a.m + q * 4) = m;
     *reinterpret_cast<float4*>(a.v + q * 4) = v;
-    if (sh) V4<bf16_t>::st(sh + q * 4, p);
+    if (a.shadow) copy_st4(a.shadow, HERO_BF16, q * 4, p);
   }
   if (blockIdx.x == 0 && threadIdx.x < (a.n & 3)) {
     const size_t i = n4 * 4 + threadIdx.x;
-    const float g = a.g[i] * gs;
-    const float m = a.beta1 * a.m[i] + (1.f - a.beta1) * g;
-    const float v = a.beta2 * a.v[i] + (1.f - a.beta2) * g * g;
-    float p = a.p[i] - step_size * m / (sqrtf(v) + a.eps);
-    p -= decay * p;
+    float p = a.p[i], m = a.m[i], v = a.v[i];
+    adam_update(p, a.g[i], m, v, c);
     a.p[i] = p; a.m[i] = m; a.v[i] = v;
-    if (sh) sh[i] = f2bf(p);
+    if (a.shadow) copy_st1(a.shadow, HERO_BF16, i, p);
   }
 }
 
 constexpr int MT_CHUNK = 16384;
+constexpr int MT_TILES = MT_CHUNK / (64 * 64);
+struct AdamCopyDst {
+  void* w;
+  void* wt;
+  int32_t rows, cols;
+  int32_t ldt;
+  int32_t dtypes;
+};
 __global__ void adamw_steps_inc_kernel(const HeroTensorDesc* descs, int n, int32_t* steps) {
   const int i = blockIdx.x * blockDim.x + threadIdx.x;
-  if (i < n) steps[descs[i].step_lag] += 1;
-}
-__global__ __launch_bounds__(256) void adamw_multi_kernel(HeroAdamWMulti a) {
+  if (i < n && descs[i].p) steps[descs[i].step_lag] += 1;
+}
+template <bool FUSED>
+__global__ __launch_bounds__(256) void adamw_multi_kernel(HeroAdamWMulti a, const AdamCopyDst* __restrict__ copy_dst, int zero_grads) {
+  __shared__ float tile[FUSED ? 64 : 1][65];
   const int ti = a.chunk_tensor[blockIdx.x];
   const HeroTensorDesc d = a.descs[ti];
-  const HeroAdamWGroup gr = a.groups[d.group];
+  float* const dg = const_cast<float*>(d.g);
   const size_t beg = (size_t)a.chunk_index[blockIdx.x] * MT_CHUNK;
   const size_t end = beg + MT_CHUNK < d.n ? beg + MT_CHUNK : d.n;
-  float gs = a.grad_scale;
-  if (a.grad_sumsq) {
-    const float norm = sqrtf(*a.grad_sumsq) * fabsf(a.grad_scale);
-    const float clip = a.max_grad_norm / (norm + 1e-6f);
-    if (clip < 1.f) gs *= clip;
-  }
+  if (FUSED && !d.p) {
+    if (((uintptr_t)dg & 15) == 0) {
+      const size_t e4 = beg + ((end - beg) & ~(size_t)3);
+      for (size_t i = beg + threadIdx.x * 4; i < e4; i += 256 * 4) *reinterpret_cast<float4*>(dg + i) = make_float4(0.f, 0.f, 0.f, 0.f);
+      for (size_t i = e4 + threadIdx.x; i < end; i += 256) dg[i] = 0.f;
+    } else {
+      for (size_t i = beg + threadIdx.x; i < end; i += 256) dg[i] = 0.f;
+    }
+    return;
+  }
+  const HeroAdamWGroup gr = a.groups[d.group];
   const float st = a.tensor_steps ? (float)a.tensor_steps[d.step_lag] : (float)((a.step_ptr ? *a.step_ptr : a.step) - d.step_lag);
   const float lr = a.lr_ptr ? a.lr_ptr[d.group] : gr.lr;
   const float bc1 = 1.f - powf(gr.beta1, st), bc2 = 1.f - powf(gr.beta2, st);
-  const float step_size = lr * sqrtf(bc2) / bc1;
-  const float decay = lr * gr.weight_decay;
+  const AdamCoef c = {clipped_scale(a.grad_sumsq, a.max_grad_norm, a.grad_scale), gr.beta1, gr.beta2, gr.eps,
+                      lr * sqrtf(bc2) / bc1, lr * gr.weight_decay};
+  const bool zg = FUSED && zero_grads;
   const bool vec = (((uintptr_t)d.p | (uintptr_t)d.g | (uintptr_t)d.m | (uintptr_t)d.v) & 15) == 0;
+  AdamCopyDst cd = {nullptr, nullptr, 0, 0, 0, 0};
+  if (FUSED && copy_dst) cd = copy_dst[ti];
+  const int wdt = cd.dtypes & 0xff, wtdt = (cd.dtypes >> 8) & 0xff;
+  const bool wvec = ((uintptr_t)cd.w & 15) == 0;
+
+  if (FUSED && cd.wt) {
+    const int tcols = (cd.cols + 63) >> 6, ntiles = ((cd.rows + 63) >> 6) * tcols;
+    const int t0 = a.chunk_index[blockIdx.x] * MT_TILES;
+    const int t1 = t0 + MT_TILES < ntiles ? t0 + MT_TILES : ntiles;
+    const int q = threadIdx.x & 15, ty = threadIdx.x >> 4;
+    const bool vin = vec && (cd.cols & 3) == 0;
+    const bool vout = (cd.ldt & 3) == 0 && ((uintptr_t)cd.wt & 15) == 0 && (cd.rows & 3) == 0;
+    for (int t = t0; t < t1; ++t) {
+      const int r0 = (t / tcols) * 64, c0 = (t % tcols) * 64;
+#pragma unroll
+      for (int k = 0; k < 4; ++k) {
+        const int rl = ty + 16 * k, r = r0 + rl, cc = c0 + 4 * q;
+        float4 p = make_float4(0.f, 0.f, 0.f, 0.f);
+        if (r < cd.rows && cc < cd.cols) {
+          const size_t i = (size_t)r * cd.cols + cc;
+          if (vin) {
+            p = *reinterpret_cast<float4*>(d.p + i);
+            const float4 g4 = *reinterpret_cast<const float4*>(d.g + i);
+            float4 m = *reinterpret_cast<float4*>(d.m + i);
+            float4 v = *reinterpret_cast<float4*>(d.v + i);
+            adam_update4(p, g4, m, v, c);
+            *reinterpret_cast<float4*>(d.p + i) = p;
+            *reinterpret_cast<float4*>(d.m + i) = m;
+            *reinterpret_cast<float4*>(d.v + i) = v;
+            if (zg) *reinterpret_cast<float4*>(dg + i) = make_float4(0.f, 0.f, 0.f, 0.f);
+            if (cd.w) {
+              if (wvec) copy_st4(cd.w, wdt, i, p);
+              else { copy_st1(cd.w, wdt, i, p.x); copy_st1(cd.w, wdt, i + 1, p.y); copy_st1(cd.w, wdt, i + 2, p.z); copy_st1(cd.w, wdt, i + 3, p.w); }
+            }
+          } else {
+            float* pe = &p.x;
+            for (int e = 0; e < 4 && cc + e < cd.cols; ++e) {
+              float m = d.m[i + e], v = d.v[i + e];
+              pe[e] = d.p[i + e];
+              adam_update(pe[e], d.g[i + e], m, v, c);
+              d.p[i + e] = pe[e]; d.m[i + e] = m; d.v[i + e] = v;
+              if (zg) dg[i + e] = 0.f;
+              if (cd.w) copy_st1(cd.w, wdt, i + e, pe[e]);
+            }
+          }
+        }
+        tile[rl][4 * q] = p.x; tile[rl][4 * q + 1] = p.y; tile[rl][4 * q + 2] = p.z; tile[rl][4 * q + 3] = p.w;
+      }
+      __syncthreads();
+#pragma unroll
+      for (int k = 0; k < 4; ++k) {
+        const int cl = ty + 16 * k, cc = c0 + cl, r = r0 + 4 * q;
+        if (cc >= cd.cols || r >= cd.rows) continue;
+        const float4 o = make_float4(tile[4 * q][cl], tile[4 * q + 1][cl], tile[4 * q + 2][cl], tile[4 * q + 3][cl]);
+        const size_t j = (size_t)cc * cd.ldt + r;
+        if (vout) copy_st4(cd.wt, wtdt, j, o);
+        else {
+          const float e4[4] = {o.x, o.y, o.z, o.w};
+          for (int e = 0; e < 4 && r + e < cd.rows; ++e) copy_st1(cd.wt, wtdt, j + e, e4[e]);
+        }
+      }
+      __syncthreads();
+    }
+    return;
+  }
+
   if (vec) {
     const size_t e4 = beg + ((end - beg) & ~(size_t)3);
     for (size_t i = beg + threadIdx.x * 4; i < e4; i += 256 * 4) {
@@ -494,35 +588,30 @@
       const float4 g4 = *reinterpret_cast<const float4*>(d.g + i);
       float4 m = *reinterpret_cast<float4*>(d.m + i);
       float4 v = *reinterpret_cast<float4*>(d.v + i);
-      float* pp = &p.x; const float* gp = &g4.x; float* mp = &m.x; float* vp = &v.x;
-#pragma unroll
-      for (int k = 0; k < 4; ++k) {
-        const float g = gp[k] * gs;
-        mp[k] = gr.beta1 * mp[k] + (1.f - gr.beta1) * g;
-        vp[k] = gr.beta2 * vp[k] + (1.f - gr.beta2) * g * g;
-        pp[k] -= step_size * mp[k] / (sqrtf(vp[k]) + gr.eps);
-        pp[k] -= decay * pp[k];
-      }
+      adam_update4(p, g4, m, v, c);
       *reinterpret_cast<float4*>(d.p + i) = p;
       *reinterpret_cast<float4*>(d.m + i) = m;
       *reinterpret_cast<float4*>(d.v + i) = v;
+      if (zg) *reinterpret_cast<float4*>(dg + i) = make_float4(0.f, 0.f, 0.f, 0.f);
+      if (FUSED && cd.w) {
+        if (wvec) copy_st4(cd.w, wdt, i, p);
+        else { copy_st1(cd.w, wdt, i, p.x); copy_st1(cd.w, wdt, i + 1, p.y); copy_st1(cd.w, wdt, i + 2, p.z); copy_st1(cd.w, wdt, i + 3, p.w); }
+      }
     }
     for (size_t i = e4 + threadIdx.x; i < end; i += 256) {
-      const float g = d.g[i] * gs;
-      const float m = gr.beta1 * d.m[i] + (1.f - gr.beta1) * g;
-      const float v = gr.beta2 * d.v[i] + (1.f - gr.beta2) * g * g;
-      float p = d.p[i] - step_size * m / (sqrtf(v) + gr.eps);
-      p -= decay * p;
+      float p = d.p[i], m = d.m[i], v = d.v[i];
+      adam_update(p, d.g[i], m, v, c);
       d.p[i] = p; d.m[i] = m; d.v[i] = v;
+      if (zg) dg[i] = 0.f;
+      if (FUSED && cd.w) copy_st1(cd.w, wdt, i, p);
     }
   } else {
     for (size_t i = beg + threadIdx.x; i < end; i += 256) {
-      const float g = d.g[i] * gs;
-      const float m = gr.beta1 * d.m[i] + (1.f - gr.beta1) * g;
-      const float v = gr.beta2 * d.v[i] + (1.f - gr.beta2) * g * g;
-      float p = d.p[i] - step_size * m / (sqrtf(v) + gr.eps);
-      p -= decay * p;
+      float p = d.p[i], m = d.m[i], v = d.v[i];
+      adam_update(p, d.g[i], m, v, c);
       d.p[i] = p; d.m[i] = m; d.v[i] = v;
+      if (zg) dg[i] = 0.f;
+      if (FUSED && cd.w) copy_st1(cd.w, wdt, i, p);
     }
   }
 }
@@ -749,18 +838,31 @@
   return check_launch("hero_adamw");
 }
 
-extern "C" int hero_adamw_multi(const HeroAdamWMulti* a, hero_stream_t stream) {
-  HERO_REQUIRE(a && a->descs && a->chunk_tensor && a->chunk_index, "hero_adamw_multi: null pointer");
-  HERO_REQUIRE(a->step >= 1 || a->step_ptr || a->tensor_steps, "hero_adamw_multi: step must be >= 1");
+static int adamw_multi_launch(const HeroAdamWMulti* a, bool fused, const void* copy_dst, int zero_grads, hero_stream_t stream, const char* who) {
+  HERO_REQUIRE(a && a->descs && a->chunk_tensor && a->chunk_index, "%s: null pointer", who);
+  HERO_REQUIRE(a->step >= 1 || a->step_ptr || a->tensor_steps, "%s: step must be >= 1", who);
   if (a->n_chunks <= 0) return HERO_OK;
   if (a->tensor_steps) {
-    HERO_REQUIRE(a->n_tensors > 0, "hero_adamw_multi: tensor_steps needs n_tensors");
+    HERO_REQUIRE(a->n_tensors > 0, "%s: tensor_steps needs n_tensors", who);
     hipLaunchKernelGGL(adamw_steps_inc_kernel, dim3((a->n_tensors + 255) / 256), dim3(256), 0, static_cast<hipStream_t>(stream), a->descs,
                        a->n_tensors, a->tensor_steps);
     const int rc = check_launch("hero_adamw_multi(steps)");
-    if (rc) return rc;
-  }
-  hipLaunchKernelGGL(adamw_multi_kernel, dim3(a->n_chunks), dim3(256), 0, static_cast<hipStream_t>(stream), *a);
-  return check_launch("hero_adamw_multi");
-}
+    if (rc != HERO_OK) return rc;
+  }
+  if (fused)
+    hipLaunchKernelGGL(adamw_multi_kernel<true>, dim3(a->n_chunks), dim3(256), 0, static_cast<hipStream_t>(stream), *a,
+                       static_cast<const AdamCopyDst*>(copy_dst), zero_grads);
+  else
+    hipLaunchKernelGGL(adamw_multi_kernel<false>, dim3(a->n_chunks), dim3(256), 0, static_cast<hipStream_t>(stream), *a,
+                       static_cast<const AdamCopyDst*>(nullptr), 0);
+  return check_launch(who);
+}
+extern "C" int hero_adamw_multi(const HeroAdamWMulti* a, hero_stream_t stream) {
+  return adamw_multi_launch(a, false, nullptr, 0, stream, "hero_adamw_multi");
+}
+extern "C" int hero_adamw_multi_fused(const HeroAdamWMulti* a, const void* copy_dst, int zero_grads, hero_stream_t stream) {
+  static_assert(sizeof(AdamCopyDst) == 32, "copy_dst records are 32 bytes (include/hero_hip.h)");
+  return adamw_multi_launch(a, true, copy_dst, zero_grads, stream, "hero_adamw_multi_fused");
+}
+extern "C" int hero_adamw_multi_tiles(void) { return MT_TILES; }
 extern "C" int hero_adamw_multi_chunk(void) { return MT_CHUNK; }
diff --git a/hero_amd/functional.py b/hero_amd/functional.py
--- a/hero_amd/functional.py
+++ b/hero_amd/functional.py
@@ -105,16 +105,53 @@
 _REFRESH_PINNED = set()
 
 
+_FUSED = [None]
+
+
+def fused_copy_targets():
+    ep, out = _WEPOCH[0], {}
+    for key, (sig, buf, params) in _WCACHE.items():
+        if sig is None or sig[2] != ep or any(not p.is_contiguous() or p.dtype != torch.float32 for p in params):
+            continue
+        transposed = len(key) == 3
+        esz, code, off = buf.element_size(), L.dt(buf), 0
+        for j, p in enumerate(params):
+            rows = p.shape[0] if p.dim() > 1 else 1
+            cols = p.numel() // rows
+            t = out.setdefault(id(p), {})
+            if transposed:
+                if "wt" not in t and sig[1][j] == p.data_ptr():
+                    t["wt"] = (buf.data_ptr() + off * esz, code, buf.shape[1], rows, cols, (key, j))
+                off += rows
+            else:
+                if "w" not in t and sig[1][j] == p.data_ptr():
+                    t["w"] = (buf.data_ptr() + off * esz, code, (key, j))
+                off += rows * cols
+    return out
+
+
+def copies_written_by_optimizer(written, updated):
+    _FUSED[0] = (_WEPOCH[0], frozenset(written), frozenset(updated))
+
+
 def refresh_weight_cache():
     if not _WCACHE:
         return
     entries = list(_WCACHE.items())
-    tsig = tuple((key, val[1].data_ptr(), tuple(p.data_ptr() for p in val[2])) for key, val in entries)
+    ep = _WEPOCH[0]
+    fused, _FUSED[0] = _FUSED[0], None
+    if fused is not None and fused[0] != ep:
+        fused = None
+    skip = tuple(fused is not None and val[0] is not None and val[0][2] == ep - 1 and
+                 ((key, j) in fused[1] or id(p) not in fused[2])
+                 for key, val in entries for j, p in enumerate(val[2]))
+    tsig = tuple((key, val[1].data_ptr(), tuple(p.data_ptr() for p in val[2])) for key, val in entries) + (skip,)
     if tsig not in _REFRESH:
         if len(_REFRESH) > 16:
             for k in [k for k in _REFRESH if k not in _REFRESH_PINNED][:8]:
                 del _REFRESH[k]
         descs, tdesc, tidx = [], [], []
+        flat = 0
         for key, (_, out, params) in entries:
             transposed = len(key) == 3
             esz, code = out.element_size(), L.dt(out)
@@ -130,20 +167,26 @@
                 else:
                     d = L.CopyDesc(p.data_ptr(), out.data_ptr() + off * esz, rows, cols, cols, 0, code, 0)
                     off += rows * cols
+                flat += 1
+                if skip[flat - 1]:
+                    continue
                 nt = (-(-rows // 64)) * (-(-cols // 64))
                 tdesc += [len(descs)] * nt
                 tidx += list(range(nt))
                 descs.append(d)
         dev = entries[0][1][1].device
-        arr = (L.CopyDesc * len(descs))(*descs)
-        raw = torch.frombuffer(bytearray(bytes(arr)), dtype=torch.uint8).to(dev)
-        _REFRESH[tsig] = (raw, torch.tensor(tdesc, dtype=torch.int32, device=dev),
-                          torch.tensor(tidx, dtype=torch.int32, device=dev), len(tdesc))
+        if descs:
+            arr = (L.CopyDesc * len(descs))(*descs)
+            raw = torch.frombuffer(bytearray(bytes(arr)), dtype=torch.uint8).to(dev)
+            _REFRESH[tsig] = (raw, torch.tensor(tdesc, dtype=torch.int32, device=dev),
+                              torch.tensor(tidx, dtype=torch.int32, device=dev), len(tdesc))
+        else:
+            _REFRESH[tsig] = (None, None, None, 0)
     if torch.cuda.is_current_stream_capturing():
         _REFRESH_PINNED.add(tsig)
     raw, tdesc, tidx, n = _REFRESH[tsig]
-    L.check(L.lib().hero_copy_multi(raw.data_ptr(), tdesc.data_ptr(), tidx.data_ptr(), n, L.stream()))
-    ep = _WEPOCH[0]
+    if n:
+        L.check(L.lib().hero_copy_multi(raw.data_ptr(), tdesc.data_ptr(), tidx.data_ptr(), n, L.stream()))
     for key, (_, out, params) in entries:
         _WCACHE[key] = ((tuple(p._version for p in params), tuple(p.data_ptr() for p in params), ep), out, params)
 
diff --git a/hero_amd/optim/adamw.py b/hero_amd/optim/adamw.py
--- a/hero_amd/optim/adamw.py
+++ b/hero_amd/optim/adamw.py
@@ -25,6 +25,7 @@
         self._tsteps = None
         self._slots = None
         self.last_active = []
+        self.last_fused = None
 
     def load_state_dict(self, state_dict):
         super().load_state_dict(state_dict)
@@ -69,10 +70,11 @@
                 self.state[p]["step"] = host[i]
         self._global_step = max([self._global_step] + host)
 
-    def _build_table(self, active, slots=False):
-        chunk = L.lib().hero_adamw_multi_chunk()
-        descs = (L.TensorDesc * len(active))()
-        ct, ci = [], []
+    def _build_table(self, active, slots=False, clear=(), targets=None):
+        chunk, tiles = L.lib().hero_adamw_multi_chunk(), L.lib().hero_adamw_multi_tiles()
+        descs = (L.TensorDesc * (len(active) + len(clear)))()
+        copy = np.zeros(len(descs), dtype=[("w", "u8"), ("wt", "u8"), ("rows", "i4"), ("cols", "i4"), ("ldt", "i4"), ("dtypes", "i4")])
+        ct, ci, written = [], [], []
         for i, (gi, p) in enumerate(active):
             st = self.state[p]
             g = p.grad
@@ -81,17 +83,36 @@
             descs[i] = L.TensorDesc(L.ptr(p), L.ptr(g), L.ptr(st["exp_avg"]), L.ptr(st["exp_avg_sq"]),
                                     p.numel(), gi, self._slots[p] if slots else self._global_step - st["step"])
             n = -(-p.numel() // chunk)
+            t = (targets or {}).get(id(p), {})
+            if "w" in t:
+                copy[i]["w"], wcode, tag = t["w"]
+                copy[i]["dtypes"] = wcode
+                written.append(tag)
+            if "wt" in t and p.dim() == 2:
+                copy[i]["wt"], tcode, copy[i]["ldt"], rows, cols, tag = t["wt"]
+                copy[i]["rows"], copy[i]["cols"] = rows, cols
+                copy[i]["dtypes"] |= tcode << 8
+                written.append(tag)
+                n = -(-((-(-rows // 64)) * (-(-cols // 64))) // tiles)
             ct.extend([i] * n)
             ci.extend(range(n))
-        dev = active[0][1].device
+        for i, g in enumerate(clear, len(active)):
+            if not g.is_contiguous():
+                raise RuntimeError("hero_amd AdamW needs contiguous gradients")
+            descs[i] = L.TensorDesc(None, L.ptr(g), None, None, g.numel(), 0, 0)
+            n = -(-g.numel() // chunk)
+            ct.extend([i] * n)
+            ci.extend(range(n))
+        dev = active[0][1].device if active else clear[0].device
         raw = torch.frombuffer(bytearray(bytes(descs)), dtype=torch.uint8).to(dev)
         t_ct = torch.from_numpy(np.asarray(ct, dtype=np.int32)).to(dev)
         t_ci = torch.from_numpy(np.asarray(ci, dtype=np.int32)).to(dev)
-        return raw, t_ct, t_ci, len(ct)
+        t_copy = torch.from_numpy(copy.view(np.uint8).copy()).to(dev) if written else None
+        return raw, t_ct, t_ci, len(ct), t_copy, tuple(written), len(descs)
 
     @torch.no_grad()
     def step(self, closure=None, grad_sumsq=None, max_grad_norm=0.0, grad_scale=1.0, skip=None,
-             step_tensor=None, lr_tensor=None):
+             step_tensor=None, lr_tensor=None, zero_grads=False, write_copies=False, clear=()):
         loss = closure() if closure is not None else None
         device_state = step_tensor is not None
         if not device_state:
@@ -112,36 +133,46 @@
                 if not device_state:
                     st["step"] += 1
                 active.append((gi, p))
-        if not active:
+        clear = list(clear) if zero_grads else []
+        if not active and not clear:
             return loss
-        tsteps = self._device_steps(active[0][1].device) if device_state else None
+        dev = active[0][1].device if active else clear[0].device
+        tsteps = self._device_steps(dev) if device_state else None
         self.last_active = active
-        sig = self._table_for(active, device_state)
-        raw, t_ct, t_ci, n_chunks = self._tables[sig]
-        return self._launch(raw, t_ct, t_ci, n_chunks, len(active), tsteps, grad_sumsq, max_grad_norm, grad_scale, step_tensor, lr_tensor, loss)
+        self.last_fused = (bool(zero_grads), bool(write_copies), clear) if (zero_grads or write_copies) else None
+        sig = self._table_for(active, device_state, self.last_fused)
+        return self._launch(self._tables[sig], active, tsteps, grad_sumsq, max_grad_norm, grad_scale, step_tensor, lr_tensor, loss,
+                            self.last_fused)
 
-    def prebuild(self, active, device_state=True):
+    def prebuild(self, active, device_state=True, fused=None):
         if active:
             self._device_steps(active[0][1].device)
-            self._table_for(list(active), device_state)
+            self._table_for(list(active), device_state, fused)
 
-    def _table_for(self, active, device_state):
+    def _table_for(self, active, device_state, fused=None):
         if device_state:
             sig = ("dev",) + tuple((id(p), p.data_ptr(), p.grad.data_ptr(), self.state[p]["exp_avg"].data_ptr(),
                                     self.state[p]["exp_avg_sq"].data_ptr(), self._slots[p]) for _, p in active)
         else:
             sig = tuple((id(p), p.data_ptr(), p.grad.data_ptr(), self.state[p]["exp_avg"].data_ptr(),
                          self.state[p]["exp_avg_sq"].data_ptr(), self._global_step - self.state[p]["step"]) for _, p in active)
+        clear, targets = (), None
+        if fused is not None:
+            clear = fused[2]
+            targets = HF.fused_copy_targets() if fused[1] else {}
+            sig += ("fused", tuple((g.data_ptr(), g.numel()) for g in clear),
+                    tuple(tuple(sorted((k, v[:-1]) for k, v in targets.get(id(p), {}).items())) for _, p in active))
         capturing = torch.cuda.is_current_stream_capturing()
         if sig not in self._tables:
             if len(self._tables) >= 16 and not capturing:
                 self._tables = {}
-            self._tables[sig] = self._build_table(active, slots=device_state)
+            self._tables[sig] = self._build_table(active, slots=device_state, clear=clear, targets=targets)
         if capturing and not any(t is self._tables[sig] for t in self._pinned):
             self._pinned.append(self._tables[sig])
         return sig
 
-    def _launch(self, raw, t_ct, t_ci, n_chunks, n_active, tsteps, grad_sumsq, max_grad_norm, grad_scale, step_tensor, lr_tensor, loss):
+    def _launch(self, table, active, tsteps, grad_sumsq, max_grad_norm, grad_scale, step_tensor, lr_tensor, loss, fused=None):
+        raw, t_ct, t_ci, n_chunks, t_copy, written, n_descs = table
         a = L.AdamWMulti()
         a.descs, a.chunk_tensor, a.chunk_index, a.n_chunks = raw.data_ptr(), t_ct.data_ptr(), t_ci.data_ptr(), n_chunks
         for gi, group in enumerate(self.param_groups):
@@ -149,9 +180,14 @@
             a.groups[gi] = L.AdamWGroup(group["lr"], b1, b2, group["eps"], group["weight_decay"])
         a.step = max(self._global_step, 1)
         a.step_ptr, a.lr_ptr = L.ptr(step_tensor), L.ptr(lr_tensor)
-        a.tensor_steps, a.n_tensors = L.ptr(tsteps), n_active
+        a.tensor_steps, a.n_tensors = L.ptr(tsteps), n_descs
         a.grad_sumsq = L.ptr(grad_sumsq)
         a.max_grad_norm, a.grad_scale = max_grad_norm, grad_scale
-        L.check(L.lib().hero_adamw_multi(C.byref(a), L.stream()))
+        if fused is None:
+            L.check(L.lib().hero_adamw_multi(C.byref(a), L.stream()))
+        else:
+            L.check(L.lib().hero_adamw_multi_fused(C.byref(a), L.ptr(t_copy), int(fused[0]), L.stream()))
         HF.notify_weights_updated()
+        if fused is not None and fused[1]:
+            HF.copies_written_by_optimizer(written, [id(p) for _, p in active])
         return loss
diff --git a/hero_amd/step.py b/hero_amd/step.py
--- a/hero_amd/step.py
+++ b/hero_amd/step.py
@@ -50,7 +50,7 @@
 
 class TrainStep:
     def __init__(self, model, opts=None, task="tvr", bucket_bytes=64 << 20, use_graph=False, static_usage=False,
-                 grad_compress="bf16", uniform_shapes=False, graph_collectives=None):
+                 grad_compress="bf16", uniform_shapes=False, graph_collectives=None, fused_boundary=True):
         self.model = model
         self.opts = SimpleNamespace(**{**TVR_OPTS, **(opts or {})})
         self.task = task
@@ -62,6 +62,9 @@
         self.arena = D.GradArena(list(model.parameters()), bucket_bytes=bucket_bytes,
                                  groups=qkv_groups(model), static_usage=static_usage,
                                  compress=grad_compress if D.collectives_active() else None)
+        self.fused_boundary = bool(fused_boundary) and hasattr(self.optimizer, "last_fused")
+        optimised = {id(p) for g in self.optimizer.param_groups for p in g["params"]}
+        self._never_optimised = [p for p in self.arena.params if id(p) not in optimised]
         self.micro = 0
         self.global_step = 0
         D.broadcast_tensors([p.data for p in model.parameters()], 0)
@@ -104,12 +107,16 @@
         sumsq = self.optimizer.grad_sumsq(self.arena.flat) if self.opts.grad_norm != -1 else None
         if device_state:
             self._step_t.add_(1)
+        kw = {}
+        if self.fused_boundary:
+            kw = dict(zero_grads=True, write_copies=True,
+                      clear=[self.arena.grad_slice(p) for p in untouched + self._never_optimised])
         self.optimizer.step(grad_sumsq=sumsq, max_grad_norm=float(self.opts.grad_norm),
                             grad_scale=1.0 / D.world_size(), skip=set(untouched),
                             step_tensor=self._step_t if device_state else None,
-                            lr_tensor=self._lr_t if device_state else None)
+                            lr_tensor=self._lr_t if device_state else None, **kw)
         HF.refresh_weight_cache()
-        self.arena.zero()
+        self.arena.zero(fill=not self.fused_boundary)
 
     def _set_lr(self):
         self.global_step += 1
@@ -201,7 +208,8 @@
         self._graph_gen = getattr(self, "_graph_gen", {})
         self._graph_gen[key] = HF.weight_cache_generation()
         self._active_of = getattr(self, "_active_of", {})
-        self._active_of[key] = list(getattr(self.optimizer, "last_active", []))
+        self._active_of[key] = (list(getattr(self.optimizer, "last_active", [])),
+                                getattr(self.optimizer, "last_fused", None))
 
     def prepare(self, batch, task=None):
         task = task or self.task
@@ -234,7 +242,8 @@
         if self.micro % accum == 0 and self._graph_gen[key] != HF.weight_cache_generation():
             torch.cuda.synchronize()
             if hasattr(self.optimizer, "prebuild"):
-                self.optimizer.prebuild(self._active_of.get(key, []))
+                active, fused = self._active_of.get(key, ([], None))
+                self.optimizer.prebuild(active, fused=fused)
             self._record(self._graphs[key][4], task)
         ga, loss_a, gb, loss_b, static_batch = self._graphs[key]
         if batch is not static_batch:
diff --git a/hero_amd/utils/distributed.py b/hero_amd/utils/distributed.py
--- a/hero_amd/utils/distributed.py
+++ b/hero_amd/utils/distributed.py
@@ -329,8 +329,13 @@
             times.append(e0.elapsed_time(e1))
         return sorted(times[1:])[len(times[1:]) // 2]
 
-    def zero(self):
-        self.flat.zero_()
+    def grad_slice(self, p):
+        s, e = self.slices[p]
+        return self.flat[s:e]
+
+    def zero(self, fill=True):
+        if fill:
+            self.flat.zero_()
         self.touched.clear()
         for p in self.params:
             if p.grad is None:
diff --git a/include/hero_hip.h b/include/hero_hip.h
--- a/include/hero_hip.h
+++ b/include/hero_hip.h
@@ -223,6 +223,9 @@
 int hero_adamw_multi(const HeroAdamWMulti* a, hero_stream_t stream);
 int hero_adamw_multi_chunk(void);
 
+int hero_adamw_multi_fused(const HeroAdamWMulti* a, const void* copy_dst, int zero_grads, hero_stream_t stream);
+int hero_adamw_multi_tiles(void);
+
 typedef struct HeroCopyDesc {
   const float* src;
   void* dst;
```

Result: no change. 5340 videos/s (-0.2%).
